# SimingShan/red-diffeq

Hardware: AMD Instinct MI355X
Metric: shot-timesteps/sec (fwd+adj) + per-iter FWI wallclock, OpenFWI 70×70 (higher is better)
Workload: dtype f32; 1 GPU; configs[1]: OpenFWI FlatVel-A 70x70 (310x310 padded), 8 shots/GPU (8 total), nt=1000, fwd+adj gradient + TV + Adam step; global_batch=1, shots_per_gpu=8, shots_total=8, nt=1000, parallelism=shot-parallel x1

## Files before the change

### include/red_diffeq_fwi.h

```cpp
#ifndef RED_DIFFEQ_FWI_H
#define RED_DIFFEQ_FWI_H

#include <stddef.h>
#include <stdint.h>
#include <hip/hip_runtime_api.h>

#ifdef __cplusplus
extern "C" {
#endif

#define RDQ_E_INVALID (-10001)
#define RDQ_E_NOMEM (-10002)
#define RDQ_E_HANDOFF (-10003)

typedef struct rdq_fwi_geom {
    int32_t nz, nx;
    int32_t nbc;
    int32_t nt;
    int32_t ns, ng;
    int32_t sample_temporal;
    float dx, dt;
    int32_t isz, igz;
    const int32_t *isx;
    const int32_t *igx;
    const double *wavelet;
} rdq_fwi_geom;

typedef struct rdq_fwi_plan rdq_fwi_plan;

typedef struct rdq_fwi_sizes_t {
    int32_t Hp, Wp, ld, nrec;
    size_t coeffs;
    size_t vstat;
    size_t seis;
    size_t history;
    size_t ring;
    size_t gA;
    size_t gk_part;
    size_t gbeta;
    size_t colsum;
} rdq_fwi_sizes_t;

int rdq_fwi_plan_create(const rdq_fwi_geom *geom, rdq_fwi_plan **plan);
int rdq_fwi_plan_destroy(rdq_fwi_plan *plan);
int rdq_fwi_sizes(const rdq_fwi_plan *plan, int32_t B, rdq_fwi_sizes_t *out);
int rdq_fwi_set_graphs(rdq_fwi_plan *plan, int32_t enable);
int rdq_fwi_set_tuning(rdq_fwi_plan *plan, int32_t fwd_steps, int32_t adj_steps, int32_t chains);
#define RDQ_VARIANT_FWD_GEN 1
#define RDQ_VARIANT_ADJ_EXACT 2
#define RDQ_VARIANT_NO_XCD_LOCAL 4
#define RDQ_VARIANT_NARROW_CHUNKED 8
#define RDQ_VARIANT_CHUNKED_ADJ_FMA 16
int rdq_fwi_set_variant(rdq_fwi_plan *plan, int32_t flags);
int rdq_fwi_set_wide_adj_steps(rdq_fwi_plan *plan, int32_t steps);
int rdq_fwi_set_wide_adj_shots(rdq_fwi_plan *plan, int32_t shots);
int rdq_fwi_set_wide_fwd_shots(rdq_fwi_plan *plan, int32_t shots);
int rdq_fwi_set_wide_fwd_steps(rdq_fwi_plan *plan, int32_t steps);
int rdq_fwi_set_rows_per_wave(rdq_fwi_plan *plan, int32_t fwd_rows, int32_t adj_rows);
int rdq_fwi_set_sweep_delay(rdq_fwi_plan *plan, int32_t fwd_ticks, int32_t adj_ticks);
int rdq_fwi_set_persistent(rdq_fwi_plan *plan, int32_t mode);
int rdq_fwi_status(rdq_fwi_plan *plan, hipStream_t stream);
int rdq_fwi_debug_words(rdq_fwi_plan *plan, uint32_t out[32]);
int rdq_fwi_set_status_buffer(rdq_fwi_plan *plan, uint32_t *words);
int rdq_fwi_launch_info(rdq_fwi_plan *plan, int32_t B, int32_t out[6]);
int rdq_fwi_wide_info(rdq_fwi_plan *plan, int32_t B, int32_t out[4]);
int rdq_fwi_set_profile(rdq_fwi_plan *plan, int32_t enable);
int rdq_fwi_read_profile(rdq_fwi_plan *plan, uint64_t out[12]);
int rdq_fwi_profile_waves(rdq_fwi_plan *plan, int32_t adj, uint64_t *out, size_t count);

#define RDQ_VEL_NORMALIZED 0
#define RDQ_VEL_PHYSICAL 1

int rdq_fwi_coeffs(const rdq_fwi_plan *plan, int32_t B, const float *v, const int64_t strides[4],
                   int32_t vel_mode, float *coeffs, void *vstat, hipStream_t stream);

int rdq_fwi_forward(const rdq_fwi_plan *plan, int32_t B, const float *coeffs, float *seis,
                    float *history, float *ring, hipStream_t stream);

int rdq_fwi_adjoint(const rdq_fwi_plan *plan, int32_t B, const float *coeffs,
                    const float *history, const float *dseis, float *ring, float *gA,
                    double *gk_part, float *gbeta, hipStream_t stream);

typedef struct rdq_fwi_ckpt_sizes_t {
    int32_t nseg; int32_t seg_levels;
    size_t ckpt;
    size_t seg;
} rdq_fwi_ckpt_sizes_t;
int rdq_fwi_ckpt_sizes(const rdq_fwi_plan *plan, int32_t B, int32_t K, rdq_fwi_ckpt_sizes_t *out);
int rdq_fwi_forward_ckpt(const rdq_fwi_plan *plan, int32_t B, int32_t K, const float *coeffs,
                         float *seis, float *ckpt, float *ring, hipStream_t stream);
int rdq_fwi_adjoint_ckpt(const rdq_fwi_plan *plan, int32_t B, int32_t K, const float *coeffs,
                         const float *ckpt, float *seg, const float *dseis, float *ring,
                         float *gA, double *gk_part, float *gbeta, hipStream_t stream);
int rdq_fwi_ckpt_info(rdq_fwi_plan *plan, int32_t B, int32_t K, int32_t out[4]);

int rdq_fwi_grad_finalize(const rdq_fwi_plan *plan, int32_t B, const float *coeffs,
                          const void *vstat, const float *gA, const double *gk_part,
                          const float *gbeta, int32_t vel_mode, double *colsum, float *g_v,
                          hipStream_t stream);

size_t rdq_l1_partial_bytes(int32_t B, int64_t n);
int rdq_l1_forward(int32_t B, int64_t n, const float *pred, const float *y, const float *mask,
                   float *loss, float *nobs, void *partial, hipStream_t stream);
int rdq_l1_backward(int32_t B, int64_t n, const float *pred, const float *y, const float *mask,
                    const float *nobs, const float *gout, float *dpred, hipStream_t stream);

int rdq_smooth_reg_forward(int32_t kind, int32_t B, int32_t H, int32_t W, const float *mu,
                           float *loss, hipStream_t stream);
int rdq_smooth_reg_backward(int32_t kind, int32_t B, int32_t H, int32_t W, const float *mu,
                            const float *gout, float *grad, hipStream_t stream);

#ifdef __cplusplus
}
#endif
#endif
```

### red-diffeq_amd/csrc/fwi.hip

```cpp
#include <hip/hip_runtime.h>

#include <algorithm>
#include <atomic>
#include <cmath>
#include <cstdint>
#include <cstdlib>
#include <cstring>
#include <new>
#include <vector>
#include <initializer_list>
#include <mutex>
#include <utility>

#include "red_diffeq_fwi.h"

#pragma clang fp contract(off)

namespace {

constexpr float C1X2 = -5.0f;
constexpr float C2 = (float)(4.0 / 3.0);
constexpr float C3 = (float)(-1.0 / 12.0);

#define RDQ_CHECK(x)                                   \
// ... 710 lines not shown
        rofs[r] = wrapn(uz, g.Hp) * g.ld;                                                          \
        const int rr = w * R + r;                                                                  \
        if (rr >= H && rr < RH - H && uz < g.Hp) rin |= 1u << r;                                   \
    }

template <int T, int NW, int R, bool GEN, bool PAIR>
__global__ __launch_bounds__(64 * NW) void k_fwd_tw(FwdTBArgs a)
{
    __shared__ f32x2 xch[2][NW][4][64];
    __shared__ f32x2 As[NW][R][64];
    TW_REGION_INIT()
    const int jg = s - g.s_off, s_first = g.s_off + jg * a.spw, nsh = min(a.spw, a.ns_sh - jg * a.spw);
    (void)bs; (void)so;
    f32x2 C1[R], C2v[R];
    unsigned smask = 0;
    int rrow = -1;
    {
        const float *AL = a.coeffs + (size_t)b * g.slice;
        const __amdgpu_buffer_rsrc_t RA = rsrc_of(AL, sbytes), R1 = rsrc_of(AL + g.cstride, sbytes),
                                     R2 = rsrc_of(AL + 2 * g.cstride, sbytes);
#pragma unroll
        for (int r = 0; r < R; ++r) {
            const int gz = wrapn(uz0 + r, g.Hp);
            if constexpr (GEN) {
                const Coef c0 = gen_coef(a.cg, b, gz, gx0), c1 = gen_coef(a.cg, b, gz, gx1);
                As[w][r][lane] = f32x2{c0.al, c1.al}; C1[r] = f32x2{c0.t1, c1.t1}; C2v[r] = f32x2{c0.t2, c1.t2};
            } else {
                As[w][r][lane] = ld2<PAIR>(RA, v0, v1, rofs[r] * 4);
                C1[r] = ld2<PAIR>(R1, v0, v1, rofs[r] * 4);
                C2v[r] = ld2<PAIR>(R2, v0, v1, rofs[r] * 4);
            }
            if (gz == g.isz) smask |= 1u << r;
            if (gz == g.igz) rrow = r;
        }
    }
    int rs0 = 0, re0 = 0, rs1 = 0, re1 = 0;
    if (rrow >= 0) { rs0 = g.rcv_start[gx0]; re0 = g.rcv_start[gx0 + 1]; rs1 = g.rcv_start[gx1]; re1 = g.rcv_start[gx1 + 1]; }
    const int rc0 = xin0 && rs0 < re0 ? g.rcv_list[rs0] : -1, rc1 = xin1 && rs1 < re1 ? g.rcv_list[rs1] : -1;
    const bool rmulti = __any(re0 - rs0 > 1 || re1 - rs1 > 1);
    const f32x2 kC2 = {C2, C2}, kC3 = {C3, C3};
    auto kargs = [&]() {
        const __attribute__((address_space(4))) FwdTBArgs *k_ =
            (const __attribute__((address_space(4))) FwdTBArgs *)__builtin_amdgcn_kernarg_segment_ptr();
        asm volatile("" : "+s"(k_));
        return k_;
    };
    f32x2 P0[R], P1[R];
    auto load_shot = [&](int ss_) {
        const auto *k_ = kargs();
        const size_t so_ = (size_t)(b * k_->g.ns + ss_) * k_->g.slice;
        const __amdgpu_buffer_rsrc_t RPv = rsrc_of(k_->in_prev + so_, sbytes), RCu = rsrc_of(k_->in_cur + so_, sbytes);
#pragma unroll
        for (int r = 0; r < R; ++r) {
            P0[r] = ld2<PAIR>(RPv, v0, v1, rofs[r] * 4);
            P1[r] = ld2<PAIR>(RCu, v0, v1, rofs[r] * 4);
        }
    };
    load_shot(s_first);
    for (int sh = 0; sh < nsh; ++sh) {
    const auto *ka = kargs();
    const int ss = s_first + sh, bss = b * ka->g.ns + ss;
    const size_t soo = (size_t)bss * ka->g.slice;
    if ((T & 1) && sh) __syncthreads();
    const int isx = ka->g.isx[ss];
    const bool sc0 = gx0 == isx, sc1 = gx1 == isx;
    const float bsrc = smask ? ka->coeffs[4 * ka->g.cstride + (size_t)b * ka->g.slice + (size_t)ka->g.isz * ka->g.ld + isx] : 0.0f;
#pragma unroll
    for (int t = 0; t < T; ++t) {
        f32x2 *cur = (t & 1) ? P0 : P1;
        f32x2 *prv = (t & 1) ? P1 : P0;
        tw_put<NW, R>(xch, t & 1, w, lane, cur);
        __syncthreads();
        const Halo2 h2 = tw_get<NW>(xch, t & 1, w, lane);
#pragma unroll
        for (int r = 0; r < R; ++r) {
            TW_VERT(cur, r, h2, zm2, zm1, zp1, zp2)
            const f32x2 c = cur[r];
            const HTaps x = htaps(c);
            f32x2 s1 = zm1 + zp1; s1 = s1 + x.l1; s1 = s1 + x.r1;
            f32x2 s2 = zm2 + zp2; s2 = s2 + x.l2; s2 = s2 + x.r2;
            f32x2 lap = kC2 * s1; const f32x2 l2 = kC3 * s2; lap = lap + l2;
            f32x2 a1 = C1[r] * c; const f32x2 a2 = C2v[r] * prv[r]; a1 = a1 - a2;
            const f32x2 a3 = As[w][r][lane] * lap;
            prv[r] = a1 + a3;
        }
        if (smask) {
            const float add = bsrc * ka->w[t];
            const f32x2 av = {sc0 ? add : -0.0f, sc1 ? add : -0.0f};
#pragma unroll
            for (int r = 0; r < R; ++r)
                if (smask & (1u << r)) prv[r] = prv[r] + av;
        }
        const int n = ka->n0 + t;
        if (ka->hist) {
            const __amdgpu_buffer_rsrc_t HS = rsrc_of(ka->hist + (size_t)(n + 2 - ka->hbase) * ka->g.level + soo, sbytes);
#pragma unroll
            for (int r = 0; r < R; ++r)
                if (rin & (1u << r)) st2<PAIR, CP_NT>(prv[r], HS, vi0, vi1, rofs[r] * 4);
        }
        if (ka->seis && rrow >= 0 && (rin & (1u << rrow)) && (n % ka->g.st) == 0) {
            f32x2 val = prv[0];
#pragma unroll
            for (int r = 1; r < R; ++r) if (r == rrow) val = prv[r];
            float *SK = ka->seis + ((size_t)bss * ka->g.nrec + n / ka->g.st) * ka->g.ng;
            if (rc0 >= 0) SK[rc0] = val.x;
            if (rc1 >= 0) SK[rc1] = val.y;
            if (rmulti) {
                if (xin0) for (int j = rs0 + 1; j < re0; ++j) SK[ka->g.rcv_list[j]] = val.x;
                if (xin1) for (int j = rs1 + 1; j < re1; ++j) SK[ka->g.rcv_list[j]] = val.y;
            }
        }
    }
    if (ka->out_cur) {
        constexpr bool odd = (T & 1) != 0;
        const __amdgpu_buffer_rsrc_t OC = rsrc_of(ka->out_cur + soo, sbytes), OP = rsrc_of(ka->out_prev + soo, sbytes);
#pragma unroll
        for (int r = 0; r < R; ++r)
            if (rin & (1u << r)) {
                st2<PAIR>(odd ? P0[r] : P1[r], OC, vi0, vi1, rofs[r] * 4);
                st2<PAIR>(odd ? P1[r] : P0[r], OP, vi0, vi1, rofs[r] * 4);
            }
    }
    if (sh + 1 < nsh) load_shot(ss + 1);
    }
}

template <int T, int NW, int R, bool PAIR, bool EXACT>
__global__ __launch_bounds__(64 * NW) void k_adj_tw(AdjTBArgs a)
{
    __shared__ f32x2 xq[2][NW][4][64];
    __shared__ f32x2 xp[2][NW][4][64];
    __shared__ f32x2 As[NW][R][64];
    TW_REGION_INIT()
    const int jg = s - g.s_off, s_first = g.s_off + jg * a.spw, nsh = min(a.spw, a.ns_sh - jg * a.spw);
    (void)bs; (void)so;
    f32x2 KP[R];
    unsigned pmask = 0, smask = 0, rmask = 0;
    const f32x2 kC2 = {C2, C2}, kC3 = {C3, C3}, kC1X2 = {C1X2, C1X2}, k2 = {2.0f, 2.0f}, k1 = {1.0f, 1.0f};
    const bool plane = lane >= H / 2 - 1 && lane < 64 - H / 2 + 1;
    const int pv0 = plane ? v0 : OOB, pv1 = plane ? v1 : OOB;
    {
        int gz[R];
#pragma unroll
        for (int r = 0; r < R; ++r) {
            gz[r] = wrapn(uz0 + r, g.Hp);
            const int rr = w * R + r;
            if (rr >= H - 2 && rr < RH - H + 2) pmask |= 1u << r;
            if (gz[r] == g.isz) smask |= 1u << r;
            if (gz[r] == g.igz) rmask |= 1u << r;
        }
        Coef c0[R], c1[R];
#pragma unroll
        for (int r = 0; r < R; ++r) { c0[r] = gen_coef(a.cg, b, gz[r], gx0); c1[r] = gen_coef(a.cg, b, gz[r], gx1); }
#pragma unroll
        for (int r = 0; r < R; ++r) { As[w][r][lane] = f32x2{c0[r].al, c1[r].al}; KP[r] = f32x2{c0[r].kp, c1[r].kp}; }
    }
    const int rcv0 = rmask ? g.rlane[gx0] : -1, rcv1 = rmask ? g.rlane[gx1] : -1;
    f32x2 L0[R], L1[R], GA[R], Pn[R];
    auto kargs = [&]() {
        const __attribute__((address_space(4))) AdjTBArgs *k_ =
            (const __attribute__((address_space(4))) AdjTBArgs *)__builtin_amdgcn_kernarg_segment_ptr();
        asm volatile("" : "+s"(k_));
        return k_;
    };
    auto load_shot = [&](int ss_) {
        const auto *k_ = kargs();
        const size_t so_ = (size_t)(b * k_->g.ns + ss_) * k_->g.slice;
        const __amdgpu_buffer_rsrc_t RL1 = rsrc_of(k_->in_l1 + so_, sbytes), RL2 = rsrc_of(k_->in_l2 + so_, sbytes);
        const __amdgpu_buffer_rsrc_t RG = rsrc_of(k_->gA + so_, sbytes);
        const __amdgpu_buffer_rsrc_t HR = rsrc_of(k_->hist + (size_t)(k_->k0 - k_->hbase) * k_->g.level + so_, sbytes);
#pragma unroll
        for (int r = 0; r < R; ++r) L1[r] = ld2<PAIR>(RL1, v0, v1, rofs[r] * 4);
#pragma unroll
        for (int r = 0; r < R; ++r) L0[r] = ld2<PAIR>(RL2, v0, v1, rofs[r] * 4);
#pragma unroll
        for (int r = 0; r < R; ++r) Pn[r] = (pmask & (1u << r)) ? ld2<PAIR>(HR, pv0, pv1, rofs[r] * 4) : f32x2{0.0f, 0.0f};
#pragma unroll
        for (int r = 0; r < R; ++r) GA[r] = (rin & (1u << r)) ? ld2<PAIR>(RG, vi0, vi1, rofs[r] * 4) : f32x2{0.0f, 0.0f};
    };
    load_shot(s_first);
    for (int sh = 0; sh < nsh; ++sh) {
    const auto *ka = kargs();
    const int ss = s_first + sh, bss = b * ka->g.ns + ss;
    const size_t soo = (size_t)bss * ka->g.slice;
    const int isx = ka->g.isx[ss];
    const bool sc0 = xin0 && gx0 == isx, sc1 = xin1 && gx1 == isx;
    const __amdgpu_buffer_rsrc_t DSR = rsrc_of(ka->dseis + (size_t)bss * ka->g.nrec * ka->g.dstride);
    const bool gbl = (smask & rin) && (sc0 || sc1);
    float gbacc = gbl ? ka->gbeta[bss] : 0.0f;
    double ksum = 0.0;
#pragma unroll
    for (int t = 0; t < T; ++t) {
        __builtin_amdgcn_sched_barrier(0);
        const int k = ka->k0 - t;
        f32x2 *cur = (t & 1) ? L0 : L1;
        f32x2 *prv = (t & 1) ? L1 : L0;
        f32x2 P[R];
#pragma unroll
        for (int r = 0; r < R; ++r) P[r] = Pn[r];
        if (t + 1 < T) {
            const __amdgpu_buffer_rsrc_t HR = rsrc_of(ka->hist + (size_t)(k - 1 - ka->hbase) * ka->g.level + soo, sbytes);
#pragma unroll
            for (int r = 0; r < R; ++r) if (pmask & (1u << r)) Pn[r] = ld2<PAIR>(HR, pv0, pv1, rofs[r] * 4);
        }
        const int ri = rmask ? rec_index(k - 1, ka->g.st) : -1;
        f32x2 dsv = {-0.0f, -0.0f};
        if (ri >= 0) {
            const int ro = ri * ka->g.dstride;
            const float d0 = bload(DSR, rcv0 >= 0 ? (ro + rcv0) * 4 : OOB, 0);
            const float d1 = bload(DSR, rcv1 >= 0 ? (ro + rcv1) * 4 : OOB, 0);
            dsv = f32x2{rcv0 >= 0 ? d0 : -0.0f, rcv1 >= 0 ? d1 : -0.0f};
        }
        f32x2 q[R];
#pragma unroll
        for (int r = 0; r < R; ++r) q[r] = As[w][r][lane] * cur[r];
        tw_put<NW, R>(xq, t & 1, w, lane, q);
        tw_put<NW, R>(xp, t & 1, w, lane, P);
        __syncthreads();
        const Halo2 hq = tw_get<NW>(xq, t & 1, w, lane);
        const Halo2 hp = tw_get<NW>(xp, t & 1, w, lane);
#pragma unroll
        for (int r = 0; r < R; ++r) {
            TW_VERT(q, r, hq, qm2, qm1, qp1, qp2)
            const HTaps x = htaps(q[r]);
            f32x2 n1 = qm1 + qp1; n1 = n1 + x.l1; n1 = n1 + x.r1;
            f32x2 n2 = qm2 + qp2; n2 = n2 + x.l2; n2 = n2 + x.r2;
            if constexpr (EXACT) {
                f32x2 nb = kC2 * n1; const f32x2 nb2 = kC3 * n2; nb = nb + nb2;
                f32x2 t1 = kC1X2 * As[w][r][lane]; t1 = t1 + k2; t1 = t1 - KP[r];
                const f32x2 t2 = k1 - KP[r];
                f32x2 l = t1 * cur[r]; const f32x2 l2 = t2 * prv[r]; l = l - l2; l = l + nb;
                prv[r] = l;
            } else {
                const f32x2 nb = fma2(kC3, n2, kC2 * n1);
                const f32x2 t1 = fma2(kC1X2, As[w][r][lane], k2) - KP[r], t2 = k1 - KP[r];
                prv[r] = fma2(t1, cur[r], fma2(-t2, prv[r], nb));
            }
        }
        if (ri >= 0) {
#pragma unroll
            for (int r = 0; r < R; ++r)
                if (rmask & (1u << r)) prv[r] = prv[r] + dsv;
        }
#pragma unroll
        for (int r = 0; r < R; ++r) {
            if (!(rin & (1u << r))) continue;
            TW_VERT(P, r, hp, pm2, pm1, pp1, pp2)
            const f32x2 pc = P[r];
            const HTaps x = htaps(pc);
            f32x2 s1 = pm1 + pp1; s1 = s1 + x.l1; s1 = s1 + x.r1;
            f32x2 s2 = pm2 + pp2; s2 = s2 + x.l2; s2 = s2 + x.r2;
            const f32x2 l = prv[r];
            const f32x2 dl = cur[r] - l;
            if constexpr (EXACT) {
                f32x2 lap = kC2 * s1; const f32x2 lq = kC3 * s2; lap = lap + lq;
                f32x2 d = kC1X2 * pc; d = d + lap;
                const f32x2 c = l * d;
                GA[r] = GA[r] + c;
                f32x2 kk = KP[r] * pc; kk = kk * dl;
                ksum += xin0 ? (double)kk.x : 0.0;
                ksum += xin1 ? (double)kk.y : 0.0;
            } else {
                const f32x2 d = fma2(kC1X2, pc, fma2(kC3, s2, kC2 * s1));
                GA[r] = fma2(l, d, GA[r]);
                const f32x2 kk = (KP[r] * pc) * dl;
                ksum += (double)(xin0 ? kk.x : 0.0f);
                ksum += (double)(xin1 ? kk.y : 0.0f);
            }
            if ((smask & (1u << r)) && (sc0 || sc1)) { const float gb = (sc0 ? l.x : l.y) * ka->w[t]; gbacc = gbacc + gb; }
        }
    }
    {
        constexpr bool odd = (T & 1) != 0;
        const __amdgpu_buffer_rsrc_t O1 = rsrc_of(ka->out_l1 + soo, sbytes), O2 = rsrc_of(ka->out_l2 + soo, sbytes);
        const __amdgpu_buffer_rsrc_t RG = rsrc_of(ka->gA + soo, sbytes);
#pragma unroll
        for (int r = 0; r < R; ++r)
            if (rin & (1u << r)) {
                st2<PAIR>(odd ? L0[r] : L1[r], O1, vi0, vi1, rofs[r] * 4);
                st2<PAIR>(odd ? L1[r] : L0[r], O2, vi0, vi1, rofs[r] * 4);
                st2<PAIR>(GA[r], RG, vi0, vi1, rofs[r] * 4);
            }
    }
    if (sh + 1 < nsh) load_shot(ss + 1);
    if (gbl) ka->gbeta[bss] = gbacc;
#pragma unroll
    for (int o = 32; o > 0; o >>= 1) ksum += __shfl_xor(ksum, o, 64);
    double *red = reinterpret_cast<double *>(&xq[0][0][0][0]);
    __syncthreads();
    if (lane == 0) red[w] = ksum;
    __syncthreads();
    if (threadIdx.x == 0) {
        double tot = red[0];
        for (int i = 1; i < NW; ++i) tot += red[i];
        unsafeAtomicAdd(&ka->gk_part[(size_t)bss * ka->nblk + ti.tile], tot);
    }
    }
}
#undef TW_VERT
#undef TW_REGION_INIT

constexpr int CP_SC1 = 16;
constexpr int PT_ADJ_SG = 8;
constexpr size_t PROF_RAW = 8;
constexpr size_t PROF_WAVES = 4096 * 16;
constexpr size_t PROF_WORDS = PROF_RAW + PROF_WAVES * 3;
constexpr unsigned long long PT_TIMEOUT_TICKS = 20000000ull;

typedef unsigned int u32x2 __attribute__((ext_vector_type(2)));
typedef unsigned int u32x4 __attribute__((ext_vector_type(4)));
typedef float f32x2 __attribute__((ext_vector_type(2)));
__device__ __forceinline__ u32x4 gran2(unsigned tag, float v0, float v1)
{
    u32x4 x;
    x.x = __float_as_uint(v0); x.y = tag; x.z = __float_as_uint(v1); x.w = tag;
    return x;
}
__device__ __forceinline__ void gran_put(__amdgpu_buffer_rsrc_t r, int voff, int soff, unsigned tag, float v0, float v1)
{
    __builtin_amdgcn_raw_buffer_store_b128(gran2(tag, v0, v1), r, voff, soff, CP_SC1);
}
__device__ __forceinline__ void gran_put_l2(__amdgpu_buffer_rsrc_t r, int voff, int soff, unsigned tag, float v0, float v1)
{
    __builtin_amdgcn_raw_buffer_store_b128(gran2(tag, v0, v1), r, voff, soff, 0);
}
__device__ __forceinline__ u32x4 gran_get(__amdgpu_buffer_rsrc_t r, int voff, int soff)
{
    return __builtin_amdgcn_raw_buffer_load_b128(r, voff, soff, CP_SC1);
}

__device__ __forceinline__ float wav_s(const float *w, int i)
{
    return ((const __attribute__((address_space(4))) float *)w)[i];
}

__device__ __forceinline__ int wrap_row(int uz, int Hp)
{
    uz = uz < 0 ? uz + Hp : uz;
    return uz >= Hp ? uz - Hp : uz;
}

struct PtTile { int tx, ty, tile, sl; bool valid, local; };
constexpr unsigned long long PT_ARRIVE_TICKS = 10000000ull;

__device__ PtTile pt_assign(const TBGeo &g, unsigned *status, int xcd_mode)
{
    __shared__ int sh[3];
    unsigned *cnt = status + 16;
    if (threadIdx.x == 0) {
        unsigned x = 0;
        if (xcd_mode) {
            asm volatile("s_getreg_b32 %0, hwreg(HW_REG_XCC_ID)" : "=s"(x));
            x &= 7u;
        }
        const unsigned slot = __hip_atomic_fetch_add(cnt + x, 1u, __ATOMIC_RELAXED, __HIP_MEMORY_SCOPE_AGENT);
        unsigned n[8], tot = 0;
        const unsigned long long t0 = __builtin_amdgcn_s_memrealtime();
        bool ok = true;
        for (;;) {
            tot = 0;
            for (int i = 0; i < 8; ++i) {
                n[i] = __hip_atomic_load(cnt + i, __ATOMIC_RELAXED, __HIP_MEMORY_SCOPE_AGENT);
                tot += n[i];
            }
            if (tot >= gridDim.x) break;
            if (__builtin_amdgcn_s_memrealtime() - t0 > PT_ARRIVE_TICKS) { ok = false; break; }
            __builtin_amdgcn_s_sleep(2);
        }
        int sl = -1, tile = 0, local = 0;
        if (ok) {
            const int Tt = g.ntiles, S = g.nsl;
            int placed = 0, take[8];
            for (int i = 0; i < 8; ++i) {
                take[i] = xcd_mode ? min((int)n[i] / Tt, S - placed) : 0;
                placed += take[i];
            }
            int base = 0;
            for (int i = 0; i < (int)x; ++i) base += take[i];
            if ((int)slot < take[x] * Tt) {
                sl = base + (int)slot / Tt; tile = (int)slot % Tt; local = 1;
            } else {
                int r = (int)slot - take[x] * Tt;
                for (int i = 0; i < (int)x; ++i) r += (int)n[i] - take[i] * Tt;
                if (r < (S - placed) * Tt) { sl = placed + r / Tt; tile = r % Tt; }
            }
        } else {
            __hip_atomic_store(status, 2u, __ATOMIC_RELAXED, __HIP_MEMORY_SCOPE_AGENT);
        }
        sh[0] = sl; sh[1] = tile; sh[2] = local;
    }
    __syncthreads();
    PtTile t;
    t.sl = sh[0]; t.tile = sh[1]; t.local = sh[2] != 0;
    t.valid = t.sl >= 0;
    t.ty = t.tile / g.tiles_x;
    t.tx = t.tile - t.ty * g.tiles_x;
    return t;
}

#define PT_REGION_INIT(NW_, RW_)                                                                    \
    PT_REGION_HEAD(NW_, RW_)                                                                        \
    const int bs = __builtin_amdgcn_readfirstlane(g.sl_off + ti.sl);                                \
    const int b = __builtin_amdgcn_readfirstlane(bs / g.ns);                                        \
    const int s = __builtin_amdgcn_readfirstlane(bs - b * g.ns);                                    \
    PT_REGION_GEOM()

#define PT_REGION_HEAD(NW_, RW_)                                                                    \
    constexpr int R = (RW_), RP = (RW_) / 2, RH = (NW_) * (RW_), H = 2 * T, IW = 64 - 2 * H,       \
                  IH = RH - 2 * H;                                                                  \
    const int lane = threadIdx.x & 63;                                                              \
    const int w = __builtin_amdgcn_readfirstlane(threadIdx.x >> 6);                                \
    const PtTile ti = pt_assign(g, a.status, a.xcd_mode);                                           \
    if (!ti.valid) return;                                                                          \
    const bool gl2 = ti.local;

#define PT_REGION_GEOM()                                                                            \
    const int tx = __builtin_amdgcn_readfirstlane(ti.tx), ty = __builtin_amdgcn_readfirstlane(ti.ty); \
    const int tile = __builtin_amdgcn_readfirstlane(ti.tile);                                       \
    const int ux = tx * IW - H + lane;                                                              \
    const int gx = wrapn(ux, g.Wp);                                                                 \
    const bool xin = lane >= H && lane < 64 - H && ux < g.Wp;                                       \
    const int vw = min(IW, g.Wp - tx * IW), vh = min(IH, g.Hp - ty * IH);                           \
    const bool bx = g.tiles_x == 1 || lane - H < H || lane - H >= vw - H;                           \
    const bool cx = lane - H < vw + H;                                                              \
    const int uz0 = ty * IH - H + w * R;                                                            \
    unsigned rin = 0, rby = 0, rcy = 0;                                                             \
    _Pragma("unroll") for (int r = 0; r < R; ++r) {                                                 \
        const int rr = w * R + r, ly = rr - H;                                                      \
        if (rr >= H && rr < RH - H && uz0 + r < g.Hp) rin |= 1u << r;                               \
        if (g.ntiles == g.tiles_x || ly < H || ly >= vh - H) rby |= 1u << r;                        \
        if (ly < vh + H) rcy |= 1u << r;                                                            \
    }                                                                                               \
    const size_t so = (size_t)bs * g.slice;                                                         \
    const int vo16 = gx * 16;                                                                       \
    const bool hx = !xin && cx, xb = xin && bx;                                                     \
                                                        \
    const int vo_hx = hx ? vo16 : OOB, vo_cx = cx ? vo16 : OOB;                                     \
    const int vo_xin = xin ? vo16 : OOB, vo_xb = xb ? vo16 : OOB;                                   \
    const bool keep_in = xin || cx;
#define PT_ROFS(r) (wrap_row(uz0 + (r), g.Hp) * g.ld)

#define PT_SWEEP(GR, TAG, V0, V1, SG)                                                               \
    {                                                                                               \
        unsigned long long t0_ = 0;                                                                 \
        const unsigned long long ts_ = prof ? __builtin_amdgcn_s_memrealtime() : 0;                 \
        if constexpr (PT_PRIO) __builtin_amdgcn_s_setprio(PT_PRIO_WAIT);                            \
        for (unsigned pass_ = 0; live; ++pass_) {                                                   \
             \
            unsigned rin_ = rin, rcy_ = rcy;                                                        \
            LAUNDER(rin_); LAUNDER(rcy_);                                                           \
            bool ok_ = true;                                                                        \
            _Pragma("unroll") for (int g_ = 0; g_ < R; g_ += (SG)) {                                \
                u32x4 x_[(SG)];                                                                     \
                int o_[(SG)];                                                                       \
                constexpr int GN_ = (SG) < R ? (SG) : R;    \
                _Pragma("unroll") for (int i_ = 0; i_ < GN_; ++i_) {                                \
                    const int r = g_ + i_ < R ? g_ + i_ : R - 1;                                    \
                    const bool rowin_ = g_ + i_ < R && ((rin_ >> r) & 1u), rowcy_ = g_ + i_ < R && ((rcy_ >> r) & 1u); \
                    o_[i_] = rowin_ ? vo_hx : (rowcy_ ? vo_cx : OOB);                               \
                    x_[i_] = gran_get(GR, o_[i_], PT_ROFS(r) * 16);                                 \
                }                                                                                   \
                _Pragma("unroll") for (int i_ = 0; i_ < GN_; ++i_) {                                \
                    const int r = g_ + i_ < R ? g_ + i_ : R - 1;                                    \
                    const bool nd_ = o_[i_] != OOB;                                                 \
                    ok_ = ok_ && (!nd_ || (x_[i_].y == (TAG) && x_[i_].w == (TAG)));                \
                    PT_AT(V0, r) = nd_ ? __uint_as_float(x_[i_].x) : PT_AT(V0, r);                  \
                    PT_AT(V1, r) = nd_ ? __uint_as_float(x_[i_].z) : PT_AT(V1, r);                  \
                }                                                                                   \
            }                                                                                       \
            const bool done_ = __all(ok_);                                                          \
            if (prof && pass_ == 0) tfp += __builtin_amdgcn_s_memrealtime() - ts_;                   \
            if (done_) { npass += pass_ + 1; break; }                                               \
            if (pass_ == 0) t0_ = __builtin_amdgcn_s_memrealtime();                                 \
            if ((pass_ & 15) == 15) {                                                               \
                if (__hip_atomic_load(a.status, __ATOMIC_RELAXED, __HIP_MEMORY_SCOPE_AGENT) != 0)   \
                    live = false;                                                                   \
                else if (__builtin_amdgcn_s_memrealtime() - t0_ > PT_TIMEOUT_TICKS) {               \
                    __hip_atomic_store(a.status, 1u, __ATOMIC_RELAXED, __HIP_MEMORY_SCOPE_AGENT);   \
                    if (lane == 0) {                          \
                        a.status[1] = (TAG); a.status[2] = blockIdx.x; a.status[3] = bs;            \
                        a.status[4] = tile; a.status[5] = gl2; a.status[6] = w;                      \
                    }                                                                               \
                    live = false;                                                                   \
                }                                                                                   \
            }                                                                                       \
            __builtin_amdgcn_s_sleep(1);                                                            \
        }                                                                                           \
        if constexpr (PT_PRIO) __builtin_amdgcn_s_setprio(PT_PRIO_SWEPT);                           \
                     \
        unsigned rin_ = rin, rcy_ = rcy;                                                            \
        LAUNDER(rin_); LAUNDER(rcy_);                                                               \
        _Pragma("unroll") for (int r = 0; r < R; ++r) {                                             \
            const bool rowin_ = (rin_ >> r) & 1u, rowcy_ = (rcy_ >> r) & 1u;                        \
            const bool keep_ = rowin_ ? keep_in : (rowcy_ && cx);                                   \
            PT_AT(V0, r) = keep_ ? PT_AT(V0, r) : 0.0f;                                             \
            PT_AT(V1, r) = keep_ ? PT_AT(V1, r) : 0.0f;                                             \
        }                                                                                           \
    }

#define PT_PUBLISH(GR, TAG, V0, V1)                                                                 \
    {                                                                                               \
        unsigned rin_ = rin, rby_ = rby;                                                            \
        LAUNDER(rin_); LAUNDER(rby_);                                                               \
        if (gl2) {                                                                                  \
            _Pragma("unroll") for (int r = 0; r < R; ++r) {                                         \
                if (!((rin_ >> r) & 1u)) continue;                                                  \
                gran_put_l2(GR, ((rby_ >> r) & 1u) ? vo_xin : vo_xb, PT_ROFS(r) * 16, (TAG),        \
                            PT_AT(V0, r), PT_AT(V1, r));                                            \
            }                                                                                       \
        } else {                                                                                    \
            _Pragma("unroll") for (int r = 0; r < R; ++r) {                                         \
                if (!((rin_ >> r) & 1u)) continue;                                                  \
                gran_put(GR, ((rby_ >> r) & 1u) ? vo_xin : vo_xb, PT_ROFS(r) * 16, (TAG),           \
                         PT_AT(V0, r), PT_AT(V1, r));                                               \
            }                                                                                       \
        }                                                                                           \
    }

#define PT_SWEEP_DELAY()                                                                            \
    if (a.sweep_delay > 0) {                                                                        \
        const unsigned long long d0_ = __builtin_amdgcn_s_memrealtime();                            \
        while (__builtin_amdgcn_s_memrealtime() - d0_ < (unsigned long long)a.sweep_delay)          \
            __builtin_amdgcn_s_sleep(1);                                                            \
    }

#define PT_PROF(ACC)                                                                                \
    if (prof) { const unsigned long long now_ = __builtin_amdgcn_s_memrealtime(); ACC += now_ - tm; tm = now_; }

#define LAUNDER(x)                                                                                  \
    do {                                                                                            \
        x = __builtin_amdgcn_readfirstlane(x);    \
        asm volatile("" : "+s"(x));                                                                 \
    } while (0)

struct FwdPtArgs {
    TBGeo g;
    const float *coeffs;
    const float *wav;
    float *hist;
    float *seis;
    unsigned long long *gran;
    unsigned *status;
    unsigned long long *prof;
    int nt;
    int xcd_mode;
    int sweep_delay;
};

#define FWD_HIST(V, N)                                                                              \
    {                                                                                               \
        const int so_ = ((N) - n0) * L4;                                                            \
        _Pragma("unroll") for (int r = 0; r < R; ++r)                                               \
            __builtin_amdgcn_raw_buffer_store_b32(__float_as_uint(PT_AT(V, r)), HFe, hv[r], so_, CP_NT); \
    }
#define FWD_RECORD                                                                                  \
    {                                                                                               \
        int rrw_ = rrow;                                                                            \
        LAUNDER(rrw_);                                                                              \
        if (rrw_ >= 0) {                                                                            \
            _Pragma("unroll") for (int t = 0; t < T; ++t) {                                         \
                const int n = n0 + t;                                                               \
                const int ri_ = n < a.nt ? rec_index(n, g.st) : -1;                                 \
                if (ri_ >= 0) {                                                                     \
                    __builtin_amdgcn_raw_buffer_store_b32(__float_as_uint(rv[t]), SKR, vrec, ri_ * ng4, 0); \
                    unsigned rm_ = rmulti;                                                          \
                    LAUNDER(rm_);                                                                   \
                    if (rm_ && rec) {                          \
                        float *SK = a.seis + ((size_t)bs * g.nrec + ri_) * g.ng;                    \
                        for (int j = rs + 1; j < re; ++j) SK[g.rcv_list[j]] = rv[t];                \
                    }                                                                               \
                }                                                                                   \
            }                                                                                       \
        }                                                                                           \
    }

template <int RP, bool M>
__device__ constexpr int pt_pair(int r) { return M ? (r < RP ? r : 2 * RP - 1 - r) : r % RP; }
template <int RP, bool M>
__device__ constexpr int pt_half(int r) { return M ? (r < RP ? 0 : 1) : r / RP; }
#define PT_AT(V, r) V[pt_pair<RP, PT_MIR>(r)][pt_half<RP, PT_MIR>(r)]
__device__ __forceinline__ f32x2 swp(f32x2 v) { return f32x2{v.y, v.x}; }
#define MIR_VERT(X, i, m1, p1, m2, p2)                                                              \
    const f32x2 m1 = (i) >= 1 ? X[(i) - 1] : E1;                                                    \
    const f32x2 p1 = (i) <= RP - 2 ? X[(i) + 1] : swp(X[RP - 1]);                                   \
    const f32x2 m2 = (i) >= 2 ? X[(i) - 2] : ((i) == 1 ? E1 : E2);                                  \
    const f32x2 p2 = (i) <= RP - 3 ? X[(i) + 2] : ((i) == RP - 2 ? swp(X[RP - 1]) : swp(X[RP - 2]));

#define FWD_PAIRS_NB(CUR, PRV, LO, HI)                                                                        \
    {                                                                                               \
        _Pragma("unroll") for (int i = (LO); i < (HI); ++i) {                                        \
            MIR_VERT(CUR, i, m1, p1, m2, p2)                                                        \
            f32x2 s1 = m1 + p1; s1 = s1 + xl1[i]; s1 = s1 + xr1[i];                                 \
            const f32x2 la = kC2 * s1;                                                              \
            f32x2 s2 = m2 + p2;                               \
            s2.x = s2.x + dpp_shr1(xl1[i].x); s2.y = s2.y + dpp_shr1(xl1[i].y);                     \
            s2.x = s2.x + dpp_shl1(xr1[i].x); s2.y = s2.y + dpp_shl1(xr1[i].y);                     \
            const f32x2 l2 = kC3 * s2; const f32x2 lap = la + l2;                                   \
            const f32x2 a3 = A[i] * lap;                                                            \
            PRV[i] = tt[i] + a3;                                                                    \
        }                                                                                           \
        unsigned sm0_ = (HI) > (LO) ? smask : 0u;                                                  \
        LAUNDER(sm0_);                                    \
        if (sm0_) {                                   \
            float wt_ = wv[t];                                                                      \
            asm volatile("" : "+s"(wt_));                                                           \
            const float add = scol ? bsrc * wt_ : -0.0f;                                            \
            unsigned one_ = s1row;                                                                  \
            LAUNDER(one_);                                                                          \
            if (one_) {                                                                             \
                const f32x2 av = shalf ? f32x2{-0.0f, add} : f32x2{add, -0.0f};                     \
                int sp_ = spair;                                                                    \
                LAUNDER(sp_);                                                                       \
                _Pragma("unroll") for (int i = (LO); i < (HI); ++i)                                  \
                    if (i == sp_) PRV[i] = PRV[i] + av;                                             \
            } else {                                                                                \
                unsigned sm_ = smask;                                                               \
                LAUNDER(sm_);                                                                       \
                _Pragma("unroll") for (int r = 0; r < R; ++r)                                       \
                    if (pt_pair<RP, PT_MIR>(r) >= (LO) && pt_pair<RP, PT_MIR>(r) < (HI) && ((sm_ >> r) & 1u)) \
                        PT_AT(PRV, r) = PT_AT(PRV, r) + add;                                        \
            }                                                                                       \
        }                                                                                           \
    }
#define FWD_STEP_NB(CUR, PRV)                                                                       \
    {                                                                                               \
        u32x2 f_;                                                                                   \
        f32x2 E1, E2;                                                                               \
        xm_load<NW>(xm, n & 1, w, lane, f_, E1, E2);                                                \
        f32x2 xl1[RP], xr1[RP], tt[RP];                                                             \
        _Pragma("unroll") for (int i = 0; i < RP; ++i) {                                             \
            const f32x2 c = CUR[i];                                                                 \
            xl1[i] = f32x2{dpp_shr1(c.x), dpp_shr1(c.y)};                                           \
            xr1[i] = f32x2{dpp_shl1(c.x), dpp_shl1(c.y)};                                           \
            f32x2 a1 = C1[i] * c; const f32x2 a2 = C2v[i] * PRV[i]; a1 = a1 - a2;                   \
            tt[i] = a1;                                                                             \
            asm volatile("" : "+v"(tt[i]));              \
        }                                                                                           \
        xm_wait<NW>(xm, n & 1, w, lane, (unsigned)n + 1u, f_, E1, E2, a.status, live);              \
        FWD_PAIRS_NB(CUR, PRV, 0, 2)                                                                          \
        if (t + 1 < T) xm_put<NW>(xm, (n + 1) & 1, w, lane, (unsigned)n + 2u, PRV[0], PRV[1]);      \
        __builtin_amdgcn_s_setprio(PT_PRIO_BODY);                                                   \
        FWD_PAIRS_NB(CUR, PRV, 2, RP)                                                                         \
        if (a.hist && (t + 1 < T || e + 1 == nep)) FWD_HIST(PRV, n)                                 \
        int rr_ = rrow;                                                                             \
        LAUNDER(rr_);                                                                               \
        if (rr_ >= 0) {                               \
            int rp_ = rpair;                                                                        \
            LAUNDER(rp_);                                                                           \
            f32x2 v_ = PRV[0];                                                                      \
            _Pragma("unroll") for (int i = 1; i < RP; ++i) if (i == rp_) v_ = PRV[i];                \
            rv[t] = rhalf ? v_.y : v_.x;                                                            \
        }                                                                                           \
    }

template <int T, int NW, int RW, bool PROF>
__global__ __launch_bounds__(64 * NW) void k_fwd_pt(FwdPtArgs a)
{
    unsigned long long *const prof = PROF ? a.prof : nullptr;
    constexpr bool PT_MIR = true;
    constexpr bool PT_PRIO = true;
    __shared__ XmBox<NW> xm;
    const TBGeo &g = a.g;
    PT_REGION_INIT(NW, RW)
    const float *AL = a.coeffs + (size_t)b * g.slice;
    f32x2 A[RP], C1[RP], C2v[RP], P0[RP], P1[RP];
    const f32x2 kC2 = {C2, C2}, kC3 = {C3, C3};
    unsigned smask = 0;
    int rrow = -1;
#pragma unroll
    for (int r = 0; r < R; ++r) {
        const int gz = wrap_row(uz0 + r, g.Hp);
        const int o = gz * g.ld + gx;
        PT_AT(A, r) = AL[o]; PT_AT(C1, r) = AL[g.cstride + o]; PT_AT(C2v, r) = AL[2 * g.cstride + o];
        PT_AT(P0, r) = 0.0f; PT_AT(P1, r) = 0.0f;
        if (gz == g.isz) smask |= 1u << r;
        if (gz == g.igz && ((rin >> r) & 1u)) rrow = r;
    }
    smask = __builtin_amdgcn_readfirstlane(smask);
    rrow = __builtin_amdgcn_readfirstlane(rrow);
    const int isx = g.isx[s];
    const bool scol = gx == isx;
    const float bsrc = (smask != 0) ? AL[4 * g.cstride + (size_t)g.isz * g.ld + isx] : 0.0f;

    int rs = 0, re = 0, rcv0 = -1;
    if (rrow >= 0) {
        rs = g.rcv_start[gx]; re = g.rcv_start[gx + 1];
        rcv0 = rs < re ? g.rcv_list[rs] : -1;
    }
    const bool rec = rrow >= 0 && xin && rcv0 >= 0;
    const unsigned rmulti = __any(re - rs > 1);
    const __amdgpu_buffer_rsrc_t SKR = rsrc_of(a.seis + (size_t)bs * g.nrec * g.ng);
    const int vrec = rec ? rcv0 * 4 : OOB, ng4 = g.ng * 4;
    const unsigned s1row = smask != 0 && (smask & (smask - 1u)) == 0;
    const int sr1 = smask ? __builtin_ctz(smask) : 0;
    const int spair = __builtin_amdgcn_readfirstlane(PT_MIR ? (sr1 < RP ? sr1 : R - 1 - sr1) : sr1 % RP);
    const int rpair = __builtin_amdgcn_readfirstlane(rrow < 0 ? 0 : PT_MIR ? (rrow < RP ? rrow : R - 1 - rrow) : rrow % RP);
    const bool shalf = sr1 >= RP, rhalf = rrow >= RP;
    float rv[T];
#pragma unroll
    for (int t = 0; t < T; ++t) rv[t] = 0.0f;
    const size_t L = g.level;
    const int L4 = (int)(L * 4);
    int hv[R];
#pragma unroll
    for (int r = 0; r < R; ++r) hv[r] = (((rin >> r) & 1u) && xin) ? (PT_ROFS(r) + gx) * 4 : OOB;
    const int nep = (a.nt + T - 1) / T;
    bool live = true;
    unsigned long long tsw = 0, tst = 0, tpb = 0, tm = prof ? __builtin_amdgcn_s_memrealtime() : 0;
    unsigned long long tfp = 0, npass = 0;
    float wv[T];
#pragma unroll
    for (int t = 0; t < T; ++t) wv[t] = wav_s(a.wav, min(t, a.nt - 1));
    __builtin_amdgcn_s_waitcnt(0x0F70);
#define FWD_ISSUE _Pragma("unroll") for (int t = 0; t < T; ++t) wv[t] = wav_s(a.wav, min(n0 + T + t, a.nt - 1));
    xm_init<NW>(xm, w, lane);
    __syncthreads();
    xm_put<NW>(xm, 0, w, lane, 1u, f32x2{0.0f, 0.0f}, f32x2{0.0f, 0.0f});
#define FWD_STEP_SEL FWD_STEP_NB
    for (int e = 0; e < nep; ++e) {
        const int n0 = e * T;
        const __amdgpu_buffer_rsrc_t HFe = rsrc_of(a.hist + (size_t)(n0 + 2) * L + so);
        PT_PROF(tsw)
#pragma unroll
        for (int t = 0; t < T; ++t) {
            const int n = n0 + t;
            if (n >= a.nt) break;
            if (t & 1) FWD_STEP_SEL(P0, P1)
            else FWD_STEP_SEL(P1, P0)
        }
        if (T & 1) {
#pragma unroll
            for (int i = 0; i < RP; ++i) { const f32x2 tmp = P0[i]; P0[i] = P1[i]; P1[i] = tmp; }
        }
        PT_PROF(tst)
        if (e + 1 < nep) {
            const unsigned tag = (unsigned)(e + 1);
            const __amdgpu_buffer_rsrc_t GR = rsrc_of(a.gran + (size_t)(2 * ((e + 1) & 1)) * L + 2 * so);
            PT_PUBLISH(GR, tag, P0, P1)
            PT_PROF(tpb)
            FWD_ISSUE
            PT_SWEEP_DELAY()
            PT_SWEEP(GR, tag, P0, P1, R)
            if (a.hist) FWD_HIST(P1, n0 + T - 1)
            xm_put<NW>(xm, (n0 + T) & 1, w, lane, (unsigned)(n0 + T) + 1u, P1[0], P1[1]);
        }
        FWD_RECORD
    }
#undef FWD_STEP_SEL
#undef FWD_ISSUE
    PT_PROF(tsw)
    if (prof && lane == 0) {
        atomicAdd(prof + 0, tsw); atomicAdd(prof + 1, tst); atomicAdd(prof + 2, tpb); atomicAdd(prof + 3, 1ull);
        atomicAdd(prof + 4, tfp); atomicAdd(prof + 5, npass);
        if (blockIdx.x < PROF_WAVES / 16) {
            unsigned long long *raw = prof + PROF_RAW + ((size_t)blockIdx.x * 16 + w) * 3;
            raw[0] = tsw; raw[1] = tst; raw[2] = tpb;
        }
    }
}

#undef FWD_HIST
#undef FWD_RECORD


struct AdjPtArgs {
    TBGeo g;
    const float *coeffs;
    const float *wav;
    const float *hist;
    const float *dseis;
    float *gA;
    double *gk_part;
    float *gbeta;
    unsigned long long *gran;
    unsigned *status;
    unsigned long long *prof;
    int nt, nblk;
    int xcd_mode;
    int sweep_delay;
};

__device__ __forceinline__ float bload_nt(__amdgpu_buffer_rsrc_t r, int voff, int soff)
{
    return __uint_as_float(__builtin_amdgcn_raw_buffer_load_b32(r, voff, soff, CP_NT));
}

#define ADJ_PLOAD(PC, PH, HR, SOFF)                                                                 \
    {                                                                                               \
        const int so_ = (SOFF);                                                                     \
        _Pragma("unroll") for (int i = 0; i < RP; ++i) {                                             \
            PC[i].x = bload_nt(HR, pv[i + 2], so_);                                                 \
            PC[i].y = bload_nt(HR, pv[i + 6], so_);                                                 \
        }                                                                                           \
        PH[0] = bload_nt(HR, pv[0], so_); PH[1] = bload_nt(HR, pv[1], so_);                         \
        PH[2] = bload_nt(HR, pv[10], so_); PH[3] = bload_nt(HR, pv[11], so_);                       \
    }

#define PAIR_VERT(X, i, m1, p1, m2, p2)                                                             \
    const f32x2 m1 = (i) >= 1 ? X[(i) - 1] : eU1;                                                   \
    const f32x2 p1 = (i) <= RP - 2 ? X[(i) + 1] : eD1;                                              \
    const f32x2 m2 = (i) >= 2 ? X[(i) - 2] : ((i) == 1 ? eU1 : eU2);                                \
    const f32x2 p2 = (i) <= RP - 3 ? X[(i) + 2] : ((i) == RP - 2 ? eD1 : eD2);

#define ADJ_GRAD(CU, LN, P, PH, WK)                                                                 \
    if (grad) {                                                                                     \
        const f32x2 eU1 = {PH[1], P[RP - 1].x}, eU2 = {PH[0], P[RP - 2].x};                         \
        const f32x2 eD1 = {P[0].y, PH[2]}, eD2 = {P[1].y, PH[3]};                                   \
        _Pragma("unroll") for (int i = 0; i < RP; ++i) {                                             \
            PAIR_VERT(P, i, m1, p1, m2, p2)                                                         \
            const f32x2 c = P[i];                                                                   \
            const f32x2 xl1 = {dpp_shr1(c.x), dpp_shr1(c.y)}, xr1 = {dpp_shl1(c.x), dpp_shl1(c.y)}; \
            f32x2 s1 = m1 + p1; s1 = s1 + xl1; s1 = s1 + xr1;                                       \
            f32x2 s2 = m2 + p2;                               \
            s2.x = s2.x + dpp_shr1(xl1.x); s2.y = s2.y + dpp_shr1(xl1.y);                           \
            s2.x = s2.x + dpp_shl1(xr1.x); s2.y = s2.y + dpp_shl1(xr1.y);                           \
            const f32x2 l = LN[i];                                                                  \
            f32x2 lap = kC2 * s1; const f32x2 lq = kC3 * s2; lap = lap + lq;                        \
            f32x2 d = kC1X2 * c; d = d + lap;                                                       \
            const f32x2 cc = l * d;                                                                 \
            GA[i] = GA[i] + cc;                                                                     \
            f32x2 kk = KP[i] * c; const f32x2 dl = CU[i] - l; kk = kk * dl;          \
            if (xin) {                                                               \
                if ((rin >> i) & 1u) ksum += (double)kk.x;                                          \
                if ((rin >> (i + RP)) & 1u) ksum += (double)kk.y;                                   \
            }                                                                                       \
        }                                                                                           \
        if (srow >= 0) {                                   \
            int sr_ = srow;                                                                         \
            LAUNDER(sr_);                                                                           \
            float ls_ = 0.0f;                                                                       \
            _Pragma("unroll") for (int r = 0; r < R; ++r) if (r == sr_) ls_ = PT_AT(LN, r);         \
            const float gb = scol ? ls_ * (WK) : -0.0f;                                             \
            gbacc = gbacc + gb;                                                                     \
        }                                                                                           \
    }

#define ADJ_STEP(CUR, PRV, P, PH, PN, PHN)                                                          \
    {                                                                                               \
        if (t + 1 < T) ADJ_PLOAD(PN, PHN, HRe, (T - 2 - t) * L4)                                    \
        const float dcur = dv[t];                                                                   \
        f32x2 q[RP];                                                                                \
        _Pragma("unroll") for (int i = 0; i < RP; ++i) q[i] = A[i] * CUR[i];                         \
        const Halo4 h4 = exchange_nw<NW>(xch, j & 1, w, lane, q[0].x, q[1].x, q[RP - 2].y, q[RP - 1].y); \
        const f32x2 eU1 = {h4.u1, q[RP - 1].x}, eU2 = {h4.u2, q[RP - 2].x};                         \
        const f32x2 eD1 = {q[0].y, h4.d1}, eD2 = {q[1].y, h4.d2};                                   \
        _Pragma("unroll") for (int i = 0; i < RP; ++i) {                                             \
            PAIR_VERT(q, i, m1, p1, m2, p2)                                                         \
            const f32x2 c = q[i];                                                                   \
            const f32x2 xl1 = {dpp_shr1(c.x), dpp_shr1(c.y)}, xr1 = {dpp_shl1(c.x), dpp_shl1(c.y)}; \
            f32x2 n1 = m1 + p1; n1 = n1 + xl1; n1 = n1 + xr1;                                       \
            f32x2 n2 = m2 + p2;                               \
            n2.x = n2.x + dpp_shr1(xl1.x); n2.y = n2.y + dpp_shr1(xl1.y);                           \
            n2.x = n2.x + dpp_shl1(xr1.x); n2.y = n2.y + dpp_shl1(xr1.y);                           \
            f32x2 nb = kC2 * n1; const f32x2 nb2 = kC3 * n2; nb = nb + nb2;                         \
            f32x2 l = T1v[i] * CUR[i]; const f32x2 l2 = T2v[i] * PRV[i]; l = l - l2; l = l + nb;     \
            PRV[i] = l;                                                                             \
        }                                                                                           \
        if (rrow >= 0 && rec_index(k - 1, g.st) >= 0) {       \
            int rr_ = rrow;                                                                         \
            LAUNDER(rr_);                                                                           \
            _Pragma("unroll") for (int r = 0; r < R; ++r)                                           \
                if (r == rr_) PT_AT(PRV, r) = PT_AT(PRV, r) + dcur;        \
        }                                                                                           \
        if (t + 1 < T || last) ADJ_GRAD(CUR, PRV, P, PH, wv[t])                                     \
    }

template <int T, int NW, bool PROF>
__global__ __launch_bounds__(64 * NW) void k_adj_pt(AdjPtArgs a)
{
    unsigned long long *const prof = PROF ? a.prof : nullptr;
    constexpr bool PT_MIR = false;
    constexpr bool PT_PRIO = false;
    __shared__ float xch[2][NW][4][64];
    __shared__ double red[64 * NW];
    const TBGeo &g = a.g;
    PT_REGION_INIT(NW, TB_R)
    const float *AL = a.coeffs + (size_t)b * g.slice;
    f32x2 A[RP], T1v[RP], T2v[RP], KP[RP], L0[RP], L1[RP], GA[RP];
    const f32x2 kC2 = {C2, C2}, kC3 = {C3, C3}, kC1X2 = {C1X2, C1X2};
    int srow = -1, rrow = -1;
#pragma unroll
    for (int r = 0; r < R; ++r) {
        const int gz = wrap_row(uz0 + r, g.Hp);
        const int o = gz * g.ld + gx;
        PT_AT(A, r) = AL[o]; PT_AT(T1v, r) = AL[g.cstride + o]; PT_AT(T2v, r) = AL[2 * g.cstride + o];
        PT_AT(KP, r) = AL[3 * g.cstride + o];
        PT_AT(L0, r) = 0.0f; PT_AT(L1, r) = 0.0f;
        PT_AT(GA, r) = 0.0f;
        if (gz == g.isz && ((rin >> r) & 1u)) srow = r;
        if (gz == g.igz) rrow = r;
    }
    const bool scol = xin && gx == g.isx[s];
    const int rcv0 = rrow >= 0 ? g.rlane[gx] : -1;
    const float *DSb = a.dseis + (size_t)bs * g.nrec * g.dstride;
    const __amdgpu_buffer_rsrc_t DSR = rsrc_of(DSb);
#define DLOAD(KK)                                                                                   \
    ({                                                                                              \
        const int ri_ = (KK) >= 1 ? rec_index((KK) - 1, g.st) : -1;                                 \
        const bool ok_ = rcv0 >= 0 && ri_ >= 0;                                                     \
        const float v_ = bload(DSR, ok_ ? (ri_ * g.dstride + rcv0) * 4 : OOB, 0);                   \
        ok_ ? v_ : -0.0f;                                                                           \
    })
    const bool grad = rin != 0;
    double ksum = 0.0;
    float gbacc = 0.0f;
    const size_t L = g.level;
    const int L4 = (int)(L * 4);
    f32x2 PA[RP], PB[RP];
    float PHA[4], PHB[4];
    int pv[12];
#pragma unroll
    for (int i = 0; i < 12; ++i) pv[i] = grad ? (wrap_row(uz0 + i - 2, g.Hp) * g.ld + gx) * 4 : OOB;
#define HIST_RSRC(KN) rsrc_of(a.hist + (ptrdiff_t)((KN) - (T - 1)) * (ptrdiff_t)L + (ptrdiff_t)so)
    float wv[T], dv[T];
    {
        const __amdgpu_buffer_rsrc_t H0 = HIST_RSRC(a.nt);
        ADJ_PLOAD(PA, PHA, H0, (T - 1) * L4)
    }
#pragma unroll
    for (int t = 0; t < T; ++t) {
        wv[t] = a.wav[max(a.nt - t - 1, 0)];
        dv[t] = DLOAD(a.nt - t);
    }
    __builtin_amdgcn_s_waitcnt(0x0F70);
#define ADJ_ISSUE                                                                                   \
    {                                                                                               \
        const __amdgpu_buffer_rsrc_t HN = HIST_RSRC(kn);                                            \
        ADJ_PLOAD(PA, PHA, HN, (T - 1) * L4)                                                        \
        _Pragma("unroll") for (int t = 0; t < T; ++t) {                                             \
            wv[t] = a.wav[max(kn - t - 1, 0)];                                                      \
            dv[t] = DLOAD(kn - t);                                                                  \
        }                                                                                           \
    }
    const int nep = (a.nt + T - 1) / T;
    bool live = true;
    unsigned long long tsw = 0, tst = 0, tpb = 0, tm = prof ? __builtin_amdgcn_s_memrealtime() : 0;
    unsigned long long tfp = 0, npass = 0;
    for (int e = 0; e < nep; ++e) {
        const int ke = a.nt - e * T;
        const bool last = e + 1 == nep;
        const __amdgpu_buffer_rsrc_t HRe = HIST_RSRC(ke);
#pragma unroll
        for (int t = 0; t < T; ++t) {
            const int j = e * T + t;
            if (j >= a.nt) break;
            const int k = ke - t;
            if (t & 1) ADJ_STEP(L0, L1, PB, PHB, PA, PHA)
            else ADJ_STEP(L1, L0, PA, PHA, PB, PHB)
        }
        if (T & 1) {
#pragma unroll
            for (int i = 0; i < RP; ++i) {
                const f32x2 tl = L0[i]; L0[i] = L1[i]; L1[i] = tl;
                const f32x2 tp = PA[i]; PA[i] = PB[i]; PB[i] = tp;
                const float th = PHA[i]; PHA[i] = PHB[i]; PHB[i] = th;
            }
        }
        PT_PROF(tst)
        if (!last) {
            const unsigned tag = (unsigned)(e + 1);
            const __amdgpu_buffer_rsrc_t GR = rsrc_of(a.gran + (size_t)(2 * ((e + 1) & 1)) * L + 2 * so);
            PT_PUBLISH(GR, tag, L0, L1)
            ADJ_GRAD(L0, L1, PB, PHB, wv[T - 1])
            const int kn = ke - T;
            PT_PROF(tpb)
            PT_SWEEP_DELAY()
            PT_SWEEP(GR, tag, L0, L1, PT_ADJ_SG)
            ADJ_ISSUE
            PT_PROF(tsw)
        }
    }
#undef DLOAD
#undef ADJ_ISSUE
#undef HIST_RSRC
    if (prof && lane == 0) {
        atomicAdd(prof + 0, tsw); atomicAdd(prof + 1, tst); atomicAdd(prof + 2, tpb); atomicAdd(prof + 3, 1ull);
        atomicAdd(prof + 4, tfp); atomicAdd(prof + 5, npass);
        if (blockIdx.x < PROF_WAVES / 16) {
            unsigned long long *raw = prof + PROF_RAW + ((size_t)blockIdx.x * 16 + w) * 3;
            raw[0] = tsw; raw[1] = tst; raw[2] = tpb;
        }
    }
    if (xin) {
#pragma unroll
        for (int r = 0; r < R; ++r)
            if ((rin >> r) & 1u) a.gA[so + (size_t)PT_ROFS(r) + gx] = PT_AT(GA, r);
    }
    if (srow >= 0 && scol) a.gbeta[bs] = gbacc;
    const int tid = threadIdx.x;
    red[tid] = ksum;
    __syncthreads();
    for (int w2 = 512; w2 > 0; w2 >>= 1) {
        if (tid < w2 && tid + w2 < 64 * NW) red[tid] += red[tid + w2];
        __syncthreads();
    }
    if (tid == 0) a.gk_part[(size_t)bs * a.nblk + tile] = red[0];
}

#define ADJR_LOAD(PD, HR, SOFF)                                                                     \
    {                                                                                               \
        const int so_ = (SOFF);                                                                     \
        _Pragma("unroll") for (int i = 0; i < RP; ++i) {                                             \
            PD[i].x = bload_nt(HR, pr[i], so_);                                                     \
            PD[i].y = bload_nt(HR, pr[R - 1 - i], so_);             \
        }                                                                                           \
    }

#define ADJR_GRAD(CU, LN, WK, P0, P1, P2)                                                           \
    if (grad) {                                                                                     \
        f32x2 u[RP];                                                                                \
        _Pragma("unroll") for (int i = 0; i < RP; ++i) {                                             \
            u[i] = fma2(-T1v[i], P1[i], P0[i]);                                                     \
            u[i] = fma2(T2v[i], P2[i], u[i]);                                                       \
        }                                                                                           \
        int sg_ = srow;                                \
        LAUNDER(sg_);                                                                               \
        if (sg_ >= 0) {                                                                             \
            int sp_ = spair;                                                                        \
            LAUNDER(sp_);                                                                           \
            const float sa_ = scol ? bsrc * (WK) : 0.0f;      \
            const f32x2 sv_ = shalf ? f32x2{0.0f, sa_} : f32x2{sa_, 0.0f};                          \
            f32x2 lp_ = LN[0];                                                                      \
            _Pragma("unroll") for (int i = 0; i < RP; ++i) {                                         \
                if (i == sp_) u[i] = u[i] - sv_;                                                    \
                if (i > 0 && i == sp_) lp_ = LN[i];                                                 \
            }                                                                                       \
            const float ls_ = shalf ? lp_.y : lp_.x;                                                \
            const float gb = scol ? ls_ * (WK) : -0.0f;     \
            gbacc = gbacc + gb;                                                                     \
        }                                                                                           \
             \
        _Pragma("unroll") for (int i = 0; i < RP; ++i) {                                             \
            const f32x2 dd = fma2(A[i], kC1X2 * P1[i], u[i]);                                       \
            GA[i] = fma2(LN[i], dd, GA[i]);                                                         \
            GK[i] = fma2(P1[i], CU[i] - LN[i], GK[i]);                                              \
        }                                                                                           \
    }

#define ADJR_PAIRS_NB(CUR, PRV, LO, HI)                                                             \
    {                                                                                               \
        _Pragma("unroll") for (int i = (LO); i < (HI); ++i) {                                        \
            MIR_VERT(q, i, m1, p1, m2, p2)                                                          \
            const f32x2 c = q[i];                                                                   \
            const f32x2 xl1 = {dpp_shr1(c.x), dpp_shr1(c.y)}, xr1 = {dpp_shl1(c.x), dpp_shl1(c.y)}; \
            f32x2 n1 = m1 + p1; n1 = n1 + xl1; n1 = n1 + xr1;                                       \
            f32x2 n2 = m2 + p2;                               \
            n2.x = n2.x + dpp_shr1(xl1.x); n2.y = n2.y + dpp_shr1(xl1.y);                           \
            n2.x = n2.x + dpp_shl1(xr1.x); n2.y = n2.y + dpp_shl1(xr1.y);                           \
            const f32x2 nb = fma2(kC3, n2, kC2 * n1);                                               \
            PRV[i] = fma2(T1v[i], CUR[i], fma2(-T2v[i], PRV[i], nb));                               \
        }                                                                                           \
        int rr_ = (LO) == 0 ? rlo : rhi;                   \
        LAUNDER(rr_);                                                                               \
        if ((HI) > (LO) && rr_ && rec_index(k - 1, g.st) >= 0) {                                    \
            int rp_ = rpair;                                                                        \
            LAUNDER(rp_);                                                                           \
            const f32x2 dv_ = rhalf ? f32x2{-0.0f, dcur} : f32x2{dcur, -0.0f};        \
            _Pragma("unroll") for (int i = (LO); i < (HI); ++i) if (i == rp_) PRV[i] = PRV[i] + dv_; \
        }                                                                                           \
    }
#define ADJR_STEP_NB(CUR, PRV, P0, P1, P2, PN)                                                      \
    {                                                                                               \
        if (ldall || (grad && k >= 2)) ADJR_LOAD(PN, HRe, (T - 1 - t) * L4)                         \
        const float dcur = dv[t];                                                                   \
        u32x2 f_;                                                                                   \
        f32x2 E1, E2;                                                                               \
        xm_load<NW>(xm, j & 1, w, lane, f_, E1, E2);                                                \
        f32x2 q[RP];                                                                                \
        _Pragma("unroll") for (int i = 0; i < RP; ++i) q[i] = A[i] * CUR[i];                         \
        xm_wait<NW>(xm, j & 1, w, lane, (unsigned)j + 1u, f_, E1, E2, a.status, live);              \
        ADJR_PAIRS_NB(CUR, PRV, 0, 2)                                                               \
        if (t + 1 < T) xm_put<NW>(xm, (j + 1) & 1, w, lane, (unsigned)j + 2u, A[0] * PRV[0], A[1] * PRV[1]); \
        __builtin_amdgcn_s_setprio(PT_PRIO_BODY);                                                   \
        ADJR_PAIRS_NB(CUR, PRV, 2, RP)                                                              \
        if (t + 1 < T || last) ADJR_GRAD(CUR, PRV, wv[t], P0, P1, P2)                               \
    }

template <int T, int NW, int RW, bool PROF>
__global__ __launch_bounds__(64 * NW) void k_adj_pr(AdjPtArgs a)
{
    unsigned long long *const prof = PROF ? a.prof : nullptr;
    constexpr bool PT_PRIO = true;
    constexpr bool PT_MIR = true;
    __shared__ XmBox<NW> xm;
    __shared__ double red[64 * NW];
    static_assert(sizeof(XmBox<NW>) + sizeof(double) * 64 * NW == (size_t)NW * 4608 && NW <= 16,
                  "k_adj_pr: 4 KB of mailboxes + 512 B of reduction per wave (72 KB at 16 waves)");
    const TBGeo &g = a.g;
    PT_REGION_INIT(NW, RW)
    const float *AL = a.coeffs + (size_t)b * g.slice;
    f32x2 A[RP], T1v[RP], T2v[RP], L0[RP], L1[RP], GA[RP], GK[RP];
    const f32x2 kC2 = {C2, C2}, kC3 = {C3, C3}, kC1X2 = {C1X2, C1X2};
    int srow = -1, rrow = -1;
#pragma unroll
    for (int r = 0; r < R; ++r) {
        const int gz = wrap_row(uz0 + r, g.Hp);
        const int o = gz * g.ld + gx;
        PT_AT(A, r) = AL[o]; PT_AT(T1v, r) = AL[g.cstride + o]; PT_AT(T2v, r) = AL[2 * g.cstride + o];
        PT_AT(L0, r) = 0.0f; PT_AT(L1, r) = 0.0f;
        PT_AT(GA, r) = 0.0f; PT_AT(GK, r) = 0.0f;
        if (gz == g.isz && ((rin >> r) & 1u)) srow = r;
        if (gz == g.igz) rrow = r;
    }
    const int isx = g.isx[s];
    const bool scol = xin && gx == isx;
    const float bsrc = srow >= 0 ? AL[4 * g.cstride + (size_t)g.isz * g.ld + isx] : 0.0f;
    const int rcv0 = rrow >= 0 ? g.rlane[gx] : -1;
    const float *DSb = a.dseis + (size_t)bs * g.nrec * g.dstride;
    const __amdgpu_buffer_rsrc_t DSR = rsrc_of(DSb);
    const int spair = __builtin_amdgcn_readfirstlane(srow < 0 ? 0 : srow < RP ? srow : R - 1 - srow);
    const int rpair = __builtin_amdgcn_readfirstlane(rrow < 0 ? 0 : rrow < RP ? rrow : R - 1 - rrow);
    const bool shalf = srow >= RP, rhalf = rrow >= RP;
    const int rlo = __builtin_amdgcn_readfirstlane(rrow >= 0 && rpair < 2 ? 1 : 0);
    const int rhi = __builtin_amdgcn_readfirstlane(rrow >= 0 && rpair >= 2 ? 1 : 0);
#define DLOAD(KK)                                                                                   \
    ({                                                                                              \
        const int ri_ = (KK) >= 1 ? rec_index((KK) - 1, g.st) : -1;                                 \
        const bool ok_ = rcv0 >= 0 && ri_ >= 0;                                                     \
        const float v_ = bload(DSR, ok_ ? (ri_ * g.dstride + rcv0) * 4 : OOB, 0);                   \
        ok_ ? v_ : -0.0f;                                                                           \
    })
    const bool grad = rin != 0;
    float gbacc = 0.0f;
    const size_t L = g.level;
    const int L4 = (int)(L * 4);
    f32x2 Q0[RP], Q1[RP], Q2[RP], Q3[RP];
    int pr[R];
#pragma unroll
    for (int r = 0; r < R; ++r)
        pr[r] = grad ? (PT_ROFS(r) + gx) * 4 : OOB;
#pragma unroll
    for (int i = 0; i < RP; ++i) { Q0[i] = 0.0f; Q1[i] = 0.0f; Q2[i] = 0.0f; Q3[i] = 0.0f; }
#define HIST_RSRC(KN) rsrc_of(a.hist + (ptrdiff_t)((KN) - T - 1) * (ptrdiff_t)L + (ptrdiff_t)so)
    float wv[T], dv[T];
    if (grad) {
        const __amdgpu_buffer_rsrc_t H0 = rsrc_of(a.hist + (ptrdiff_t)(a.nt - 1) * (ptrdiff_t)L + (ptrdiff_t)so);
        ADJR_LOAD(Q0, H0, 2 * L4)
        ADJR_LOAD(Q1, H0, L4)
        ADJR_LOAD(Q2, H0, 0)
    }
#pragma unroll
    for (int t = 0; t < T; ++t) {
        wv[t] = a.wav[max(a.nt - t - 1, 0)];
        dv[t] = DLOAD(a.nt - t);
    }
    __builtin_amdgcn_s_waitcnt(0x0F70);
#define ADJ_ISSUE                                                                                   \
    _Pragma("unroll") for (int t = 0; t < T; ++t) {                                                 \
        wv[t] = a.wav[max(kn - t - 1, 0)];                                                          \
        dv[t] = DLOAD(kn - t);                                                                      \
    }
    const int nep = (a.nt + T - 1) / T;
    bool live = true;
    unsigned long long tsw = 0, tst = 0, tpb = 0, tm = prof ? __builtin_amdgcn_s_memrealtime() : 0;
    unsigned long long tfp = 0, npass = 0;
    xm_init<NW>(xm, w, lane);
    __syncthreads();
    xm_put<NW>(xm, 0, w, lane, 1u, f32x2{0.0f, 0.0f}, f32x2{0.0f, 0.0f});
    for (int e = 0; e < nep; ++e) {
        const int ke = a.nt - e * T;
        const bool last = e + 1 == nep;
        const __amdgpu_buffer_rsrc_t HRe = HIST_RSRC(ke);
        int ldall = grad && ke >= T + 1;
        LAUNDER(ldall);
#pragma unroll
        for (int t = 0; t < T; ++t) {
            const int j = e * T + t;
            if (j >= a.nt) break;
            const int k = ke - t;
            if ((t & 3) == 0) ADJR_STEP_NB(L1, L0, Q0, Q1, Q2, Q3)
            else if ((t & 3) == 1) ADJR_STEP_NB(L0, L1, Q1, Q2, Q3, Q0)
            else if ((t & 3) == 2) ADJR_STEP_NB(L1, L0, Q2, Q3, Q0, Q1)
            else ADJR_STEP_NB(L0, L1, Q3, Q0, Q1, Q2)
        }
        if (T & 1) {
#pragma unroll
            for (int i = 0; i < RP; ++i) { const f32x2 tl = L0[i]; L0[i] = L1[i]; L1[i] = tl; }
        }
#define QW(o) (((T - 1 + (o)) & 3) == 0 ? Q0 : ((T - 1 + (o)) & 3) == 1 ? Q1 : ((T - 1 + (o)) & 3) == 2 ? Q2 : Q3)
        PT_PROF(tst)
        if (!last) {
            const unsigned tag = (unsigned)(e + 1);
            const __amdgpu_buffer_rsrc_t GR = rsrc_of(a.gran + (size_t)(2 * ((e + 1) & 1)) * L + 2 * so);
            PT_PUBLISH(GR, tag, L0, L1)
            ADJR_GRAD(L0, L1, wv[T - 1], QW(0), QW(1), QW(2))
            const int kn = ke - T;
            PT_PROF(tpb)
            PT_SWEEP_DELAY()
            PT_SWEEP(GR, tag, L0, L1, PT_ADJ_SG)
            xm_put<NW>(xm, (e + 1) * T & 1, w, lane, (unsigned)((e + 1) * T) + 1u, A[0] * L1[0], A[1] * L1[1]);
            ADJ_ISSUE
            PT_PROF(tsw)
        }
        if constexpr ((T & 3) != 0) {
#pragma unroll
            for (int i = 0; i < RP; ++i) {
                const f32x2 a0 = QW(1)[i], a1 = QW(2)[i], a2 = QW(3)[i], a3 = QW(4)[i];
                Q0[i] = a0; Q1[i] = a1; Q2[i] = a2; Q3[i] = a3;
            }
        }
    }
#undef QW
#undef DLOAD
#undef ADJ_ISSUE
#undef HIST_RSRC
    if (prof && lane == 0) {
        atomicAdd(prof + 0, tsw); atomicAdd(prof + 1, tst); atomicAdd(prof + 2, tpb); atomicAdd(prof + 3, 1ull);
        atomicAdd(prof + 4, tfp); atomicAdd(prof + 5, npass);
        if (blockIdx.x < PROF_WAVES / 16) {
            unsigned long long *raw = prof + PROF_RAW + ((size_t)blockIdx.x * 16 + w) * 3;
            raw[0] = tsw; raw[1] = tst; raw[2] = tpb;
        }
    }
    double ksum = 0.0;
    if (xin) {
#pragma unroll
        for (int r = 0; r < R; ++r)
            if ((rin >> r) & 1u) {
                a.gA[so + (size_t)PT_ROFS(r) + gx] = PT_AT(GA, r) / PT_AT(A, r);
                const float kp = AL[3 * g.cstride + PT_ROFS(r) + gx];
                ksum += (double)kp * (double)PT_AT(GK, r);
            }
    }
    if (srow >= 0 && scol) a.gbeta[bs] = gbacc;
    const int tid = threadIdx.x;
    red[tid] = ksum;
    __syncthreads();
    for (int w2 = 512; w2 > 0; w2 >>= 1) {
        if (tid < w2 && tid + w2 < 64 * NW) red[tid] += red[tid + w2];
        __syncthreads();
    }
    if (tid == 0) a.gk_part[(size_t)bs * a.nblk + tile] = red[0];
}
#undef ADJR_STEP_NB
#undef ADJR_PAIRS_NB
#undef FWD_STEP_NB
#undef FWD_PAIRS_NB
#undef MIR_VERT
#undef ADJR_GRAD
#undef ADJR_LOAD
#undef ADJ_STEP
#undef ADJ_GRAD
#undef ADJ_PLOAD
#undef PAIR_VERT
#undef PT_AT
#undef PT_SWEEP
#undef PT_PUBLISH
#undef PT_PROF
#undef PT_SWEEP_DELAY
#undef PT_ROFS
#undef PT_REGION_INIT
#undef PT_REGION_HEAD
#undef PT_REGION_GEOM
#undef LAUNDER
#undef TB_VERT

__global__ __launch_bounds__(256) void k_rcv_fold(const float *__restrict__ ds, float *__restrict__ out,
                                                  const int *__restrict__ colx, const int *__restrict__ rcv_start,
                                                  const int *__restrict__ rcv_list, int ng, int ncolr, size_t rows)
{
    const size_t n = rows * (size_t)ncolr;
    for (size_t i = (size_t)blockIdx.x * blockDim.x + threadIdx.x; i < n; i += (size_t)gridDim.x * blockDim.x) {
        const size_t row = i / ncolr;
        const int c = (int)(i - row * ncolr), x = colx[c];
        const float *d = ds + row * ng;
        const int r0 = rcv_start[x], r1 = rcv_start[x + 1];
        float v = d[rcv_list[r0]];
        for (int j = r0 + 1; j < r1; ++j) v = v + d[rcv_list[j]];
        out[i] = v;
    }
}

struct FinArgs {
    int B, ns, nz, nx, nbc, Hp, Wp, ld, isz, nblk;
    float dt, dx;
    double scale;
    size_t cstride, slice;
    const float *coeffs, *gA, *gbeta, *vmin;
    const int64_t *amin;
    const double *gk_part;
    const int *isx;
    double *colsum;
    float *out;
};

constexpr int FIN_MAXW = 4096;
__global__ __launch_bounds__(256) void k_fin_rows(FinArgs p)
{
    __shared__ double gv_s[FIN_MAXW];
    const int z = blockIdx.x, b = blockIdx.y;
    const size_t ro = (size_t)b * p.slice + (size_t)z * p.ld;
    const float *GA = p.gA + (size_t)b * p.ns * p.slice + (size_t)z * p.ld;
    const float *V = p.coeffs + 5 * p.cstride + ro;
    const int amz = (int)(p.amin[b] / p.nx), amx = (int)(p.amin[b] - (int64_t)amz * p.nx);
    const int apz = amz == 0 ? 0 : amz + p.nbc, apx = amx == 0 ? 0 : amx + p.nbc;
    __shared__ double gk_s[256];
    if (z == apz) {
        const int cnt = p.ns * p.nblk, per = (cnt + 255) / 256;
        const double *GK = p.gk_part + (size_t)b * cnt;
        double acc = 0.0;
        const int j0 = threadIdx.x * per, j1 = min(cnt, j0 + per);
        for (int j = j0; j < j1; j += 4) {
            double v[4];
#pragma unroll
            for (int u = 0; u < 4; ++u) v[u] = GK[min(j + u, cnt - 1)];
#pragma unroll
            for (int u = 0; u < 4; ++u) if (j + u < j1) acc += v[u];
        }
        gk_s[threadIdx.x] = acc;
    }
    __syncthreads();
    for (int x = threadIdx.x; x < p.Wp; x += blockDim.x) {
        float a1 = V[x] * p.dt; a1 = a1 / p.dx;
        float ga = 0.0f;
        {
            int s = 0;
            for (; s + 4 <= p.ns; s += 4) {
                float v[4];
#pragma unroll
                for (int u = 0; u < 4; ++u) v[u] = GA[(size_t)(s + u) * p.slice + x];
#pragma unroll
                for (int u = 0; u < 4; ++u) ga = ga + v[u];
            }
            for (; s < p.ns; ++s) ga = ga + GA[(size_t)s * p.slice + x];
        }
        float t = ga * (2.0f * a1); t = t / p.dx; t = t * p.dt;
        double gv = (double)t;
        if (z == p.isz) {
            for (int s = 0; s < p.ns; ++s)
                if (p.isx[s] == x) {
                    const float b1 = V[x] * p.dt;
                    float u = p.gbeta[b * p.ns + s] * (2.0f * b1); u = u * p.dt;
                    gv += (double)u;
                }
        }
        if (z == apz && x == apx) {
            double gk = 0.0;
            for (int j = 0; j < 256; ++j) gk += gk_s[j];
            gv += gk / (double)p.vmin[b];
        }
        gv_s[x] = gv;
    }
    __syncthreads();
    double *CS = p.colsum + ((size_t)b * p.Hp + z) * p.nx;
    for (int ix = 1 + threadIdx.x; ix < p.nx - 1; ix += blockDim.x) CS[ix] = gv_s[ix + p.nbc];
    const int w = threadIdx.x >> 6, lane = threadIdx.x & 63;
    if (w < 2) {
        const int x0 = w == 0 ? 0 : p.nbc + p.nx - 1, x1 = w == 0 ? p.nbc + 1 : p.Wp;
        double acc = 0.0;
        for (int x = x0 + lane; x < x1; x += 64) acc += gv_s[x];
        for (int o = 32; o > 0; o >>= 1) acc += __shfl_down(acc, o, 64);
        if (lane == 0) {
            if (p.nx == 1) { if (w == 0) { double t2 = acc; for (int x = p.nbc + 1; x < p.Wp; ++x) t2 += gv_s[x]; CS[0] = t2; } }
            else CS[w == 0 ? 0 : p.nx - 1] = acc;
        }
    }
}
__global__ __launch_bounds__(256) void k_fin_cols(FinArgs p)
{
    const int i = blockIdx.x * blockDim.x + threadIdx.x;
    const int b = blockIdx.y;
    if (i >= p.nz * p.nx) return;
    const int iz = i / p.nx, ix = i - iz * p.nx;
    const int z0 = iz == 0 ? 0 : iz + p.nbc;
    const int z1 = iz == p.nz - 1 ? p.Hp : iz + p.nbc + 1;
    const double *cs = p.colsum + (size_t)b * p.Hp * p.nx + ix;
    double acc = 0.0;
    int z = z0;
    for (; z + 16 <= z1; z += 16) {
        double v[16];
#pragma unroll
        for (int u = 0; u < 16; ++u) v[u] = cs[(size_t)(z + u) * p.nx];
#pragma unroll
        for (int u = 0; u < 16; ++u) acc += v[u];
    }
    for (; z < z1; ++z) acc += cs[(size_t)z * p.nx];
    p.out[(size_t)b * p.nz * p.nx + i] = (float)(acc * p.scale);
}

constexpr int L1_BLOCK = 256;
constexpr int L1_ITEMS = 16;

__device__ __forceinline__ double block_sum(double v, double *sh)
{
    const int t = threadIdx.x;
    sh[t] = v;
    __syncthreads();
    for (int w = blockDim.x / 2; w > 0; w >>= 1) {
        if (t < w) sh[t] += sh[t + w];
        __syncthreads();
    }
    const double r = sh[0];
    __syncthreads();
    return r;
}

__global__ __launch_bounds__(L1_BLOCK) void k_l1_partial(int64_t n, const float *__restrict__ pred,
                                                         const float *__restrict__ y,
                                                         const float *__restrict__ mask,
                                                         double *__restrict__ part, int nchunk)
{
    __shared__ double sh[L1_BLOCK];
    const int b = blockIdx.y, c = blockIdx.x;
    const int64_t base = (int64_t)b * n;
    const int64_t c0 = (int64_t)c * L1_BLOCK * L1_ITEMS;
    double se = 0.0, sm = 0.0;
    float dv[L1_ITEMS], mv[L1_ITEMS];
#pragma unroll
    for (int k = 0; k < L1_ITEMS; ++k) {
        const int64_t j = min(c0 + (int64_t)k * L1_BLOCK + threadIdx.x, n - 1);
        mv[k] = mask ? mask[base + j] : 1.0f;
        dv[k] = fabsf(y[base + j] - pred[base + j]);
    }
#pragma unroll
    for (int k = 0; k < L1_ITEMS; ++k) {
        const int64_t j = c0 + (int64_t)k * L1_BLOCK + threadIdx.x;
        if (j < n) {
            se += (double)(dv[k] * mv[k]);
            sm += (double)mv[k];
        }
    }
    se = block_sum(se, sh);
    sm = block_sum(sm, sh);
    if (threadIdx.x == 0) {
        part[((size_t)b * nchunk + c) * 2] = se;
        part[((size_t)b * nchunk + c) * 2 + 1] = sm;
    }
}

__global__ __launch_bounds__(L1_BLOCK) void k_l1_final(int B, int nchunk, const double *__restrict__ part,
                                                       float *loss, float *nobs)
{
    __shared__ double sh[L1_BLOCK];
    const int b = blockIdx.x;
    const double *pb = part + (size_t)b * nchunk * 2;
    double se = 0.0, sm = 0.0;
    int c = threadIdx.x;
    for (; c + 7 * L1_BLOCK < nchunk; c += 8 * L1_BLOCK) {
        double e[8], m[8];
#pragma unroll
        for (int u = 0; u < 8; ++u) { e[u] = pb[(c + u * L1_BLOCK) * 2]; m[u] = pb[(c + u * L1_BLOCK) * 2 + 1]; }
#pragma unroll
        for (int u = 0; u < 8; ++u) { se += e[u]; sm += m[u]; }
    }
    for (; c < nchunk; c += L1_BLOCK) { se += pb[c * 2]; sm += pb[c * 2 + 1]; }
    se = block_sum(se, sh);
    sm = block_sum(sm, sh);
    if (threadIdx.x == 0) {
        const float no = fmaxf((float)sm, 1.0f);
        nobs[b] = no;
        loss[b] = (float)(se / (double)no);
    }
}

__global__ __launch_bounds__(256) void k_l1_backward(int B, int64_t n, const float *__restrict__ pred,
                                                     const float *__restrict__ y,
                                                     const float *__restrict__ mask,
                                                     const float *__restrict__ nobs,
                                                     const float *__restrict__ gout,
                                                     float *__restrict__ dpred)
{
    const int64_t j = (int64_t)blockIdx.x * blockDim.x + threadIdx.x;
    const int b = blockIdx.y;
    if (j >= n) return;
    const int64_t i = (int64_t)b * n + j;
    const float g = gout[b] / nobs[b];
    const float m = mask ? mask[i] : 1.0f;
    const float d = pred[i] - y[i];
    const float sg = d > 0.0f ? 1.0f : (d < 0.0f ? -1.0f : 0.0f);
    dpred[i] = sg * (m * g);
}

__global__ __launch_bounds__(256) void k_smooth_fwd(int kind, int H, int W, const float *__restrict__ mu,
                                                    float *loss)
{
    __shared__ double sh[256];
    const int b = blockIdx.x;
    const float *m = mu + (size_t)b * H * W;
    double sx = 0.0, sy = 0.0;
    const int n = H * W;
    constexpr int CH = 8;
    for (int base = threadIdx.x; base < n; base += CH * blockDim.x) {
        float c[CH], r[CH], d[CH];
#pragma unroll
        for (int u = 0; u < CH; ++u) {
            const int i = base + u * blockDim.x;
            const int z = i / W, x = i - z * W;
            c[u] = i < n ? m[i] : 0.0f;
            r[u] = (i < n && x + 1 < W) ? m[i + 1] : 0.0f;
            d[u] = (i < n && z + 1 < H) ? m[i + W] : 0.0f;
        }
#pragma unroll
        for (int u = 0; u < CH; ++u) {
            const int i = base + u * blockDim.x;
            if (i >= n) break;
            const int z = i / W, x = i - z * W;
            if (x + 1 < W) { const float e = r[u] - c[u]; sx += kind == 0 ? (double)fabsf(e) : (double)(e * e); }
            if (z + 1 < H) { const float e = d[u] - c[u]; sy += kind == 0 ? (double)fabsf(e) : (double)(e * e); }
        }
    }
    sx = block_sum(sx, sh);
    sy = block_sum(sy, sh);
    if (threadIdx.x == 0) {
        const float tx = (float)(sx / (double)((size_t)H * (W - 1)));
        const float ty = (float)(sy / (double)((size_t)(H - 1) * W));
        loss[b] = tx + ty;
    }
}

__global__ __launch_bounds__(256) void k_smooth_bwd(int kind, int H, int W, const float *__restrict__ mu,
                                                    const float *__restrict__ gout, float *__restrict__ grad)
{
    const int i = blockIdx.x * blockDim.x + threadIdx.x;
    const int b = blockIdx.y;
    if (i >= H * W) return;
    const float *m = mu + (size_t)b * H * W;
    const int z = i / W, x = i - z * W;
    const float gx = gout[b] / (float)((size_t)H * (W - 1));
    const float gy = gout[b] / (float)((size_t)(H - 1) * W);
    auto dterm = [&](float d, float g) {
        if (kind == 0) return d > 0.0f ? g : (d < 0.0f ? -g : 0.0f);
        return 2.0f * d * g;
    };
    float acc = 0.0f;
    if (x + 1 < W) acc -= dterm(m[i + 1] - m[i], gx);
    if (x > 0) acc += dterm(m[i] - m[i - 1], gx);
    if (z + 1 < H) acc -= dterm(m[i + W] - m[i], gy);
    if (z > 0) acc += dterm(m[i] - m[i - W], gy);
    grad[(size_t)b * H * W + i] = acc;
}

}

struct GraphEntry {
    int kind;
    int B;
    int K;
    const void *ptrs[8];
    hipGraphExec_t exec;
    uint64_t last_use;
};

constexpr int RDQ_SWEEP_DELAY_FWD = 15, RDQ_SWEEP_DELAY_ADJ = 0;

struct rdq_fwi_plan {
    rdq_fwi_geom g;
    std::vector<int32_t> isx, igx;
    std::vector<double> wav;
    std::vector<float> wavf;
    int Hp, Wp, ld, nrec;
    int *d_isx = nullptr, *d_rcv_start = nullptr, *d_rcv_list = nullptr;
    int *d_rlane = nullptr;
    int *d_colx = nullptr;
    int ncolr = 0;
    bool rmulti = false;
    float *d_wav = nullptr;
    unsigned *d_status = nullptr;
    unsigned *d_status_own = nullptr;
    unsigned long long *d_prof = nullptr;
    std::vector<unsigned long long> prof_host;
    bool graphs = true;
    int persist = 1;
    int xcd_mode = 1;
    std::vector<std::pair<const void *, int>> resident;
    int fwd_rw = 6, adj_rw = 6;
    int fwd_T = 4, adj_T = 4;
    int fwd_delay = RDQ_SWEEP_DELAY_FWD, adj_delay = RDQ_SWEEP_DELAY_ADJ;
    int adj_Tw = 0;
    int fwd_Tw = 0;
    int adj_spw = 0;
    int fwd_spw = 0;
    int chains = 0;
    bool fwd_gen = true;
    bool adj_fma = true;
    bool adj_tw_fma = false;
    bool wide = true;
    hipStream_t cap = nullptr;
    std::vector<hipStream_t> aux;
    std::vector<hipEvent_t> evs;
    std::vector<GraphEntry> cache;
    uint64_t tick = 0;
    std::mutex mu;
    hipStream_t last = nullptr;
    bool have_last = false;
    hipEvent_t handover = nullptr;
};

namespace {

int tiles_x(int Wp, int T) { return (Wp + (64 - 4 * T) - 1) / (64 - 4 * T); }
int tiles_y(int Hp, int T) { return (Hp + (TB_RH - 4 * T) - 1) / (TB_RH - 4 * T); }


TBGeo tb_geo(const rdq_fwi_plan *p, int B)
{
    TBGeo g;
    g.B = B; g.ns = p->g.ns; g.Hp = p->Hp; g.Wp = p->Wp; g.ld = p->ld;
    g.isz = p->g.isz; g.igz = p->g.igz; g.ng = p->g.ng; g.nrec = p->nrec; g.st = p->g.sample_temporal;
    g.slice = (size_t)p->Hp * p->ld;
    g.cstride = (size_t)B * g.slice;
    g.level = (size_t)B * g.ns * g.slice;
    g.isx = p->d_isx; g.rcv_start = p->d_rcv_start; g.rcv_list = p->d_rcv_list;
    g.rlane = p->d_rlane; g.dstride = p->rmulti ? p->ncolr : p->g.ng;
    g.s_off = 0; g.ns_grp = p->g.ns;
    g.sl_off = 0; g.nsl = B * p->g.ns;
    return g;
}

int chain_count(const rdq_fwi_plan *p)
{
    const int c = p->chains > 0 ? p->chains : (p->wide ? 2 : 1);
    return std::max(1, std::min(c, p->g.ns));
}

constexpr int TW_ADJ_DEFAULT = 5;
int wide_adj_depth(const rdq_fwi_plan *p) { return p->adj_Tw > 0 ? p->adj_Tw : TW_ADJ_DEFAULT; }
int wide_fwd_depth(const rdq_fwi_plan *p) { return p->fwd_Tw > 0 ? p->fwd_Tw : p->fwd_T; }

int device_cus()
{
    constexpr int MAXDEV = 64;
    static std::atomic<int> cache[MAXDEV];
    int dev = 0, n = 0;
    if (hipGetDevice(&dev) != hipSuccess) return 256;
    if (dev >= 0 && dev < MAXDEV && (n = cache[dev].load(std::memory_order_relaxed)) > 0) return n;
    if (hipDeviceGetAttribute(&n, hipDeviceAttributeMultiprocessorCount, dev) != hipSuccess || n < 1) n = 256;
    if (dev >= 0 && dev < MAXDEV) cache[dev].store(n, std::memory_order_relaxed);
    return n;
}

int wide_spw(int setting, int regions, int ns, bool adj, int chains)
{
    if (setting > 0) return std::max(1, std::min(setting, ns));
    const int cus = std::max(1, device_cus() / std::max(1, chains));
    const double kappa = adj ? 0.25 : 0.6;
    int pick = 1;
    double best = 1e300;
    for (const int c : {16, 8, 4, 2, 1}) {
        const int spw = std::min(c, ns), groups = (ns + spw - 1) / spw;
        const long long wgs = (long long)regions * groups, rounds = (wgs + cus - 1) / cus;
        const double cost = (double)rounds * (spw + kappa);
        if (cost < best - 1e-9) { best = cost; pick = spw; }
    }
    return pick;
}

int plan_enter(rdq_fwi_plan *p, hipStream_t st)
{
    if (p->have_last && p->last != st) {
        hipStreamCaptureStatus cs = hipStreamCaptureStatusNone, cl = hipStreamCaptureStatusNone;
        RDQ_CHECK(hipStreamIsCapturing(st, &cs));
        RDQ_CHECK(hipStreamIsCapturing(p->last, &cl));
        if (cs == hipStreamCaptureStatusNone && cl == hipStreamCaptureStatusNone) {
            if (!p->handover) RDQ_CHECK(hipEventCreateWithFlags(&p->handover, hipEventDisableTiming));
            RDQ_CHECK(hipEventRecord(p->handover, p->last));
            RDQ_CHECK(hipStreamWaitEvent(st, p->handover, 0));
        }
    }
    p->last = st;
    p->have_last = true;
    return 0;
}

struct GkWriters {
    std::vector<int> chain;
    std::vector<unsigned> stamp;
    unsigned launch = 0;
    int nblk;
    GkWriters(size_t slices, int nblk_) : chain(slices * nblk_, -1), stamp(slices * nblk_, 0u), nblk(nblk_) {}
    bool add(int c, unsigned grid, int tiles_x, int ntiles, int B, int ns, int ns_grp, int s_off, int spw, int ns_sh)
    {
        ++launch;
        const int nsg = B * ns_grp;
        for (unsigned L = 0; L < grid; ++L) {
            const TileId ti = decode_tile((int)L, tiles_x, ntiles, nsg);
            if (!ti.valid) continue;
            if (ti.tile >= nblk) return false;
            const int b = ti.sl / ns_grp, jg = ti.sl - b * ns_grp;
            const int s_first = s_off + jg * spw, nsh = std::min(spw, ns_sh - jg * spw);
            for (int sh = 0; sh < nsh; ++sh) {
                const size_t slot = (size_t)(b * ns + s_first + sh) * nblk + ti.tile;
                if (s_first + sh >= ns || slot >= chain.size()) return false;
                if (stamp[slot] == launch || (chain[slot] >= 0 && chain[slot] != c)) return false;
                stamp[slot] = launch;
                chain[slot] = c;
            }
        }
        return true;
    }
};

int ensure_aux(rdq_fwi_plan *p, int S)
{
    while ((int)p->aux.size() < S - 1) {
        hipStream_t s;
        RDQ_CHECK(hipStreamCreateWithFlags(&s, hipStreamNonBlocking));
        p->aux.push_back(s);
    }
    while ((int)p->evs.size() < S) {
        hipEvent_t e;
        RDQ_CHECK(hipEventCreateWithFlags(&e, hipEventDisableTiming));
        p->evs.push_back(e);
    }
    return 0;
}

int fork_chains(rdq_fwi_plan *p, hipStream_t st, int S)
{
    if (S == 1) return 0;
    RDQ_TRY(ensure_aux(p, S));
    RDQ_CHECK(hipEventRecord(p->evs[0], st));
    for (int c = 1; c < S; ++c) RDQ_CHECK(hipStreamWaitEvent(p->aux[c - 1], p->evs[0], 0));
    return 0;
}

int join_chains(rdq_fwi_plan *p, hipStream_t st, int S)
{
    for (int c = 1; c < S; ++c) {
        RDQ_CHECK(hipEventRecord(p->evs[c], p->aux[c - 1]));
        RDQ_CHECK(hipStreamWaitEvent(st, p->evs[c], 0));
    }
    return 0;
}

CoefGen coef_gen(const rdq_fwi_plan *p, int B, const float *coeffs)
{
    CoefGen c;
    const size_t cstride = (size_t)B * p->Hp * p->ld;
    c.vmod = coeffs + 6 * cstride;
    c.ks = c.vmod + (size_t)B * p->g.nz * p->g.nx;
    c.nz = p->g.nz; c.nx = p->g.nx; c.nbc = p->g.nbc; c.Hp = p->Hp; c.Wp = p->Wp;
    c.dt = p->g.dt; c.dx = p->g.dx;
    c.a = (float)((double)(p->g.nbc - 1) * (double)p->g.dx);
    return c;
}

template <class Args>
struct KernelRef {
    void (*fn)(Args);
    int threads;
};

template <class Args>
void launch_kernel(KernelRef<Args> k, unsigned grid, hipStream_t st, const Args &a)
{
    void *argv[] = {const_cast<Args *>(&a)};
    (void)hipLaunchKernel(reinterpret_cast<const void *>(k.fn), dim3(grid), dim3(k.threads), argv, 0, st);
}

template <int N, class F>
auto with_depth(int T, F &&f)
{
    if constexpr (N == 1) return f(std::integral_constant<int, 1>{});
    else return T >= N ? f(std::integral_constant<int, N>{}) : with_depth<N - 1>(T, f);
}

KernelRef<FwdTBArgs> fwd_tb_kernel(int T, bool gen)
{
    return with_depth<TB_MAXT>(T, [&](auto t) -> KernelRef<FwdTBArgs> {
        return {gen ? k_fwd_tb<t(), true> : k_fwd_tb<t(), false>, 64 * TB_NW};
    });
}
KernelRef<AdjTBArgs> adj_tb_kernel(int T)
{
    return with_depth<TB_MAXT>(T, [](auto t) -> KernelRef<AdjTBArgs> { return {k_adj_tb<t()>, 64 * TB_NW}; });
}

constexpr int TW_FWD_NW = 16, TW_FWD_R = 8, TW_ADJ_NW = 16, TW_ADJ_R = 4;
static_assert(ADJ_W_MAX >= TW_ADJ_MAXT && ADJ_W_MAX >= TB_MAXT, "AdjTBArgs::w holds one sample per step of a launch");
int tw_tiles_x(int Wp, int T) { return (Wp + (TW_W - 4 * T) - 1) / (TW_W - 4 * T); }
int tw_tiles_y(int Hp, int T, bool adj)
{
    const int ih = (adj ? TW_ADJ_NW * TW_ADJ_R : TW_FWD_NW * TW_FWD_R) - 4 * T;
    return (Hp + ih - 1) / ih;
}

static_assert(FWD_W_MAX >= TW_FWD_MAXT && FWD_W_MAX >= TB_MAXT, "FwdTBArgs::w holds one sample per step of a launch");

KernelRef<FwdTBArgs> fwd_tw_kernel(int T, bool gen, bool pair)
{
    constexpr int N = TW_FWD_NW, R = TW_FWD_R;
    return with_depth<TW_FWD_MAXT>(T, [&](auto t) -> KernelRef<FwdTBArgs> {
        if (gen) return {pair ? k_fwd_tw<t(), N, R, true, true> : k_fwd_tw<t(), N, R, true, false>, 64 * N};
        return {pair ? k_fwd_tw<t(), N, R, false, true> : k_fwd_tw<t(), N, R, false, false>, 64 * N};
    });
}
KernelRef<AdjTBArgs> adj_tw_kernel(int T, bool pair, bool exact)
{
    constexpr int N = TW_ADJ_NW, R = TW_ADJ_R;
    return with_depth<TW_ADJ_MAXT>(T, [&](auto t) -> KernelRef<AdjTBArgs> {
        if (exact) return {pair ? k_adj_tw<t(), N, R, true, true> : k_adj_tw<t(), N, R, false, true>, 64 * N};
        return {pair ? k_adj_tw<t(), N, R, true, false> : k_adj_tw<t(), N, R, false, false>, 64 * N};
    });
}

int chunk_depth(const rdq_fwi_plan *p, bool adj)
{
    if (p->wide) return adj ? wide_adj_depth(p) : wide_fwd_depth(p);
    return adj ? p->adj_T : p->fwd_T;
}
KernelRef<FwdTBArgs> chunk_fwd_kernel(const rdq_fwi_plan *p, int nsteps)
{
    return p->wide ? fwd_tw_kernel(nsteps, p->fwd_gen, (p->Wp & 1) == 0) : fwd_tb_kernel(p->fwd_T, p->fwd_gen);
}
KernelRef<AdjTBArgs> chunk_adj_kernel(const rdq_fwi_plan *p, int nsteps)
{
    return p->wide ? adj_tw_kernel(nsteps, (p->Wp & 1) == 0, !p->adj_tw_fma) : adj_tb_kernel(p->adj_T);
}

template <int T, bool PROF>
KernelRef<FwdPtArgs> fwd_pt_T(int NW, int rw)
{
    if (NW == 16) return {k_fwd_pt<T, 16, 4, PROF>, 64 * 16};
    if (NW != 12) return {k_fwd_pt<T, 8, 8, PROF>, 64 * 8};
    switch (rw) {
    case 24: return {k_fwd_pt<T, 4, 24, PROF>, 64 * 4};
    case 12: return {k_fwd_pt<T, 8, 12, PROF>, 64 * 8};
    case 6: return {k_fwd_pt<T, 16, 6, PROF>, 64 * 16};
    default: return {k_fwd_pt<T, 12, 8, PROF>, 64 * 12};
    }
}
KernelRef<FwdPtArgs> fwd_pt_kernel(const rdq_fwi_plan *p, int NW, int T, bool prof)
{
    if (prof && T == 4) return fwd_pt_T<4, true>(NW, p->fwd_rw);
    return with_depth<TB_MAXT>(T, [&](auto t) { return fwd_pt_T<t(), false>(NW, p->fwd_rw); });
}
template <int T, bool PROF>
KernelRef<AdjPtArgs> adj_pt_T(int NW, int rw, bool fma)
{
    if (!fma) {
        if (NW != 12) return {k_adj_pt<T, 8, PROF>, 64 * 8};
        return {k_adj_pt<T, 12, PROF>, 64 * 12};
    }
    if (NW == 16) return {k_adj_pr<T, 16, 4, PROF>, 64 * 16};
    if (NW != 12) return {k_adj_pr<T, 8, 8, PROF>, 64 * 8};
    switch (rw) {
    case 12: return {k_adj_pr<T, 8, 12, PROF>, 64 * 8};
    case 6: return {k_adj_pr<T, 16, 6, PROF>, 64 * 16};
    default: return {k_adj_pr<T, 12, 8, PROF>, 64 * 12};
    }
}
KernelRef<AdjPtArgs> adj_pt_kernel(const rdq_fwi_plan *p, int NW, int T, bool fma, bool prof)
{
    if (prof && T == 4) return adj_pt_T<4, true>(NW, p->adj_rw, fma);
    return with_depth<TB_MAXT>(T, [&](auto t) { return adj_pt_T<t(), false>(NW, p->adj_rw, fma); });
}

template <class Args>
int resident_capacity(rdq_fwi_plan *p, KernelRef<Args> k)
{
    const void *fn = reinterpret_cast<const void *>(k.fn);
    for (const auto &e : p->resident)
        if (e.first == fn) return e.second;
    int dev = 0, cus = 0, nb = 0;
    if (hipGetDevice(&dev) != hipSuccess) return -1;
    if (hipDeviceGetAttribute(&cus, hipDeviceAttributeMultiprocessorCount, dev) != hipSuccess) return -1;
    if (hipOccupancyMaxActiveBlocksPerMultiprocessor(&nb, fn, k.threads, 0) != hipSuccess) return -1;
    if (cus * nb) p->resident.emplace_back(fn, cus * nb);
    return cus * nb;
}

int capacity_nw(rdq_fwi_plan *p, int NW, bool adj, int T)
{
    if (!adj) return resident_capacity(p, fwd_pt_kernel(p, NW, T, false));
    return std::min(resident_capacity(p, adj_pt_kernel(p, NW, T, false, false)),
                    resident_capacity(p, adj_pt_kernel(p, NW, T, true, false)));
}

static int region_rows(int NW) { return NW == 12 ? 96 : 64; }

unsigned pt_tiles_padded(const rdq_fwi_plan *p, int T, int NW)
{
    const int ih = region_rows(NW) - 4 * T;
    const int nt_ = tiles_x(p->Wp, T) * ((p->Hp + ih - 1) / ih);
    return (unsigned)((nt_ + 7) / 8 * 8);
}

int gk_blocks(const rdq_fwi_plan *p)
{
    int n = 0;
    for (int T = 1; T <= TW_ADJ_MAXT; ++T)
        n = std::max(n, tw_tiles_x(p->Wp, T) * tw_tiles_y(p->Hp, T, true));
    for (int T = 1; T <= TB_MAXT; ++T) {
        n = std::max(n, tiles_x(p->Wp, T) * tiles_y(p->Hp, T));
        n = std::max(n, tw_tiles_x(p->Wp, T) * tw_tiles_y(p->Hp, T, true));
        for (int NW : {8, 12, 16}) {
            const int ih = region_rows(NW) - 4 * T;
            n = std::max(n, tiles_x(p->Wp, T) * ((p->Hp + ih - 1) / ih));
        }
    }
    return n;
}

int pt_slices_per_launch(const rdq_fwi_plan *p, int B, int T, int NW, int cap)
{
    if (cap <= 0) return 0;
    const unsigned per = (unsigned)cap / pt_tiles_padded(p, T, NW);
    if (per < 1) return 0;
    const int total = B * p->g.ns, groups = (total + (int)per - 1) / (int)per;
    return (total + groups - 1) / groups;
}

unsigned pt_grid(const rdq_fwi_plan *p, int T, int NW, int nsl, bool adj)
{
    const unsigned S = (unsigned)nsl;
    unsigned grid = pt_tiles_padded(p, T, NW) * S;
    if (p->xcd_mode) {
        const int ih = region_rows(NW) - 4 * T;
        const unsigned Tt = (unsigned)(tiles_x(p->Wp, T) * ((p->Hp + ih - 1) / ih));
        const unsigned want = 8u * Tt * ((S + 7u) / 8u);
        const int cap = capacity_nw(const_cast<rdq_fwi_plan *>(p), NW, adj, T);
        if (want > grid && (int)want <= cap) grid = want;
    }
    if (p->persist == -1) {
        const int cap = capacity_nw(const_cast<rdq_fwi_plan *>(p), NW, adj, T);
        grid = std::max(grid, 2u * (unsigned)std::max(cap, 1));
    }
    return grid;
}

constexpr unsigned PT_SMALL_WG = 200;
int persistent_nw(rdq_fwi_plan *p, int B, bool adj, int *per = nullptr)
{
    if (!p->persist) return 0;
    const int T = adj ? p->adj_T : p->fwd_T;
    const int want = p->persist == -1 ? 1 : p->persist;
    if (want == 1 || want == 16) {
        const int k = pt_slices_per_launch(p, B, T, 16, capacity_nw(p, 16, adj, T));
        const bool small = k >= B * p->g.ns && pt_tiles_padded(p, T, 16) * (unsigned)(B * p->g.ns) <= PT_SMALL_WG;
        if (k > 0 && (want == 16 || small)) { if (per) *per = k; return 16; }
    }
    if (want == 1 || want == 12) {
        const int k = pt_slices_per_launch(p, B, T, 12, capacity_nw(p, 12, adj, T));
        if (k > 0) { if (per) *per = k; return 12; }
    }
    if (want == 1 || want == 8) {
        const int k = pt_slices_per_launch(p, B, T, 8, capacity_nw(p, 8, adj, T));
        if (k > 0) { if (per) *per = k; return 8; }
    }
    return 0;
}

constexpr int ZERO_MAXR = 6;
struct ZeroArgs {
    void *p[ZERO_MAXR];
    size_t n[ZERO_MAXR];
    int nr;
};
__global__ __launch_bounds__(256) void k_zero_regions(ZeroArgs z)
{
    const size_t stride = (size_t)gridDim.x * blockDim.x, t = (size_t)blockIdx.x * blockDim.x + threadIdx.x;
    for (int r = 0; r < z.nr; ++r) {
        if ((reinterpret_cast<uintptr_t>(z.p[r]) & 15) == 0) {
            uint4 *q = static_cast<uint4 *>(z.p[r]);
            const size_t n4 = z.n[r] / 16;
            for (size_t i = t; i < n4; i += stride) q[i] = make_uint4(0u, 0u, 0u, 0u);
            const size_t tail = (z.n[r] - n4 * 16) / 4;
            if (t < tail) reinterpret_cast<unsigned *>(q + n4)[t] = 0u;
        } else {
            unsigned *q = static_cast<unsigned *>(z.p[r]);
            for (size_t i = t; i < z.n[r] / 4; i += stride) q[i] = 0u;
        }
    }
}
static int zero_regions(std::initializer_list<std::pair<void *, size_t>> regs, hipStream_t st)
{
    ZeroArgs z{};
    size_t tot = 0;
    auto flush = [&]() -> int {
        if (!z.nr) return 0;
        const size_t blocks = std::min<size_t>(2048, std::max<size_t>(1, (tot / 16 + 255) / 256));
        hipLaunchKernelGGL(k_zero_regions, dim3((unsigned)blocks), dim3(256), 0, st, z);
        RDQ_CHECK(hipGetLastError());
        z = ZeroArgs{};
        tot = 0;
        return 0;
    };
    for (const auto &r : regs)
        if (r.first && (r.second & 3)) return RDQ_E_INVALID;
    for (const auto &r : regs) {
        if (!r.first || !r.second) continue;
        if (z.nr == ZERO_MAXR) RDQ_TRY(flush());
        z.p[z.nr] = r.first;
        z.n[z.nr++] = r.second;
        tot += r.second;
    }
    return flush();
}

int launch_forward_pt(rdq_fwi_plan *p, int B, int NW, int per, const float *coeffs, float *seis, float *hist, float *ring,
                      hipStream_t st)
{
    FwdPtArgs a{};
    a.g = tb_geo(p, B);
    const int T = p->fwd_T;
    const size_t L = a.g.level;
    if (int e = zero_regions({{hist, hist ? 2 * L * sizeof(float) : 0}, {ring, 4 * L * sizeof(unsigned long long)},
                              {p->d_status + 16, 8 * sizeof(unsigned)}}, st))
        return e;
    const int ih = region_rows(NW) - 4 * T;
    a.g.tiles_x = tiles_x(p->Wp, T);
    a.g.ntiles = a.g.tiles_x * ((p->Hp + ih - 1) / ih);
    a.coeffs = coeffs; a.wav = p->d_wav; a.hist = hist; a.seis = seis;
    a.gran = reinterpret_cast<unsigned long long *>(ring);
    a.status = p->d_status; a.nt = p->g.nt; a.prof = p->d_prof; a.xcd_mode = p->xcd_mode;
    a.sweep_delay = p->fwd_delay;
    for (int s0 = 0; s0 < B * p->g.ns; s0 += per) {
        a.g.sl_off = s0;
        a.g.nsl = std::min(per, B * p->g.ns - s0);
        const unsigned grid = pt_grid(p, T, NW, a.g.nsl, false);
        if (s0 > 0) RDQ_TRY(zero_regions({{p->d_status + 16, 8 * sizeof(unsigned)}}, st));
        launch_kernel(fwd_pt_kernel(p, NW, T, a.prof != nullptr), grid, st, a);
        RDQ_CHECK(hipGetLastError());
    }
    return 0;
}

int launch_adjoint_pt(rdq_fwi_plan *p, int B, int NW, int per, const float *coeffs, const float *hist, const float *dseis,
                      float *ring, float *gA, double *gk, float *gbeta, hipStream_t st)
{
    AdjPtArgs a{};
    a.g = tb_geo(p, B);
    const int T = p->adj_T;
    const size_t L = a.g.level;
    const int nblk_alloc = gk_blocks(p);
    if (int e = zero_regions({{ring, 4 * L * sizeof(unsigned long long)}, {gA, L * sizeof(float)},
                              {gk, (size_t)B * p->g.ns * nblk_alloc * sizeof(double)},
                              {gbeta, (size_t)B * p->g.ns * sizeof(float)}, {p->d_status + 16, 8 * sizeof(unsigned)}},
                             st))
        return e;
    const int ih = region_rows(NW) - 4 * T;
    a.g.tiles_x = tiles_x(p->Wp, T);
    a.g.ntiles = a.g.tiles_x * ((p->Hp + ih - 1) / ih);
    a.coeffs = coeffs; a.wav = p->d_wav; a.hist = hist; a.dseis = dseis;
    a.gA = gA; a.gk_part = gk; a.gbeta = gbeta;
    a.gran = reinterpret_cast<unsigned long long *>(ring);
    a.status = p->d_status; a.nt = p->g.nt; a.nblk = nblk_alloc; a.prof = p->d_prof ? p->d_prof + PROF_WORDS : nullptr;
    a.xcd_mode = p->xcd_mode;
    a.sweep_delay = p->adj_delay;
    for (int s0 = 0; s0 < B * p->g.ns; s0 += per) {
        a.g.sl_off = s0;
        a.g.nsl = std::min(per, B * p->g.ns - s0);
        const unsigned grid = pt_grid(p, T, NW, a.g.nsl, true);
        if (s0 > 0) RDQ_TRY(zero_regions({{p->d_status + 16, 8 * sizeof(unsigned)}}, st));
        launch_kernel(adj_pt_kernel(p, NW, T, p->adj_fma, a.prof != nullptr), grid, st, a);
        RDQ_CHECK(hipGetLastError());
    }
    return 0;
}

struct CkptPlan {
    int K, nseg;
    int lo(int c) const { return hi(c + 1); }
    int hi(int c) const { return (int)std::max<long long>(nt - (long long)c * K, 0); }
    int nt;
};
CkptPlan ckpt_plan(const rdq_fwi_plan *p, int K)
{
    CkptPlan c;
    c.nt = p->g.nt;
    c.K = std::min(K, c.nt);
    c.nseg = (c.nt + c.K - 1) / c.K;
    return c;
}

__global__ __launch_bounds__(256) void k_ckpt_levels(const float *src, float *dst, size_t level, size_t model,
                                                     size_t off, size_t run, int B)
{
    const int lvl = blockIdx.y / B, b = blockIdx.y - lvl * B;
    const size_t base = (size_t)lvl * level + (size_t)b * model + off;
    const size_t stride = (size_t)gridDim.x * blockDim.x;
    for (size_t i = (size_t)blockIdx.x * blockDim.x + threadIdx.x; i < run; i += stride)
        dst[base + i] = src ? src[base + i] : 0.0f;
}

enum class Pass { fwd_ring, fwd_hist, adj_hist, adj_ckpt };
enum class Store { none, ring, ckpt, hist };
struct LevelPair {
    Store store;
    int slot;
};
struct Launch {
    enum Kind { levels, fwd, adj } kind;
    int chain, s_off, ns_sh;
    int first, nsteps;
    int seg, hbase;
    int tiles_x, ntiles, spw, ns_grp;
    unsigned grid;
    LevelPair in, out;
};

std::vector<Launch> chunked_schedule(const rdq_fwi_plan *p, int B, Pass pass, const CkptPlan &cp)
{
    const int Tf = chunk_depth(p, false), Ta = chunk_depth(p, true), S = chain_count(p), ns = p->g.ns;
    std::vector<Launch> sched;
    auto add = [&](Launch::Kind kind, int c, int sg, int first, int nsteps, LevelPair in, LevelPair out) {
        Launch l{};
        l.kind = kind; l.chain = c; l.seg = sg; l.first = first; l.nsteps = nsteps; l.in = in; l.out = out;
        l.hbase = pass == Pass::fwd_ring ? 0 : cp.lo(sg);
        l.s_off = c * ns / S;
        l.ns_sh = (c + 1) * ns / S - l.s_off;
        if (kind != Launch::levels) {
            const bool adj = kind == Launch::adj;
            const int Tl = p->wide ? nsteps : (adj ? Ta : Tf);
            l.tiles_x = p->wide ? tw_tiles_x(p->Wp, Tl) : tiles_x(p->Wp, Tl);
            l.ntiles = l.tiles_x * (p->wide ? tw_tiles_y(p->Hp, Tl, adj) : tiles_y(p->Hp, Tl));
            l.spw = p->wide ? wide_spw(adj ? p->adj_spw : p->fwd_spw, B * l.ntiles, l.ns_sh, adj, S) : 1;
            l.ns_grp = (l.ns_sh + l.spw - 1) / l.spw;
            l.grid = (unsigned)((l.ntiles + 7) / 8 * 8 * B * l.ns_grp);
        }
        sched.push_back(l);
    };
    for (int c = 0; c < S; ++c) {
        int i = 0;
        if (pass == Pass::fwd_ring) {
            for (int sg = cp.nseg - 1; sg >= 0; --sg) {
                const int lo = cp.lo(sg), hi = cp.hi(sg);
                for (int n0 = lo; n0 < hi; n0 += Tf, ++i) {
                    const int n = std::min(Tf, hi - n0), pin = i & 1, pout = pin ^ 1;
                    add(Launch::fwd, c, sg, n0, n,
                        n0 == lo && lo > 0 ? LevelPair{Store::ckpt, 2 * sg} : LevelPair{Store::ring, 2 * pin},
                        n0 + n == hi && hi < cp.nt ? LevelPair{Store::ckpt, 2 * (sg - 1)} : LevelPair{Store::ring, 2 * pout});
                }
            }
            continue;
        }
        for (int sg = 0; sg < cp.nseg; ++sg) {
            const int lo = cp.lo(sg), hi = cp.hi(sg);
            if (pass == Pass::adj_ckpt)
                add(Launch::levels, c, sg, lo, 0, lo > 0 ? LevelPair{Store::ckpt, 2 * sg} : LevelPair{Store::none, 0},
                    LevelPair{Store::hist, 0});
            if (pass != Pass::adj_hist)
                for (int n0 = lo; n0 < hi; n0 += Tf)
                    add(Launch::fwd, c, sg, n0, std::min(Tf, hi - n0), LevelPair{Store::hist, n0 - lo},
                        LevelPair{Store::none, 0});
            if (pass != Pass::fwd_hist)
                for (int k0 = hi; k0 > lo; k0 -= Ta, ++i) {
                    const int pin = i & 1, pout = pin ^ 1;
                    add(Launch::adj, c, sg, k0, std::min(Ta, k0 - lo), LevelPair{Store::ring, 2 * pin},
                        LevelPair{Store::ring, 2 * pout});
                }
        }
    }
    return sched;
}

// ... 15 lines not shown

int enqueue_chunked(rdq_fwi_plan *p, int B, Pass pass, int K, const ChunkBufs &b, hipStream_t st)
{
    const std::vector<Launch> sched = chunked_schedule(p, B, pass, ckpt_plan(p, K));
    FwdTBArgs f{};
    AdjTBArgs a{};
    f.g = a.g = tb_geo(p, B);
    const size_t L = a.g.level, slice = a.g.slice;
    const int S = chain_count(p), ns = p->g.ns, nblk_alloc = gk_blocks(p);
    const bool adjoint = pass == Pass::adj_hist || pass == Pass::adj_ckpt;
    if (adjoint) {
        GkWriters writers((size_t)B * ns, nblk_alloc);
        for (const Launch &l : sched)
            if (l.kind == Launch::adj &&
                !writers.add(l.chain, l.grid, l.tiles_x, l.ntiles, B, ns, l.ns_grp, l.s_off, l.spw, l.ns_sh))
                return RDQ_E_INVALID;
    }
    if (adjoint)
        RDQ_TRY(zero_regions({{b.ring, 4 * L * sizeof(float)}, {b.gA, L * sizeof(float)},
                              {b.gk, (size_t)B * ns * nblk_alloc * sizeof(double)},
                              {b.gbeta, (size_t)B * ns * sizeof(float)}}, st));
    else if (pass == Pass::fwd_hist) RDQ_TRY(zero_regions({{b.hist, 2 * L * sizeof(float)}}, st));
    else RDQ_TRY(zero_regions({{b.ring, 4 * L * sizeof(float)}}, st));
    f.coeffs = a.coeffs = b.coeffs;
    f.cg = a.cg = coef_gen(p, B, b.coeffs);
    f.seis = b.seis; f.hist = b.hist;
    a.hist = b.hist; a.dseis = b.dseis; a.gA = b.gA; a.gk_part = b.gk; a.gbeta = b.gbeta;
    a.nblk = nblk_alloc;
    auto level = [&](LevelPair lp, int j) -> float * {
        float *base = lp.store == Store::ring ? b.ring : lp.store == Store::ckpt ? b.ckpt
                      : lp.store == Store::hist ? b.hist : nullptr;
        return base ? base + (size_t)(lp.slot + j) * L : nullptr;
    };
    RDQ_TRY(fork_chains(p, st, S));
    for (const Launch &l : sched) {
        const hipStream_t cs = l.chain == 0 ? st : p->aux[l.chain - 1];
        if (l.kind == Launch::levels) {
            const size_t run = (size_t)l.ns_sh * slice;
            const unsigned gx = (unsigned)std::min<size_t>((run + 255) / 256, 1024);
            hipLaunchKernelGGL(k_ckpt_levels, dim3(gx, 2 * B), dim3(256), 0, cs, level(l.in, 0), level(l.out, 0), L,
                               (size_t)ns * slice, (size_t)l.s_off * slice, run, B);
        } else if (l.kind == Launch::fwd) {
            f.g.s_off = l.s_off; f.g.ns_grp = l.ns_grp; f.g.tiles_x = l.tiles_x; f.g.ntiles = l.ntiles;
            f.ns_sh = l.ns_sh; f.spw = l.spw;
            f.n0 = l.first; f.nsteps = l.nsteps; f.hbase = l.hbase;
            for (int t = 0; t < FWD_W_MAX; ++t) f.w[t] = t < l.nsteps ? p->wavf[l.first + t] : 0.0f;
            f.in_prev = level(l.in, 0); f.in_cur = level(l.in, 1);
            f.out_prev = level(l.out, 0); f.out_cur = level(l.out, 1);
            launch_kernel(chunk_fwd_kernel(p, l.nsteps), l.grid, cs, f);
        } else {
            a.g.s_off = l.s_off; a.g.ns_grp = l.ns_grp; a.g.tiles_x = l.tiles_x; a.g.ntiles = l.ntiles;
            a.ns_sh = l.ns_sh; a.spw = l.spw;
            a.k0 = l.first; a.nsteps = l.nsteps; a.hbase = l.hbase;
            for (int t = 0; t < ADJ_W_MAX; ++t) a.w[t] = t < l.nsteps ? p->wavf[l.first - 1 - t] : 0.0f;
            a.in_l1 = level(l.in, 0); a.in_l2 = level(l.in, 1);
            a.out_l1 = level(l.out, 0); a.out_l2 = level(l.out, 1);
            launch_kernel(chunk_adj_kernel(p, l.nsteps), l.grid, cs, a);
        }
    }
    RDQ_CHECK(hipGetLastError());
    return join_chains(p, st, S);
}

void drop_graphs(rdq_fwi_plan *p)
{
    if (p->cache.empty()) return;
    (void)hipDeviceSynchronize();
    for (auto &e : p->cache) (void)hipGraphExecDestroy(e.exec);
    p->cache.clear();
}

template <class T>
void set_knob(rdq_fwi_plan *p, T &knob, T value)
{
    if (knob != value) drop_graphs(p);
    knob = value;
}

int fold_residuals(const rdq_fwi_plan *p, int B, const float *&dseis, float *ring, hipStream_t st)
{
    if (!p->rmulti) return 0;
    float *fold = ring + 8 * (size_t)B * p->g.ns * p->Hp * p->ld;
    const size_t rows = (size_t)B * p->g.ns * p->nrec, n = rows * p->ncolr;
    hipLaunchKernelGGL(k_rcv_fold, dim3((unsigned)std::min<size_t>((n + 255) / 256, 4096)), dim3(256), 0, st,
                       dseis, fold, p->d_colx, p->d_rcv_start, p->d_rcv_list, p->g.ng, p->ncolr, rows);
    RDQ_CHECK(hipGetLastError());
    dseis = fold;
    return 0;
}

template <class F>
int run_cached(rdq_fwi_plan *p, int kind, int B, std::initializer_list<const void *> key, hipStream_t st, F &&launch,
               int K = 0)
{
    if (!p->graphs) return launch(st);
    const void *k[8] = {nullptr};
    int n = 0;
    for (const void *v : key) k[n++] = v;
    for (auto &e : p->cache)
        if (e.kind == kind && e.B == B && e.K == K && std::equal(k, k + 8, e.ptrs)) {
            e.last_use = ++p->tick;
            RDQ_CHECK(hipGraphLaunch(e.exec, st));
            return 0;
        }
    if (!p->cap) RDQ_CHECK(hipStreamCreateWithFlags(&p->cap, hipStreamNonBlocking));
    hipGraph_t graph = nullptr;
    RDQ_CHECK(hipStreamBeginCapture(p->cap, hipStreamCaptureModeThreadLocal));
    const int rc = launch(p->cap);
    const hipError_t ee = hipStreamEndCapture(p->cap, &graph);
    if (rc) { if (graph) (void)hipGraphDestroy(graph); return rc; }
    RDQ_CHECK(ee);
    GraphEntry e{};
    e.kind = kind; e.B = B; e.K = K;
    std::copy(k, k + 8, e.ptrs);
    const hipError_t ie = hipGraphInstantiate(&e.exec, graph, nullptr, nullptr, 0);
    (void)hipGraphDestroy(graph);
    RDQ_CHECK(ie);
    e.last_use = ++p->tick;
    if (p->cache.size() >= 16) {
        auto old = std::min_element(p->cache.begin(), p->cache.end(),
                                    [](const GraphEntry &a, const GraphEntry &b) { return a.last_use < b.last_use; });
        RDQ_CHECK(hipStreamSynchronize(st));
        (void)hipGraphExecDestroy(old->exec);
        p->cache.erase(old);
    }
    p->cache.push_back(e);
    RDQ_CHECK(hipGraphLaunch(e.exec, st));
    return 0;
}

}

extern "C" {

constexpr int RDQ_RECURRENCE_MIN_NBC = 20;
static bool recurrence_ok(const rdq_fwi_plan *p) { return p->g.nbc >= RDQ_RECURRENCE_MIN_NBC; }

int rdq_fwi_plan_create(const rdq_fwi_geom *geom, rdq_fwi_plan **out)
{
    if (!geom || !out || geom->nz < 1 || geom->nx < 1 || geom->nbc < 0 || geom->nt < 1 || geom->ns < 1 ||
        geom->ng < 1 || geom->sample_temporal < 1 || !geom->isx || !geom->igx || !geom->wavelet)
        return RDQ_E_INVALID;
    rdq_fwi_plan *p = new (std::nothrow) rdq_fwi_plan();
    if (!p) return RDQ_E_NOMEM;
    p->g = *geom;
    p->Hp = geom->nz + 2 * geom->nbc;
    p->Wp = geom->nx + 2 * geom->nbc;
    p->ld = (p->Wp + 63) / 64 * 64;
    p->nrec = (geom->nt + geom->sample_temporal - 1) / geom->sample_temporal;
    p->isx.assign(geom->isx, geom->isx + geom->ns);
    p->igx.assign(geom->igx, geom->igx + geom->ng);
    p->wav.assign(geom->wavelet, geom->wavelet + geom->nt);
    p->wavf.resize(geom->nt);
    for (int i = 0; i < geom->nt; ++i) p->wavf[i] = (float)p->wav[i];
    for (int v : p->isx) if (v < 0 || v >= p->Wp) { delete p; return RDQ_E_INVALID; }
    for (int v : p->igx) if (v < 0 || v >= p->Wp) { delete p; return RDQ_E_INVALID; }
    if (geom->isz < 0 || geom->isz >= p->Hp || geom->igz < 0 || geom->igz >= p->Hp) { delete p; return RDQ_E_INVALID; }
    if (p->Wp > FIN_MAXW) { delete p; return RDQ_E_INVALID; }
    p->g.isx = p->isx.data();
    p->g.igx = p->igx.data();
    p->g.wavelet = p->wav.data();
    std::vector<int> order(geom->ng), start(p->Wp + 1, 0);
    for (int r = 0; r < geom->ng; ++r) order[r] = r;
    std::stable_sort(order.begin(), order.end(), [&](int a, int b) { return p->igx[a] < p->igx[b]; });
    for (int r = 0; r < geom->ng; ++r) start[p->igx[r] + 1]++;
    for (int x = 0; x < p->Wp; ++x) start[x + 1] += start[x];
    std::vector<int> rlane(p->Wp, -1), colx;
    for (int x = 0; x < p->Wp; ++x) {
        if (start[x + 1] - start[x] > 1) p->rmulti = true;
        if (start[x + 1] > start[x]) colx.push_back(x);
    }
    p->ncolr = (int)colx.size();
    for (int c = 0; c < p->ncolr; ++c) rlane[colx[c]] = p->rmulti ? c : order[start[colx[c]]];
    hipError_t e = hipMalloc(&p->d_isx, sizeof(int) * geom->ns);
    if (e == hipSuccess) e = hipMalloc(&p->d_rcv_start, sizeof(int) * (p->Wp + 1));
    if (e == hipSuccess) e = hipMalloc(&p->d_rcv_list, sizeof(int) * geom->ng);
    if (e == hipSuccess) e = hipMemcpy(p->d_isx, p->isx.data(), sizeof(int) * geom->ns, hipMemcpyHostToDevice);
    if (e == hipSuccess) e = hipMemcpy(p->d_rcv_start, start.data(), sizeof(int) * (p->Wp + 1), hipMemcpyHostToDevice);
    if (e == hipSuccess) e = hipMemcpy(p->d_rcv_list, order.data(), sizeof(int) * geom->ng, hipMemcpyHostToDevice);
    if (e == hipSuccess) e = hipMalloc(&p->d_rlane, sizeof(int) * p->Wp);
    if (e == hipSuccess) e = hipMemcpy(p->d_rlane, rlane.data(), sizeof(int) * p->Wp, hipMemcpyHostToDevice);
    if (e == hipSuccess) e = hipMalloc(&p->d_colx, sizeof(int) * std::max(p->ncolr, 1));
    if (e == hipSuccess && p->ncolr)
        e = hipMemcpy(p->d_colx, colx.data(), sizeof(int) * p->ncolr, hipMemcpyHostToDevice);
    if (e == hipSuccess) e = hipMalloc(&p->d_wav, sizeof(float) * geom->nt);
    if (e == hipSuccess) e = hipMemcpy(p->d_wav, p->wavf.data(), sizeof(float) * geom->nt, hipMemcpyHostToDevice);
    if (e == hipSuccess) e = hipMalloc(&p->d_status_own, 256);
    if (e == hipSuccess) e = hipMemset(p->d_status_own, 0, 256);
    p->d_status = p->d_status_own;
    p->adj_fma = recurrence_ok(p);
    if (e != hipSuccess) { rdq_fwi_plan_destroy(p); return -(int)e; }
    *out = p;
    return 0;
}

int rdq_fwi_plan_destroy(rdq_fwi_plan *p)
{
    if (!p) return 0;
    drop_graphs(p);
    if (p->cap) (void)hipStreamDestroy(p->cap);
    for (auto st : p->aux) (void)hipStreamDestroy(st);
    for (auto e : p->evs) (void)hipEventDestroy(e);
    if (p->handover) (void)hipEventDestroy(p->handover);
    if (p->d_isx) (void)hipFree(p->d_isx);
    if (p->d_rcv_start) (void)hipFree(p->d_rcv_start);
    if (p->d_rcv_list) (void)hipFree(p->d_rcv_list);
    if (p->d_rlane) (void)hipFree(p->d_rlane);
    if (p->d_colx) (void)hipFree(p->d_colx);
    if (p->d_wav) (void)hipFree(p->d_wav);
    if (p->d_status_own) (void)hipFree(p->d_status_own);
    if (p->d_prof) (void)hipFree(p->d_prof);
    delete p;
    return 0;
}

int rdq_fwi_set_graphs(rdq_fwi_plan *p, int32_t enable)
{
    if (!p) return RDQ_E_INVALID;
    std::lock_guard<std::mutex> lk(p->mu);
    p->graphs = enable != 0;
    return 0;
}

int rdq_fwi_set_tuning(rdq_fwi_plan *p, int32_t fwd_steps, int32_t adj_steps, int32_t chains)
{
    if (!p || fwd_steps < 1 || fwd_steps > TB_MAXT || adj_steps < 1 || adj_steps > TB_MAXT || chains < 0 ||
        chains > 16)
        return RDQ_E_INVALID;
    std::lock_guard<std::mutex> lk(p->mu);
    set_knob(p, p->fwd_T, fwd_steps);
    set_knob(p, p->adj_T, adj_steps);
    set_knob(p, p->chains, chains);
    return 0;
}

int rdq_fwi_set_wide_fwd_steps(rdq_fwi_plan *p, int32_t steps)
{
    if (!p || steps < 0 || steps > TW_FWD_MAXT) return RDQ_E_INVALID;
    std::lock_guard<std::mutex> lk(p->mu);
    set_knob(p, p->fwd_Tw, steps);
    return 0;
}

int rdq_fwi_set_wide_fwd_shots(rdq_fwi_plan *p, int32_t shots)
{
    if (!p || shots < 0 || shots > 64) return RDQ_E_INVALID;
    std::lock_guard<std::mutex> lk(p->mu);
    set_knob(p, p->fwd_spw, shots);
    return 0;
}

int rdq_fwi_set_wide_adj_shots(rdq_fwi_plan *p, int32_t shots)
{
    if (!p || shots < 0 || shots > 64) return RDQ_E_INVALID;
    std::lock_guard<std::mutex> lk(p->mu);
    set_knob(p, p->adj_spw, shots);
    return 0;
}

int rdq_fwi_set_wide_adj_steps(rdq_fwi_plan *p, int32_t steps)
{
    if (!p || steps < 0 || steps > TW_ADJ_MAXT) return RDQ_E_INVALID;
    std::lock_guard<std::mutex> lk(p->mu);
    set_knob(p, p->adj_Tw, steps);
    return 0;
}

int rdq_fwi_set_variant(rdq_fwi_plan *p, int32_t flags)
{
    if (!p || (flags & ~31)) return RDQ_E_INVALID;
    std::lock_guard<std::mutex> lk(p->mu);
    const bool gen = (flags & RDQ_VARIANT_FWD_GEN) != 0;
    const bool fma = (flags & RDQ_VARIANT_ADJ_EXACT) == 0 && recurrence_ok(p);
    const bool twfma = (flags & RDQ_VARIANT_CHUNKED_ADJ_FMA) != 0 && (flags & RDQ_VARIANT_ADJ_EXACT) == 0 &&
                       recurrence_ok(p);
    const int xcd = (flags & RDQ_VARIANT_NO_XCD_LOCAL) ? 0 : 1;
    const bool wide = (flags & RDQ_VARIANT_NARROW_CHUNKED) == 0;
    set_knob(p, p->fwd_gen, gen);
    set_knob(p, p->adj_fma, fma);
    set_knob(p, p->adj_tw_fma, twfma);
    set_knob(p, p->xcd_mode, xcd);
    set_knob(p, p->wide, wide);
    return 0;
}

int rdq_fwi_set_rows_per_wave(rdq_fwi_plan *p, int32_t fwd_rows, int32_t adj_rows)
{
    if (!p || (fwd_rows != 6 && fwd_rows != 8 && fwd_rows != 12 && fwd_rows != 24) ||
        (adj_rows != 6 && adj_rows != 8 && adj_rows != 12))
        return RDQ_E_INVALID;
    std::lock_guard<std::mutex> lk(p->mu);
    set_knob(p, p->fwd_rw, fwd_rows);
    set_knob(p, p->adj_rw, adj_rows);
    return 0;
}
int rdq_fwi_set_persistent(rdq_fwi_plan *p, int32_t mode)
{
    if (!p || (mode != 0 && mode != 1 && mode != 8 && mode != 12 && mode != 16 && mode != -1)) return RDQ_E_INVALID;
    std::lock_guard<std::mutex> lk(p->mu);
    set_knob(p, p->persist, mode);
    return 0;
}

int rdq_fwi_launch_info(rdq_fwi_plan *p, int32_t B, int32_t out[6])
{
    if (!p || !out || B < 1) return RDQ_E_INVALID;
    std::lock_guard<std::mutex> lk(p->mu);
    int perf = 0, pera = 0;
    out[0] = persistent_nw(p, B, false, &perf);
    out[1] = persistent_nw(p, B, true, &pera);
    out[2] = out[0] ? p->fwd_T : chunk_depth(p, false);
    out[3] = out[1] ? p->adj_T : chunk_depth(p, true);
    const int ns = B * p->g.ns;
    const CkptPlan all = ckpt_plan(p, p->g.nt);
    out[4] = out[0] ? (ns + perf - 1) / perf : count_launches(chunked_schedule(p, B, Pass::fwd_ring, all), Launch::fwd);
    out[5] = out[1] ? (ns + pera - 1) / pera : count_launches(chunked_schedule(p, B, Pass::adj_hist, all), Launch::adj);
    return 0;
}

int rdq_fwi_set_sweep_delay(rdq_fwi_plan *p, int32_t fwd_ticks, int32_t adj_ticks)
{
    if (!p || fwd_ticks < 0 || fwd_ticks > 100000 || adj_ticks < 0 || adj_ticks > 100000) return RDQ_E_INVALID;
    std::lock_guard<std::mutex> lk(p->mu);
    p->fwd_delay = fwd_ticks;
    p->adj_delay = adj_ticks;
    return 0;
}

int rdq_fwi_wide_info(rdq_fwi_plan *p, int32_t B, int32_t out[4])
{
    if (!p || !out || B < 1) return RDQ_E_INVALID;
    std::lock_guard<std::mutex> lk(p->mu);
    const CkptPlan all = ckpt_plan(p, p->g.nt);
    const Launch f = chunked_schedule(p, B, Pass::fwd_ring, all).front();
    const Launch a = chunked_schedule(p, B, Pass::adj_hist, all).front();
    out[0] = chain_count(p);
    out[1] = f.spw;
    out[2] = a.spw;
    out[3] = f.ns_sh;
    return 0;
}

int rdq_fwi_set_profile(rdq_fwi_plan *p, int32_t enable)
{
    if (!p) return RDQ_E_INVALID;
    std::lock_guard<std::mutex> lk(p->mu);
    drop_graphs(p);
    if (enable && !p->d_prof) {
        RDQ_CHECK(hipMalloc(&p->d_prof, 2 * PROF_WORDS * sizeof(unsigned long long)));
        RDQ_CHECK(hipMemset(p->d_prof, 0, 2 * PROF_WORDS * sizeof(unsigned long long)));
    } else if (!enable && p->d_prof) {
        RDQ_CHECK(hipFree(p->d_prof));
        p->d_prof = nullptr;
    }
    return 0;
}

int rdq_fwi_read_profile(rdq_fwi_plan *p, uint64_t out[12])
{
    if (!p || !out) return RDQ_E_INVALID;
    std::lock_guard<std::mutex> lk(p->mu);
    if (!p->d_prof) { for (int i = 0; i < 8; ++i) out[i] = 0; return 0; }
    RDQ_CHECK(hipDeviceSynchronize());
    p->prof_host.resize(2 * PROF_WORDS);
    RDQ_CHECK(hipMemcpy(p->prof_host.data(), p->d_prof, 2 * PROF_WORDS * sizeof(unsigned long long),
                        hipMemcpyDeviceToHost));
    RDQ_CHECK(hipMemset(p->d_prof, 0, 2 * PROF_WORDS * sizeof(unsigned long long)));
    for (int i = 0; i < 6; ++i) { out[i] = p->prof_host[i]; out[6 + i] = p->prof_host[PROF_WORDS + i]; }
    return 0;
}

int rdq_fwi_profile_waves(rdq_fwi_plan *p, int32_t adj, uint64_t *out, size_t count)
{
    if (!p || !out || (adj != 0 && adj != 1)) return RDQ_E_INVALID;
    std::lock_guard<std::mutex> lk(p->mu);
    const size_t n = std::min(count, PROF_WAVES * 3);
    for (size_t i = 0; i < n; ++i)
        out[i] = p->prof_host.empty() ? 0 : p->prof_host[(adj ? PROF_WORDS : 0) + PROF_RAW + i];
    return 0;
}

int rdq_fwi_status(rdq_fwi_plan *p, hipStream_t st)
{
    if (!p) return RDQ_E_INVALID;
    std::lock_guard<std::mutex> lk(p->mu);
    unsigned v = 0;
    RDQ_CHECK(hipMemcpyAsync(&v, p->d_status, sizeof(v), hipMemcpyDeviceToHost, st));
    RDQ_CHECK(hipStreamSynchronize(st));
    if (v) {
        RDQ_CHECK(hipMemsetAsync(p->d_status, 0, sizeof(v), st));
        RDQ_CHECK(hipStreamSynchronize(st));
        return RDQ_E_HANDOFF;
    }
    return 0;
}

int rdq_fwi_set_status_buffer(rdq_fwi_plan *p, uint32_t *words)
{
    if (!p) return RDQ_E_INVALID;
    std::lock_guard<std::mutex> lk(p->mu);
    set_knob(p, p->d_status, words ? words : p->d_status_own);
    return 0;
}

int rdq_fwi_debug_words(rdq_fwi_plan *p, uint32_t out[32])
{
    if (!p || !out) return RDQ_E_INVALID;
    std::lock_guard<std::mutex> lk(p->mu);
    RDQ_CHECK(hipDeviceSynchronize());
    RDQ_CHECK(hipMemcpy(out, p->d_status, 32 * sizeof(uint32_t), hipMemcpyDeviceToHost));
    return 0;
}

int rdq_fwi_sizes(const rdq_fwi_plan *p, int32_t B, rdq_fwi_sizes_t *o)
{
    if (!p || !o || B < 1) return RDQ_E_INVALID;
    const size_t slice = (size_t)p->Hp * p->ld, ns = p->g.ns;
    o->Hp = p->Hp; o->Wp = p->Wp; o->ld = p->ld; o->nrec = p->nrec;
    o->coeffs = (6 * (size_t)B * slice + (size_t)B * p->g.nz * p->g.nx + B + 4) * sizeof(float);
    o->vstat = (size_t)B * (sizeof(float) + sizeof(int64_t)) + 16;
    o->seis = (size_t)B * ns * p->nrec * p->g.ng * sizeof(float);
    o->history = (size_t)(p->g.nt + 2) * B * ns * slice * sizeof(float);
    o->ring = 4 * (size_t)B * ns * slice * sizeof(unsigned long long);
    if (p->rmulti) o->ring += (size_t)B * ns * p->nrec * p->ncolr * sizeof(float);
    o->gA = (size_t)B * ns * slice * sizeof(float);
    o->gk_part = (size_t)B * ns * gk_blocks(p) * sizeof(double);
    o->gbeta = (size_t)B * ns * sizeof(float);
    o->colsum = (size_t)B * p->Hp * p->g.nx * sizeof(double);
    return 0;
}

static void vstat_ptrs(const void *vstat, int B, float **vmin, int64_t **amin)
{
    char *base = (char *)vstat;
    *vmin = (float *)base;
    *amin = (int64_t *)(base + (((size_t)B * sizeof(float) + 15) / 16) * 16);
}

int rdq_fwi_coeffs(const rdq_fwi_plan *p, int32_t B, const float *vn, const int64_t strides[4],
                   int32_t vel_mode, float *coeffs, void *vstat, hipStream_t st)
{
    if (!p || !vn || !strides || !coeffs || !vstat || B < 1 || (vel_mode != 0 && vel_mode != 1))
        return RDQ_E_INVALID;
    float *vmin; int64_t *amin;
    vstat_ptrs(vstat, B, &vmin, &amin);
    CoefArgs a;
    a.cg = coef_gen(p, B, coeffs);
    const double ad = (double)(p->g.nbc - 1) * (double)p->g.dx;
    {
        const int n = p->g.nz * p->g.nx, parts = std::max(1, std::min(256, (n + 8191) / 8192));
        const int chunk = (n + parts - 1) / parts;
        float *pv = coeffs + 5 * (size_t)B * p->Hp * p->ld;
        int64_t *pi = reinterpret_cast<int64_t *>(pv + (((size_t)B * parts + 3) / 4) * 4);
        hipLaunchKernelGGL(k_vstat_part, dim3(B, parts), dim3(256), 0, st, vn, strides[0], strides[2], strides[3],
                           p->g.nz, p->g.nx, vel_mode, chunk, pv, pi);
        hipLaunchKernelGGL(k_vstat_final, dim3(B), dim3(256), 0, st, pv, pi, parts, (float)std::log(10000000.0),
                           (float)(2.0 * ad), vmin, amin, const_cast<float *>(a.cg.ks));
    }
    a.vn = vn; a.s0 = strides[0]; a.s2 = strides[2]; a.s3 = strides[3];
    a.vel_mode = vel_mode; a.ld = p->ld;
    a.vmod_out = const_cast<float *>(a.cg.vmod);
    a.coeffs = coeffs;
    a.cstride = (size_t)B * p->Hp * p->ld;
    hipLaunchKernelGGL(k_coeffs, dim3((p->ld + 255) / 256, p->Hp, B), dim3(256), 0, st, a);
    hipLaunchKernelGGL(k_coeff_fields, dim3((p->ld + 255) / 256, p->Hp, B), dim3(256), 0, st, a);
    RDQ_CHECK(hipGetLastError());
    return 0;
}

int rdq_fwi_forward(const rdq_fwi_plan *pc, int32_t B, const float *coeffs, float *seis, float *hist,
                    float *ring, hipStream_t st)
{
    rdq_fwi_plan *p = const_cast<rdq_fwi_plan *>(pc);
    if (!p || !coeffs || !seis || (!hist && !ring) || B < 1) return RDQ_E_INVALID;
    std::lock_guard<std::mutex> lk(p->mu);
    RDQ_TRY(plan_enter(p, st));
    int per = 0;
    if (const int nw = persistent_nw(p, B, false, &per)) {
        if (!ring) return RDQ_E_INVALID;
        return launch_forward_pt(p, B, nw, per, coeffs, seis, hist, ring, st);
    }
    ChunkBufs b{};
    b.coeffs = coeffs; b.seis = seis; b.hist = hist; b.ring = ring;
    return run_cached(p, hist ? 0 : 1, B, {coeffs, seis, hist, ring}, st, [&](hipStream_t s) {
        return enqueue_chunked(p, B, hist ? Pass::fwd_hist : Pass::fwd_ring, p->g.nt, b, s);
    });
}

int rdq_fwi_adjoint(const rdq_fwi_plan *pc, int32_t B, const float *coeffs, const float *hist,
                    const float *dseis, float *ring, float *gA, double *gk, float *gbeta, hipStream_t st)
{
    rdq_fwi_plan *p = const_cast<rdq_fwi_plan *>(pc);
    if (!p || !coeffs || !hist || !dseis || !ring || !gA || !gk || !gbeta || B < 1) return RDQ_E_INVALID;
    std::lock_guard<std::mutex> lk(p->mu);
    RDQ_TRY(plan_enter(p, st));
    RDQ_TRY(fold_residuals(p, B, dseis, ring, st));
    int per = 0;
    if (const int nw = persistent_nw(p, B, true, &per))
        return launch_adjoint_pt(p, B, nw, per, coeffs, hist, dseis, ring, gA, gk, gbeta, st);
    ChunkBufs b{};
    b.coeffs = coeffs; b.hist = const_cast<float *>(hist); b.ring = ring; b.dseis = dseis;
    b.gA = gA; b.gk = gk; b.gbeta = gbeta;
    return run_cached(p, 2, B, {coeffs, hist, dseis, ring, gA, gk, gbeta}, st,
                      [&](hipStream_t s) { return enqueue_chunked(p, B, Pass::adj_hist, p->g.nt, b, s); });
}

int rdq_fwi_ckpt_sizes(const rdq_fwi_plan *p, int32_t B, int32_t K, rdq_fwi_ckpt_sizes_t *o)
{
    if (!p || !o || B < 1 || K < 1) return RDQ_E_INVALID;
    const CkptPlan cp = ckpt_plan(p, K);
    const size_t level = (size_t)B * p->g.ns * p->Hp * p->ld * sizeof(float);
    o->nseg = cp.nseg;
    o->seg_levels = cp.K + 2;
    o->ckpt = 2 * (size_t)(cp.nseg - 1) * level;
    o->seg = (size_t)(cp.K + 2) * level;
    return 0;
}

int rdq_fwi_ckpt_info(rdq_fwi_plan *p, int32_t B, int32_t K, int32_t out[4])
{
    if (!p || !out || B < 1 || K < 1) return RDQ_E_INVALID;
    std::lock_guard<std::mutex> lk(p->mu);
    const CkptPlan cp = ckpt_plan(p, K);
    const std::vector<Launch> bwd = chunked_schedule(p, B, Pass::adj_ckpt, cp);
    out[0] = 0;
    out[1] = cp.nseg;
    out[2] = count_launches(chunked_schedule(p, B, Pass::fwd_ring, cp), Launch::fwd);
    out[3] = count_launches(bwd, Launch::fwd) + count_launches(bwd, Launch::adj);
    return 0;
}

int rdq_fwi_forward_ckpt(const rdq_fwi_plan *pc, int32_t B, int32_t K, const float *coeffs, float *seis,
                         float *ckpt, float *ring, hipStream_t st)
{
    rdq_fwi_plan *p = const_cast<rdq_fwi_plan *>(pc);
    if (!p || !coeffs || !seis || !ring || B < 1 || K < 1) return RDQ_E_INVALID;
    if (!ckpt && ckpt_plan(p, K).nseg > 1) return RDQ_E_INVALID;
    std::lock_guard<std::mutex> lk(p->mu);
    RDQ_TRY(plan_enter(p, st));
    ChunkBufs b{};
    b.coeffs = coeffs; b.seis = seis; b.ckpt = ckpt; b.ring = ring;
    return run_cached(p, 3, B, {coeffs, seis, ckpt, ring}, st,
                      [&](hipStream_t s) { return enqueue_chunked(p, B, Pass::fwd_ring, K, b, s); }, ckpt_plan(p, K).K);
}

int rdq_fwi_adjoint_ckpt(const rdq_fwi_plan *pc, int32_t B, int32_t K, const float *coeffs, const float *ckpt,
                         float *seg, const float *dseis, float *ring, float *gA, double *gk, float *gbeta,
                         hipStream_t st)
{
    rdq_fwi_plan *p = const_cast<rdq_fwi_plan *>(pc);
    if (!p || !coeffs || !seg || !dseis || !ring || !gA || !gk || !gbeta || B < 1 || K < 1) return RDQ_E_INVALID;
    if (!ckpt && ckpt_plan(p, K).nseg > 1) return RDQ_E_INVALID;
    std::lock_guard<std::mutex> lk(p->mu);
    RDQ_TRY(plan_enter(p, st));
    RDQ_TRY(fold_residuals(p, B, dseis, ring, st));
    ChunkBufs b{};
    b.coeffs = coeffs; b.hist = seg; b.ckpt = const_cast<float *>(ckpt); b.ring = ring; b.dseis = dseis;
    b.gA = gA; b.gk = gk; b.gbeta = gbeta;
    return run_cached(p, 4, B, {coeffs, ckpt, seg, dseis, ring, gA, gk, gbeta}, st,
                      [&](hipStream_t s) { return enqueue_chunked(p, B, Pass::adj_ckpt, K, b, s); }, ckpt_plan(p, K).K);
}

int rdq_fwi_grad_finalize(const rdq_fwi_plan *p, int32_t B, const float *coeffs, const void *vstat,
                          const float *gA, const double *gk, const float *gbeta, int32_t vel_mode,
                          double *colsum, float *out, hipStream_t st)
{
    if (!p || !coeffs || !vstat || !gA || !gk || !gbeta || !colsum || !out || B < 1 ||
        (vel_mode != 0 && vel_mode != 1))
        return RDQ_E_INVALID;
    float *vmin; int64_t *amin;
    vstat_ptrs(vstat, B, &vmin, &amin);
    FinArgs a;
    a.B = B; a.ns = p->g.ns; a.nz = p->g.nz; a.nx = p->g.nx; a.nbc = p->g.nbc; a.Hp = p->Hp; a.Wp = p->Wp;
    a.ld = p->ld; a.isz = p->g.isz; a.nblk = gk_blocks(p); a.dt = p->g.dt; a.dx = p->g.dx;
    a.scale = vel_mode == 0 ? 1500.0 : 1.0;
    a.slice = (size_t)p->Hp * p->ld; a.cstride = (size_t)B * a.slice;
    a.coeffs = coeffs; a.gA = gA; a.gbeta = gbeta; a.vmin = vmin; a.amin = amin; a.gk_part = gk;
    a.isx = p->d_isx; a.colsum = colsum; a.out = out;
    if (p->Wp > FIN_MAXW) return RDQ_E_INVALID;
    hipLaunchKernelGGL(k_fin_rows, dim3(p->Hp, B), dim3(256), 0, st, a);
    hipLaunchKernelGGL(k_fin_cols, dim3((p->g.nz * p->g.nx + 255) / 256, B), dim3(256), 0, st, a);
    RDQ_CHECK(hipGetLastError());
    return 0;
}

size_t rdq_l1_partial_bytes(int32_t B, int64_t n)
{
    const int64_t nchunk = (n + L1_BLOCK * L1_ITEMS - 1) / (L1_BLOCK * L1_ITEMS);
    return (size_t)B * nchunk * 2 * sizeof(double);
}

int rdq_l1_forward(int32_t B, int64_t n, const float *pred, const float *y, const float *mask, float *loss,
                   float *nobs, void *partial, hipStream_t st)
{
    if (B < 1 || n < 1 || !pred || !y || !loss || !nobs || !partial) return RDQ_E_INVALID;
    const int nchunk = (int)((n + L1_BLOCK * L1_ITEMS - 1) / (L1_BLOCK * L1_ITEMS));
    hipLaunchKernelGGL(k_l1_partial, dim3(nchunk, B), dim3(L1_BLOCK), 0, st, n, pred, y, mask, (double *)partial, nchunk);
    hipLaunchKernelGGL(k_l1_final, dim3(B), dim3(L1_BLOCK), 0, st, B, nchunk, (const double *)partial, loss, nobs);
    RDQ_CHECK(hipGetLastError());
    return 0;
}

int rdq_l1_backward(int32_t B, int64_t n, const float *pred, const float *y, const float *mask,
                    const float *nobs, const float *gout, float *dpred, hipStream_t st)
{
    if (B < 1 || n < 1 || !pred || !y || !nobs || !gout || !dpred) return RDQ_E_INVALID;
    hipLaunchKernelGGL(k_l1_backward, dim3((unsigned)((n + 255) / 256), B), dim3(256), 0, st, B, n, pred, y, mask,
                       nobs, gout, dpred);
    RDQ_CHECK(hipGetLastError());
    return 0;
}

int rdq_smooth_reg_forward(int32_t kind, int32_t B, int32_t H, int32_t W, const float *mu, float *loss,
                           hipStream_t st)
{
    if ((kind != 0 && kind != 1) || B < 1 || H < 2 || W < 2 || !mu || !loss) return RDQ_E_INVALID;
    hipLaunchKernelGGL(k_smooth_fwd, dim3(B), dim3(256), 0, st, kind, H, W, mu, loss);
    RDQ_CHECK(hipGetLastError());
    return 0;
}

int rdq_smooth_reg_backward(int32_t kind, int32_t B, int32_t H, int32_t W, const float *mu,
                            const float *gout, float *grad, hipStream_t st)
{
    if ((kind != 0 && kind != 1) || B < 1 || H < 2 || W < 2 || !mu || !gout || !grad) return RDQ_E_INVALID;
    hipLaunchKernelGGL(k_smooth_bwd, dim3((H * W + 255) / 256, B), dim3(256), 0, st, kind, H, W, mu, gout, grad);
    RDQ_CHECK(hipGetLastError());
    return 0;
}

}
```

### red-diffeq_amd/red_diffeq/_hip.py

```python
import ctypes
import os

import torch

_PKG = os.path.dirname(os.path.abspath(__file__))
LIB_PATH = os.environ.get("RDQ_HIP_LIB") or os.path.join(os.path.dirname(_PKG), "lib", "libred_diffeq_hip.so")

c_int32, c_int64, c_float, c_double, c_size_t, c_void_p = (
    ctypes.c_int32, ctypes.c_int64, ctypes.c_float, ctypes.c_double, ctypes.c_size_t, ctypes.c_void_p)


class FwiGeom(ctypes.Structure):
    _fields_ = [("nz", c_int32), ("nx", c_int32), ("nbc", c_int32), ("nt", c_int32),
                ("ns", c_int32), ("ng", c_int32), ("sample_temporal", c_int32),
                ("dx", c_float), ("dt", c_float), ("isz", c_int32), ("igz", c_int32),
                ("isx", ctypes.POINTER(c_int32)), ("igx", ctypes.POINTER(c_int32)),
                ("wavelet", ctypes.POINTER(c_double))]


class FwiSizes(ctypes.Structure):
    _fields_ = [("Hp", c_int32), ("Wp", c_int32), ("ld", c_int32), ("nrec", c_int32),
                ("coeffs", c_size_t), ("vstat", c_size_t), ("seis", c_size_t), ("history", c_size_t),
                ("ring", c_size_t), ("gA", c_size_t), ("gk_part", c_size_t), ("gbeta", c_size_t),
                ("colsum", c_size_t)]


class FwiCkptSizes(ctypes.Structure):
    _fields_ = [("nseg", c_int32), ("seg_levels", c_int32), ("ckpt", c_size_t), ("seg", c_size_t)]


class ConvDesc(ctypes.Structure):
    _fields_ = [(n, c_int32) for n in ("B", "cin1", "cin2", "H", "W", "cout", "kh", "kw", "pad", "in_mode")]


SIGNATURES = {
    "rdq_fwi_plan_create": (c_int32, [ctypes.POINTER(FwiGeom), ctypes.POINTER(c_void_p)]),
    "rdq_fwi_plan_destroy": (c_int32, [c_void_p]),
    "rdq_fwi_sizes": (c_int32, [c_void_p, c_int32, ctypes.POINTER(FwiSizes)]),
    "rdq_fwi_set_graphs": (c_int32, [c_void_p, c_int32]),
    "rdq_fwi_set_tuning": (c_int32, [c_void_p, c_int32, c_int32, c_int32]),
    "rdq_fwi_set_variant": (c_int32, [c_void_p, c_int32]),
    "rdq_fwi_set_wide_adj_steps": (c_int32, [c_void_p, c_int32]),
    "rdq_fwi_set_wide_adj_shots": (c_int32, [c_void_p, c_int32]),
    "rdq_fwi_set_wide_fwd_shots": (c_int32, [c_void_p, c_int32]),
    "rdq_fwi_set_wide_fwd_steps": (c_int32, [c_void_p, c_int32]),
    "rdq_fwi_set_persistent": (c_int32, [c_void_p, c_int32]),
    "rdq_fwi_set_rows_per_wave": (c_int32, [c_void_p, c_int32, c_int32]),
    "rdq_fwi_status": (c_int32, [c_void_p, c_void_p]),
    "rdq_fwi_debug_words": (c_int32, [c_void_p, ctypes.POINTER(ctypes.c_uint32)]),
    "rdq_fwi_set_status_buffer": (c_int32, [c_void_p, c_void_p]),
    "rdq_fwi_set_profile": (c_int32, [c_void_p, c_int32]),
    "rdq_fwi_profile_waves": (c_int32, [c_void_p, c_int32, ctypes.POINTER(ctypes.c_uint64), c_size_t]),
    "rdq_fwi_launch_info": (c_int32, [c_void_p, c_int32, ctypes.POINTER(c_int32)]),
    "rdq_fwi_wide_info": (c_int32, [c_void_p, c_int32, ctypes.POINTER(c_int32)]),
    "rdq_fwi_set_sweep_delay": (c_int32, [c_void_p, c_int32, c_int32]),
    "rdq_fwi_read_profile": (c_int32, [c_void_p, ctypes.POINTER(ctypes.c_uint64)]),
    "rdq_fwi_coeffs": (c_int32, [c_void_p, c_int32, c_void_p, ctypes.POINTER(c_int64), c_int32,
                                 c_void_p, c_void_p, c_void_p]),
    "rdq_fwi_forward": (c_int32, [c_void_p, c_int32, c_void_p, c_void_p, c_void_p, c_void_p, c_void_p]),
    "rdq_fwi_adjoint": (c_int32, [c_void_p, c_int32, c_void_p, c_void_p, c_void_p, c_void_p, c_void_p,
                                  c_void_p, c_void_p, c_void_p]),
    "rdq_fwi_ckpt_sizes": (c_int32, [c_void_p, c_int32, c_int32, ctypes.POINTER(FwiCkptSizes)]),
    "rdq_fwi_forward_ckpt": (c_int32, [c_void_p, c_int32, c_int32, c_void_p, c_void_p, c_void_p, c_void_p, c_void_p]),
    "rdq_fwi_adjoint_ckpt": (c_int32, [c_void_p, c_int32, c_int32, c_void_p, c_void_p, c_void_p, c_void_p, c_void_p,
                                       c_void_p, c_void_p, c_void_p, c_void_p]),
    "rdq_fwi_ckpt_info": (c_int32, [c_void_p, c_int32, c_int32, ctypes.POINTER(c_int32)]),
    "rdq_fwi_grad_finalize": (c_int32, [c_void_p, c_int32, c_void_p, c_void_p, c_void_p, c_void_p,
                                        c_void_p, c_int32, c_void_p, c_void_p, c_void_p]),
    "rdq_l1_partial_bytes": (c_size_t, [c_int32, c_int64]),
    "rdq_l1_forward": (c_int32, [c_int32, c_int64, c_void_p, c_void_p, c_void_p, c_void_p, c_void_p,
                                 c_void_p, c_void_p]),
    "rdq_l1_backward": (c_int32, [c_int32, c_int64, c_void_p, c_void_p, c_void_p, c_void_p, c_void_p,
                                  c_void_p, c_void_p]),
    "rdq_smooth_reg_forward": (c_int32, [c_int32, c_int32, c_int32, c_int32, c_void_p, c_void_p, c_void_p]),
    "rdq_smooth_reg_backward": (c_int32, [c_int32, c_int32, c_int32, c_int32, c_void_p, c_void_p,
                                          c_void_p, c_void_p]),
    "rdq_conv2d_ws_bytes": (c_size_t, [ctypes.POINTER(ConvDesc)]),
    "rdq_conv2d_tickets": (c_size_t, [ctypes.POINTER(ConvDesc)]),
    "rdq_conv2d": (c_int32, [ctypes.POINTER(ConvDesc), c_void_p, c_void_p, c_void_p, c_void_p, c_void_p, c_void_p,
                             c_void_p, c_size_t, c_void_p, c_void_p]),
    "rdq_conv2d_rms": (c_int32, [ctypes.POINTER(ConvDesc), c_void_p, c_void_p, c_void_p, c_void_p, c_void_p, c_void_p,
                                 c_void_p, c_size_t, c_void_p, c_void_p]),
    "rdq_conv2d_gn_ws_bytes": (c_size_t, [ctypes.POINTER(ConvDesc), c_int32]),
    "rdq_conv2d_gn_sc_ws_bytes": (c_size_t, [ctypes.POINTER(ConvDesc), c_int32, c_int32]),
    "rdq_conv2d_gn_sc_tickets": (c_size_t, [ctypes.POINTER(ConvDesc), c_int32]),
    "rdq_conv2d_gn_silu_sc": (c_int32, [ctypes.POINTER(ConvDesc), c_void_p, c_void_p, c_void_p, c_void_p, c_int32,
                                        c_float, c_void_p, c_void_p, c_void_p, c_void_p, c_int32, c_void_p, c_void_p,
                                        c_void_p, c_void_p, c_size_t, c_void_p, c_void_p]),
    "rdq_conv2d_gn_silu": (c_int32, [ctypes.POINTER(ConvDesc), c_void_p, c_void_p, c_void_p, c_void_p, c_int32,
                                     c_float, c_void_p, c_void_p, c_void_p, c_void_p, c_void_p, c_void_p, c_size_t,
                                     c_void_p, c_void_p]),
    "rdq_conv2d_gn_silu_lsm": (c_int32, [ctypes.POINTER(ConvDesc), c_void_p, c_void_p, c_void_p, c_void_p, c_int32,
                                         c_float, c_void_p, c_void_p, c_void_p, c_void_p, c_void_p, c_size_t,
                                         c_void_p, c_int32, c_void_p, c_int32, c_void_p, c_void_p, c_void_p, c_void_p,
                                         c_int32, c_void_p]),
    "rdq_conv2d_gn_silu_out": (c_int32, [ctypes.POINTER(ConvDesc), c_void_p, c_void_p, c_void_p, c_void_p, c_int32,
                                         c_float, c_void_p, c_void_p, c_void_p, c_void_p, c_int32, c_void_p, c_void_p,
                                         c_void_p, c_void_p, c_size_t, c_void_p, c_void_p]),
    "rdq_unet_head": (c_int32, [ctypes.POINTER(ConvDesc), c_void_p, c_void_p, c_void_p, c_void_p, c_int32, c_float,
                                c_void_p, c_void_p, c_void_p, c_int32, c_void_p, c_void_p, c_int32, c_void_p, c_void_p]),
    "rdq_conv2d_bf16_wpack_bytes": (c_size_t, [ctypes.POINTER(ConvDesc)]),
    "rdq_conv2d_stem": (c_int32, [ctypes.POINTER(ConvDesc), c_void_p, c_void_p, c_void_p, c_void_p, c_void_p]),
    "rdq_conv2d_bf16_pack": (c_int32, [ctypes.POINTER(ConvDesc), c_void_p, c_void_p, c_void_p]),
    "rdq_conv2d_bf16_ws_bytes": (c_size_t, [ctypes.POINTER(ConvDesc)]),
    "rdq_unet_set_option": (c_int32, [c_int32, c_int32]),
    "rdq_unet_options_generation": (c_int32, []),
    "rdq_conv2d_bf16": (c_int32, [ctypes.POINTER(ConvDesc), c_void_p, c_void_p, c_void_p, c_void_p, c_void_p,
                                  c_void_p, c_void_p, c_size_t, c_void_p]),
    "rdq_conv2d_bf16_gn_ws_bytes": (c_size_t, [ctypes.POINTER(ConvDesc), c_int32]),
    "rdq_conv2d_bf16_gn_silu": (c_int32, [ctypes.POINTER(ConvDesc), c_void_p, c_void_p, c_void_p, c_void_p, c_int32,
                                          c_float, c_void_p, c_void_p, c_void_p, c_void_p, c_void_p, c_void_p,
                                          c_size_t, c_void_p]),
    "rdq_conv2d_bf16_gn_silu8": (c_int32, [ctypes.POINTER(ConvDesc), c_void_p, c_void_p, c_void_p, c_void_p, c_int32,
                                           c_float, c_void_p, c_void_p, c_void_p, c_void_p, c_void_p, c_size_t,
                                           c_void_p]),
    "rdq_conv2d_bf16_gn_silu_x8": (c_int32, [ctypes.POINTER(ConvDesc), c_void_p, c_void_p, c_void_p, c_int32, c_float,
                                             c_void_p, c_void_p, c_void_p, c_void_p, c_void_p, c_void_p, c_size_t,
                                             c_void_p]),
    "rdq_conv2d_bf16_gn_silu_out": (c_int32, [ctypes.POINTER(ConvDesc), c_void_p, c_void_p, c_void_p, c_void_p,
                                              c_int32, c_float, c_void_p, c_void_p, c_void_p, c_void_p, c_int32,
                                              c_void_p, c_void_p, c_void_p, c_void_p, c_size_t, c_void_p]),
    "rdq_group_norm_ws_bytes": (c_size_t, [c_int32, c_int32, c_int32, c_int32]),
    "rdq_group_norm_silu": (c_int32, [c_int32, c_int32, c_int32, c_int32, c_float, c_void_p, c_void_p, c_void_p,
                                      c_void_p, c_void_p, c_void_p, c_void_p]),
    "rdq_rmsnorm": (c_int32, [c_int32, c_int32, c_int32, c_void_p, c_void_p, c_void_p, c_void_p, c_void_p]),
    "rdq_linear": (c_int32, [c_int32, c_int32, c_int32, c_void_p, c_void_p, c_void_p, c_int32, c_int32, c_void_p,
                             c_void_p]),
    "rdq_time_mlp": (c_int32, [c_int32, c_int32, c_float, c_void_p, c_void_p, c_void_p, c_int32, c_void_p, c_void_p,
                               c_int32, c_void_p, c_void_p]),
    "rdq_linear_silu_multi": (c_int32, [c_int32, c_int32, c_void_p, c_int32, c_void_p, c_void_p, c_void_p, c_void_p,
                                        c_void_p]),
    "rdq_sinusoidal_emb": (c_int32, [c_int32, c_int32, c_float, c_void_p, c_void_p, c_void_p]),
    "rdq_linear_attention_ws_bytes": (c_size_t, [c_int32, c_int32, c_int32, c_int32, c_int32]),
    "rdq_linear_attention": (c_int32, [c_int32, c_int32, c_int32, c_int32, c_int32, c_float, c_void_p, c_void_p,
                                       c_void_p, c_void_p, c_void_p]),
    "rdq_linear_attention_block": (c_int32, [c_int32, c_int32, c_int32, c_int32, c_int32, c_float, c_void_p,
                                             c_void_p, c_int32, c_void_p, c_void_p, c_void_p, c_void_p, c_void_p,
                                             c_void_p, c_void_p]),
    "rdq_linear_attention_bf16_ws_bytes": (c_size_t, [c_int32, c_int32, c_int32]),
    "rdq_linear_attention_f32_ws_bytes": (c_size_t, [c_int32, c_int32, c_int32]),
    "rdq_linear_attention_f32": (c_int32, [c_int32, c_int32, c_int32, c_int32, c_float, c_void_p, c_void_p, c_void_p,
                                           c_void_p, c_void_p, c_void_p, c_void_p, c_void_p, c_void_p, c_size_t,
                                           c_void_p]),
    "rdq_linear_attention_bf16": (c_int32, [c_int32, c_int32, c_int32, c_int32, c_float, c_void_p, c_void_p, c_void_p,
                                            c_void_p, c_void_p, c_void_p, c_void_p, c_void_p, c_void_p, c_size_t,
                                            c_void_p]),
    "rdq_full_attention": (c_int32, [c_int32, c_int32, c_int32, c_int32, c_int32, c_void_p, c_void_p, c_void_p,
                                     c_void_p]),
    "rdq_red_q_sample": (c_int32, [c_int32, c_int64, c_void_p, c_void_p, c_void_p, c_void_p, c_void_p, c_void_p,
                                   c_void_p]),
    "rdq_red_q_sample_t": (c_int32, [c_int32, c_int64, c_void_p, c_void_p, c_void_p, c_void_p, c_void_p, c_void_p,
                                     c_void_p, c_void_p]),
    "rdq_red_epilogue": (c_int32, [c_int32, c_int64, c_void_p, c_void_p, c_void_p, c_void_p, c_void_p, c_void_p,
                                   c_void_p, c_void_p]),
    "rdq_adam_step": (c_int32, [c_int64, c_void_p, c_void_p, c_void_p, c_void_p, c_float, c_float, c_float, c_float,
                                c_float, c_int32, c_float, c_float, c_void_p, c_void_p]),
    "rdq_metrics_ws_bytes": (c_size_t, [c_int32, c_int32, c_int32]),
    "rdq_metrics": (c_int32, [c_int32, c_int32, c_int32, c_void_p, ctypes.POINTER(c_int64), c_void_p, c_void_p, c_void_p,
                              c_void_p]),
}


_lib = None


def load_library():
    global _lib
    if _lib is None:
        if not os.path.exists(LIB_PATH):
            raise RuntimeError(
                f"red-diffeq_amd HIP library not built: {LIB_PATH} is missing "
                "(run `make -C red-diffeq_amd` or __graft_entry__.build()).")
        lib = ctypes.CDLL(LIB_PATH)
        for name, (res, args) in SIGNATURES.items():
            fn = getattr(lib, name)
            fn.restype, fn.argtypes = res, args
        _lib = lib
    return _lib


def lib():
    return load_library()


def check(rc, what):
    if rc != 0:
        raise RuntimeError(f"{what} failed with code {rc}")


def require_device(*tensors):
    for t in tensors:
        if t is not None and not t.is_cuda:
            raise RuntimeError("red-diffeq_amd kernels run on the MI355X only (got a CPU tensor); "
                               "there is deliberately no CPU fallback")


def stream_of(t):
    return c_void_p(torch.cuda.current_stream(t.device).cuda_stream)


def ptr(t):
    return c_void_p(t.data_ptr()) if t is not None else c_void_p(0)
```

### red-diffeq_amd/red_diffeq/solvers/pde.py

```python
import ctypes
import os

import numpy as np
import torch
import torch.nn as nn
import torch.nn.functional as F

from .. import _hip
from .. import ops as _ops
from ..utils.data_trans import v_denormalize


def ricker(f, dt, nt):
    nw = 2.2 / f / dt
    nw = 2 * np.floor(nw / 2) + 1
    nc = np.floor(nw / 2)
    k = np.arange(nw)
    alpha = (nc - k) * f * dt * np.pi
    beta = alpha ** 2
    w0 = (1 - beta * 2) * np.exp(-beta)
    w = np.zeros(nt)
    w[:len(w0)] = w0
    return w


def adj_sr(sx, sz, gx, gz, dx, nbc):
    isx = np.around(sx / dx) + nbc
    isz = np.around(sz / dx) + nbc
    igx = np.around(gx / dx) + nbc
    igz = np.around(gz / dx) + nbc
    return isx.astype("int"), int(isz), igx.astype("int"), int(igz)


class FwiPlan:

    def __init__(self, nz, nx, ctx, sample_temporal, isx, isz, igx, igz, wavelet, device):
        self.lib = _hip.lib()
        self.device = device
        self._isx = np.ascontiguousarray(isx, np.int32)
        self._igx = np.ascontiguousarray(igx, np.int32)
        self._wav = np.ascontiguousarray(wavelet, np.float64)
        g = _hip.FwiGeom(nz=nz, nx=nx, nbc=int(ctx["nbc"]), nt=int(ctx["nt"]), ns=len(self._isx),
                         ng=len(self._igx), sample_temporal=int(sample_temporal),
                         dx=float(ctx["dx"]), dt=float(ctx["dt"]), isz=int(isz), igz=int(igz),
                         isx=self._isx.ctypes.data_as(ctypes.POINTER(ctypes.c_int32)),
                         igx=self._igx.ctypes.data_as(ctypes.POINTER(ctypes.c_int32)),
                         wavelet=self._wav.ctypes.data_as(ctypes.POINTER(ctypes.c_double)))
        self.ns, self.ng, self.nt, self.nz, self.nx = len(self._isx), len(self._igx), int(ctx["nt"]), nz, nx
        h = ctypes.c_void_p()
        with torch.cuda.device(device):
            _hip.check(self.lib.rdq_fwi_plan_create(ctypes.byref(g), ctypes.byref(h)), "rdq_fwi_plan_create")
        self.handle = h
        self._sizes = {}
        self.persist_mode = 1
        self._saved_mode = None
        self.status_t = torch.zeros(64, dtype=torch.int32, device=device)
        _hip.check(self.lib.rdq_fwi_set_status_buffer(self.handle, _hip.ptr(self.status_t)),
                   "rdq_fwi_set_status_buffer")
        self.op_id = _ops.register_plan(self)

    def sizes(self, B):
        if B not in self._sizes:
            s = _hip.FwiSizes()
            _hip.check(self.lib.rdq_fwi_sizes(self.handle, B, ctypes.byref(s)), "rdq_fwi_sizes")
            self._sizes[B] = s
        return self._sizes[B]

    def set_graphs(self, enable):
        _hip.check(self.lib.rdq_fwi_set_graphs(self.handle, int(bool(enable))), "rdq_fwi_set_graphs")

    def set_variant(self, fwd_gen_coeffs=True, adj_exact=False, xcd_local=True, wide_chunked=True,
                    chunked_adj_fma=False):
        flags = ((1 if fwd_gen_coeffs else 0) | (2 if adj_exact else 0) | (0 if xcd_local else 4)
                 | (0 if wide_chunked else 8) | (16 if chunked_adj_fma else 0))
        _hip.check(self.lib.rdq_fwi_set_variant(self.handle, flags), "rdq_fwi_set_variant")

    def set_wide_adj_steps(self, steps):
        _hip.check(self.lib.rdq_fwi_set_wide_adj_steps(self.handle, int(steps)), "rdq_fwi_set_wide_adj_steps")

    def set_wide_adj_shots(self, shots):
        _hip.check(self.lib.rdq_fwi_set_wide_adj_shots(self.handle, int(shots)), "rdq_fwi_set_wide_adj_shots")

    def set_wide_fwd_steps(self, steps):
        _hip.check(self.lib.rdq_fwi_set_wide_fwd_steps(self.handle, int(steps)), "rdq_fwi_set_wide_fwd_steps")

    def set_wide_fwd_shots(self, shots):
        _hip.check(self.lib.rdq_fwi_set_wide_fwd_shots(self.handle, int(shots)), "rdq_fwi_set_wide_fwd_shots")

    def set_rows_per_wave(self, fwd_rows, adj_rows):
        _hip.check(self.lib.rdq_fwi_set_rows_per_wave(self.handle, int(fwd_rows), int(adj_rows)),
                   "rdq_fwi_set_rows_per_wave")

    def set_persistent(self, enable):
        mode = int(enable) if not isinstance(enable, bool) else int(enable)
        self._set_mode(mode)
        if self._saved_mode is not None:
            self._saved_mode = mode

    def _set_mode(self, mode):
        _hip.check(self.lib.rdq_fwi_set_persistent(self.handle, mode), "rdq_fwi_set_persistent")
        self.persist_mode = mode

    def status(self, stream=None):
        if stream is None:
            stream = torch.cuda.current_stream(self.device).cuda_stream
        _hip.check(self.lib.rdq_fwi_status(self.handle, ctypes.c_void_p(stream)), "rdq_fwi_status")

    def debug_words(self):
        out = (ctypes.c_uint32 * 32)()
        _hip.check(self.lib.rdq_fwi_debug_words(self.handle, out), "rdq_fwi_debug_words")
        return int(out[0]), [int(v) for v in out[1:7]], [int(v) for v in out[16:24]]

    def launch_info(self, B):
        out = (ctypes.c_int32 * 6)()
        _hip.check(self.lib.rdq_fwi_launch_info(self.handle, int(B), out), "rdq_fwi_launch_info")
        return {"fwd_persistent": bool(out[0]), "adj_persistent": bool(out[1]),
                "fwd_class": int(out[0]), "adj_class": int(out[1]), "fwd_T": int(out[2]),
                "adj_T": int(out[3]), "fwd_launches": int(out[4]), "adj_launches": int(out[5])}

    def set_sweep_delay(self, fwd_ticks, adj_ticks):
        _hip.check(self.lib.rdq_fwi_set_sweep_delay(self.handle, int(fwd_ticks), int(adj_ticks)),
                   "rdq_fwi_set_sweep_delay")

    def wide_info(self, B):
        out = (ctypes.c_int32 * 4)()
        _hip.check(self.lib.rdq_fwi_wide_info(self.handle, int(B), out), "rdq_fwi_wide_info")
        return {"chains": int(out[0]), "fwd_spw": int(out[1]), "adj_spw": int(out[2]), "chain0_shots": int(out[3])}

    def set_profile(self, enable):
        _hip.check(self.lib.rdq_fwi_set_profile(self.handle, int(bool(enable))), "rdq_fwi_set_profile")

    def read_profile(self):
        out = (ctypes.c_uint64 * 12)()
        _hip.check(self.lib.rdq_fwi_read_profile(self.handle, out), "rdq_fwi_read_profile")
        res = {}
        for name, o in (("fwd", 0), ("adj", 6)):
            n = max(int(out[o + 3]), 1)
            res[name] = {"wait_us": out[o] / n / 100.0, "steps_us": out[o + 1] / n / 100.0,
                         "publish_us": out[o + 2] / n / 100.0, "waves": int(out[o + 3]),
                         "first_pass_us": out[o + 4] / n / 100.0, "passes": out[o + 5] / n}
        return res

    def profile_waves(self, adj):
        n = 4096 * 16 * 3
        out = (ctypes.c_uint64 * n)()
        _hip.check(self.lib.rdq_fwi_profile_waves(self.handle, int(bool(adj)), out, n), "rdq_fwi_profile_waves")
        return np.frombuffer(out, dtype=np.uint64).reshape(-1, 3).astype(np.float64) / 100.0

    def set_tuning(self, fwd_steps, adj_steps, chains=0):
        _hip.check(self.lib.rdq_fwi_set_tuning(self.handle, int(fwd_steps), int(adj_steps), int(chains)),
                   "rdq_fwi_set_tuning")

    def __del__(self):
        try:
            _ops.unregister_plan(getattr(self, "op_id", -1))
        except Exception:
            pass
        h = getattr(self, "handle", None)
        if h is not None and h.value:
            try:
                self.lib.rdq_fwi_plan_destroy(h)
            except Exception:
                pass
            self.handle = None

    def coeffs(self, v, vel_mode):
        return torch.ops.red_diffeq.fwi_coeffs(v, self.op_id, vel_mode)

    def forward(self, coeffs, B, keep_history):
        seis, hist = torch.ops.red_diffeq.fwi_forward(coeffs, self.op_id, B, bool(keep_history))
        return seis, (hist if keep_history else None)

    def adjoint(self, coeffs, hist, dseis, B):
        return torch.ops.red_diffeq.fwi_adjoint(coeffs, hist, dseis, self.op_id, B)

    def finalize(self, coeffs, vstat, gA, gk, gb, B, vel_mode):
        return torch.ops.red_diffeq.fwi_grad_finalize(coeffs, vstat, gA, gk, gb, self.op_id, B, vel_mode)

    def ckpt_sizes(self, B, K):
        key = ("ckpt", int(B), int(K))
        if key not in self._sizes:
            s = _hip.FwiCkptSizes()
            _hip.check(self.lib.rdq_fwi_ckpt_sizes(self.handle, int(B), int(K), ctypes.byref(s)), "rdq_fwi_ckpt_sizes")
            self._sizes[key] = s
        return self._sizes[key]

    def ckpt_info(self, B, K):
        out = (ctypes.c_int32 * 4)()
        _hip.check(self.lib.rdq_fwi_ckpt_info(self.handle, int(B), int(K), out), "rdq_fwi_ckpt_info")
        return {"fwd_class": int(out[0]), "nseg": int(out[1]), "fwd_launches": int(out[2]),
                "bwd_launches": int(out[3])}

    def forward_ckpt(self, coeffs, B, K):
        return torch.ops.red_diffeq.fwi_forward_ckpt(coeffs, self.op_id, int(B), int(K))

    def adjoint_ckpt(self, coeffs, ckpt, dseis, B, K):
        seg = torch.empty(int(self.ckpt_sizes(B, K).seg) // 4, dtype=torch.float32, device=coeffs.device)
        return torch.ops.red_diffeq.fwi_adjoint_ckpt(coeffs, ckpt, seg, dseis, self.op_id, int(B), int(K))


def checkpoint_levels(nt, K):
    K = min(int(K), int(nt))
    nseg = -(-int(nt) // K)
    return 2 * (nseg - 1) + K + 2


def choose_checkpoint(nt, level_bytes, budget_bytes):
    nt, level_bytes = int(nt), int(level_bytes)
    if nt < 1 or level_bytes < 1:
        raise ValueError("choose_checkpoint: nt and level_bytes must be positive")
    if (nt + 2) * level_bytes <= budget_bytes:
        return None
    for K in range(nt, 0, -1):
        if checkpoint_levels(nt, K) * level_bytes <= budget_bytes:
            return K
    need = min(checkpoint_levels(nt, K) for K in range(1, nt + 1)) * level_bytes
    raise ValueError(f"history budget of {int(budget_bytes)} bytes is too small: the smallest checkpointed "
                     f"history needs {need} bytes (store-all: {(nt + 2) * level_bytes})")


class FWIForward(nn.Module):

    def __init__(self, ctx, device, sample_temporal=1, sample_spatial=1.0, normalize=True,
                 v_denorm_func=None, s_norm_func=None, shots=None, checkpoint=None, history_budget_gb=None):
        super().__init__()
        self.device = device
        self.normalize = normalize
        if normalize:
            self.v_denorm_func = v_denorm_func
            self.s_norm_func = s_norm_func
        self.sample_temporal = sample_temporal
        if "sx" not in ctx.keys():
            ctx["sx"] = np.linspace(0, ctx["n_grid"] - 1, num=ctx["ns"]) * ctx["dx"]
        else:
            ctx["sx"] = np.array(ctx["sx"]) * ctx["dx"]
        if "gx" not in ctx.keys():
            ctx["gx"] = np.linspace(0, ctx["n_grid"] - 1, num=int(sample_spatial * ctx["ng"])) * ctx["dx"]
        else:
            ctx["gx"] = np.array(ctx["gx"]) * ctx["dx"]
        self.ctx = ctx
        self.checkpoint = checkpoint if checkpoint is not None else ctx.get("checkpoint")
        self.history_budget_gb = history_budget_gb if history_budget_gb is not None else ctx.get("history_budget_gb")
        if isinstance(self.checkpoint, str):
            if self.checkpoint != "auto":
                raise ValueError(f"checkpoint must be None, an int >= 1 or 'auto', got {self.checkpoint!r}")
            if self.history_budget_gb is None:
                raise ValueError("checkpoint='auto' needs history_budget_gb")
        elif self.checkpoint is not None:
            self.checkpoint = int(self.checkpoint)
            if self.checkpoint < 1:
                raise ValueError(f"checkpoint must be >= 1, got {self.checkpoint}")
        self.shots = (0, len(ctx["sx"])) if shots is None else (int(shots[0]), int(shots[1]))
        self.shots_explicit = shots is not None
        self._plans = {}
        self._last = None
        self._fallen_back = False

    def ricker(self, f, dt, nt):
        return ricker(f, dt, nt)

    def adj_sr(self, sx, sz, gx, gz, dx, nbc):
        return adj_sr(sx, sz, gx, gz, dx, nbc)

    def get_Abc(self, vp, nbc, dx):
        dimrange = 1.0 * torch.unsqueeze(torch.arange(nbc, device=vp.device), dim=-1)
        velmin, _ = torch.min(vp.view(vp.shape[0], -1), dim=-1)
        a = (nbc - 1) * dx
        kappa = (3.0 * velmin * np.log(10000000.0) / (2.0 * a)).unsqueeze(0).expand(nbc, -1)
        prof = (kappa * (dimrange * dx / a) ** 2).permute(1, 0).unsqueeze(1)
        damp = torch.zeros_like(vp)
        H, W = vp.shape[-2:]
        damp[:, :, :nbc, :] = torch.flip(prof, dims=[-1]).unsqueeze(-1).expand(-1, -1, -1, W)
        damp[:, :, H - nbc:, :] = prof.unsqueeze(-1).expand(-1, -1, -1, W)
        damp[:, :, :, :nbc] = torch.flip(prof, dims=[-1]).unsqueeze(-2).expand(-1, -1, H, -1)
        damp[:, :, :, W - nbc:] = prof.unsqueeze(-2).expand(-1, -1, H, -1)
        return damp

    def _plan(self, nz, nx, device):
        key = (nz, nx, device.index)
        if key not in self._plans:
            c = self.ctx
            isx, isz, igx, igz = adj_sr(np.asarray(c["sx"]), c["sz"], np.asarray(c["gx"]), c["gz"],
                                        c["dx"], c["nbc"])
            isx = isx[self.shots[0]:self.shots[1]]
            if len(isx) == 0:
                raise ValueError("empty shot range")
            self._plans[key] = FwiPlan(nz, nx, c, self.sample_temporal, isx, isz, igx, igz,
                                       ricker(c["f"], c["dt"], c["nt"]), device)
            if os.environ.get("RDQ_NO_XCD_LOCAL"):
                self._plans[key].set_variant(xcd_local=False)
            if os.environ.get("RDQ_NO_GRAPHS"):
                self._plans[key].set_graphs(False)
            if os.environ.get("RDQ_ROWS_PER_WAVE"):
                self._plans[key].set_rows_per_wave(*[int(x) for x in os.environ["RDQ_ROWS_PER_WAVE"].split(",")])
            if self._fallen_back:
                plan = self._plans[key]
                plan._saved_mode = plan.persist_mode
                plan._set_mode(0)
        return self._plans[key]

    def _fused_denorm(self):
        return self.normalize and self.v_denorm_func is v_denormalize

    def forward(self, v):
        _hip.require_device(v)
        if v.dim() != 4 or v.shape[1] != 1:
            raise ValueError(f"expected v of shape (B,1,H,W), got {tuple(v.shape)}")
        if v.dtype != torch.float32:
            v = v.float()
        if self._fused_denorm():
            vel_mode = 0
        else:
            if self.normalize:
                v = self.v_denorm_func(v)
            vel_mode = 1
        plan = self._plan(v.shape[2], v.shape[3], v.device)
        self._last = plan
        keep = bool(v.requires_grad and torch.is_grad_enabled())
        K = self.checkpoint_interval(plan, v.shape[0]) if keep else None
        if K is not None:
            s = torch.ops.red_diffeq.fwi_ckpt(v, plan.op_id, vel_mode, K)[0]
        else:
            s = torch.ops.red_diffeq.fwi(v, plan.op_id, vel_mode, keep)[0]
        return self.s_norm_func(s) if self.normalize else s

    def checkpoint_interval(self, plan, B):
        if isinstance(self.checkpoint, int):
            return self.checkpoint
        if self.history_budget_gb is None:
            return None
        sz = plan.sizes(B)
        return choose_checkpoint(plan.nt, sz.history // (plan.nt + 2), int(float(self.history_budget_gb) * 2 ** 30))

    def check(self):
        for plan in self._plans.values():
            plan.status()

    def status_word(self):
        return None if self._last is None else self._last.status_t[:1]

    def fallback_to_chunked(self):
        self._fallen_back = True
        for plan in self._plans.values():
            if plan._saved_mode is None:
                plan._saved_mode = plan.persist_mode
            plan._set_mode(0)
            plan.status_t.zero_()

    def restore_persistent(self):
        self._fallen_back = False
        for plan in self._plans.values():
            mode = plan._saved_mode
            if mode is None:
                continue
            plan._saved_mode = None
            plan._set_mode(1 if mode == -1 else mode)

    def coefficients(self, v):
        _hip.require_device(v)
        plan = self._plan(v.shape[2], v.shape[3], v.device)
        v = v.float()
        if self.normalize and not self._fused_denorm():
            v = self.v_denorm_func(v)
        coeffs, vstat = plan.coeffs(v, 0 if self._fused_denorm() else 1)
        sz = plan.sizes(v.shape[0])
        f = coeffs[:6 * v.shape[0] * sz.Hp * sz.ld].view(6, v.shape[0], sz.Hp, sz.ld)[..., :sz.Wp]
        return dict(zip(("alpha", "temp1", "temp2", "kappa", "beta", "v"), f.unbind(0)))
```

Before: 3.124 million shot-timesteps/s.

## Overlap adjoint halo handoff loads with zeroing in persistent adjoint kernel

Adds a shadow sweep mode for the persistent adjoint kernel. It issues the halo-row loads for the neighbour handoff early, zeroes the stale rows while those loads are in flight, then merges them and falls back to the polling loop only if the first pass sees stale tags. This aims to hide the load latency of the inter-wave handoff wait behind other work. It is on by default for the FMA adjoint at depth 4, and it adds finer profiling counters and a control API. The early loads can read data that is not yet published, which costs an extra pass when that happens.

Result: faster. 3.166 million shot-timesteps/s (median of 6 runs) (+1.3%).

```diff
diff --git a/include/red_diffeq_fwi.h b/include/red_diffeq_fwi.h
--- a/include/red_diffeq_fwi.h
+++ b/include/red_diffeq_fwi.h
@@ -58,15 +58,18 @@
 int rdq_fwi_set_wide_fwd_steps(rdq_fwi_plan *plan, int32_t steps);
 int rdq_fwi_set_rows_per_wave(rdq_fwi_plan *plan, int32_t fwd_rows, int32_t adj_rows);
 int rdq_fwi_set_sweep_delay(rdq_fwi_plan *plan, int32_t fwd_ticks, int32_t adj_ticks);
+int rdq_fwi_set_handoff_overlap(rdq_fwi_plan *plan, int32_t fwd_mode, int32_t adj_mode);
 int rdq_fwi_set_persistent(rdq_fwi_plan *plan, int32_t mode);
 int rdq_fwi_status(rdq_fwi_plan *plan, hipStream_t stream);
 int rdq_fwi_debug_words(rdq_fwi_plan *plan, uint32_t out[32]);
 int rdq_fwi_set_status_buffer(rdq_fwi_plan *plan, uint32_t *words);
-int rdq_fwi_launch_info(rdq_fwi_plan *plan, int32_t B, int32_t out[6]);
+int rdq_fwi_launch_info(rdq_fwi_plan *plan, int32_t B, int32_t out[8]);
 int rdq_fwi_wide_info(rdq_fwi_plan *plan, int32_t B, int32_t out[4]);
 int rdq_fwi_set_profile(rdq_fwi_plan *plan, int32_t enable);
 int rdq_fwi_read_profile(rdq_fwi_plan *plan, uint64_t out[12]);
 int rdq_fwi_profile_waves(rdq_fwi_plan *plan, int32_t adj, uint64_t *out, size_t count);
+int rdq_fwi_profile_split(rdq_fwi_plan *plan, uint64_t out[10]);
+int rdq_fwi_profile_waves_split(rdq_fwi_plan *plan, int32_t adj, uint64_t *out, size_t count);
 
 #define RDQ_VEL_NORMALIZED 0
 #define RDQ_VEL_PHYSICAL 1
diff --git a/red-diffeq_amd/csrc/fwi.hip b/red-diffeq_amd/csrc/fwi.hip
--- a/red-diffeq_amd/csrc/fwi.hip
+++ b/red-diffeq_amd/csrc/fwi.hip
@@ -1036,9 +1036,10 @@
 
 constexpr int CP_SC1 = 16;
 constexpr int PT_ADJ_SG = 8;
-constexpr size_t PROF_RAW = 8;
+constexpr size_t PROF_RAW = 16;
+constexpr size_t PROF_REC = 8;
 constexpr size_t PROF_WAVES = 4096 * 16;
-constexpr size_t PROF_WORDS = PROF_RAW + PROF_WAVES * 3;
+constexpr size_t PROF_WORDS = PROF_RAW + PROF_WAVES * PROF_REC;
 constexpr unsigned long long PT_TIMEOUT_TICKS = 20000000ull;
 
 typedef unsigned int u32x2 __attribute__((ext_vector_type(2)));
@@ -1178,8 +1179,17 @@
     {                                                                                               \
         unsigned long long t0_ = 0;                                                                 \
         const unsigned long long ts_ = prof ? __builtin_amdgcn_s_memrealtime() : 0;                 \
+        unsigned long long tb_ = ts_;                                                               \
+        if (prof) tsa += ts_ - tm;                                                                  \
         if constexpr (PT_PRIO) __builtin_amdgcn_s_setprio(PT_PRIO_WAIT);                            \
-        for (unsigned pass_ = 0; live; ++pass_) {                                                   \
+        PT_SWEEP_PASSES(GR, TAG, V0, V1, SG, 0)                                                     \
+        if (prof) { tlast = __builtin_amdgcn_s_memrealtime(); tsc += tlast - tb_; }                 \
+        if constexpr (PT_PRIO) __builtin_amdgcn_s_setprio(PT_PRIO_SWEPT);                           \
+        PT_SWEEP_ZERO(V0, V1)                                                                       \
+    }
+#define PT_SWEEP_PASSES(GR, TAG, V0, V1, SG, P0)                                                    \
+    {                                                                                               \
+        for (unsigned pass_ = (P0); live; ++pass_) {                                                \
              \
             unsigned rin_ = rin, rcy_ = rcy;                                                        \
             LAUNDER(rin_); LAUNDER(rcy_);                                                           \
@@ -1203,7 +1213,7 @@
                 }                                                                                   \
             }                                                                                       \
             const bool done_ = __all(ok_);                                                          \
-            if (prof && pass_ == 0) tfp += __builtin_amdgcn_s_memrealtime() - ts_;                   \
+            if (prof && pass_ == 0) { tb_ = __builtin_amdgcn_s_memrealtime(); tfp += tb_ - ts_; tsb += tb_ - ts_; } \
             if (done_) { npass += pass_ + 1; break; }                                               \
             if (pass_ == 0) t0_ = __builtin_amdgcn_s_memrealtime();                                 \
             if ((pass_ & 15) == 15) {                                                               \
@@ -1220,7 +1230,9 @@
             }                                                                                       \
             __builtin_amdgcn_s_sleep(1);                                                            \
         }                                                                                           \
-        if constexpr (PT_PRIO) __builtin_amdgcn_s_setprio(PT_PRIO_SWEPT);                           \
+    }
+#define PT_SWEEP_ZERO(V0, V1)                                                                       \
+    {                                                                                               \
                      \
         unsigned rin_ = rin, rcy_ = rcy;                                                            \
         LAUNDER(rin_); LAUNDER(rcy_);                                                               \
@@ -1230,6 +1242,75 @@
             PT_AT(V0, r) = keep_ ? PT_AT(V0, r) : 0.0f;                                             \
             PT_AT(V1, r) = keep_ ? PT_AT(V1, r) : 0.0f;                                             \
         }                                                                                           \
+    }
+#define PT_SWEEP_ZERO_LEAN(V0, V1)                                                                  \
+    {                                                                                               \
+        unsigned rin_ = rin, rcy_ = rcy;                                                            \
+        LAUNDER(rin_); LAUNDER(rcy_);                                                               \
+        const unsigned kc_ = (keep_in ? 1u : 0u) | (cx ? 2u : 0u);                                  \
+        _Pragma("unroll") for (int r = 0; r < R; ++r) {                                             \
+            const unsigned sel_ = ((rin_ >> r) & 1u) ? 1u : (((rcy_ >> r) & 1u) ? 2u : 0u);         \
+            const bool keep_ = (kc_ & sel_) != 0u;                                                  \
+            PT_AT(V0, r) = keep_ ? PT_AT(V0, r) : 0.0f;                                             \
+            PT_AT(V1, r) = keep_ ? PT_AT(V1, r) : 0.0f;                                             \
+        }                                                                                           \
+    }
+
+#define PT_SWEEP_SHADOW(GR, TAG, V0, V1, SG, EN)                                                    \
+    {                                                                                               \
+        u32x4 xe_[(EN)];                                                                            \
+        unsigned long long tei = 0;                                                                 \
+        PT_SWEEP_EARLY(GR, xe_, EN)                                                                 \
+        PT_SWEEP_ZERO_LEAN(V0, V1)                                                                  \
+        _Pragma("unroll") for (int i_ = 0; i_ < RP; ++i_) asm volatile("" : "+v"(V0[i_]), "+v"(V1[i_])); \
+        PT_SWEEP_OV(GR, TAG, V0, V1, SG, xe_, EN)                                                   \
+    }
+#define PT_SWEEP_ROW_OFS(r) ((((rin_) >> (r)) & 1u) ? vo_hx : ((((rcy_) >> (r)) & 1u) ? vo_cx : OOB))
+#define PT_SWEEP_EARLY(GR, XE, EN)                                                                  \
+    {                                                                                               \
+        if (prof) { tei = __builtin_amdgcn_s_memrealtime(); tsa += tei - tm; }                      \
+        unsigned rin_ = rin, rcy_ = rcy;                                                            \
+        LAUNDER(rin_); LAUNDER(rcy_);                                                               \
+        _Pragma("unroll") for (int r = 0; r < (EN); ++r)                                            \
+            XE[r] = gran_get(GR, PT_SWEEP_ROW_OFS(r), PT_ROFS(r) * 16);                             \
+        asm volatile("" ::: "memory");                                                              \
+    }
+#define PT_SWEEP_MERGE(X, r, TAG, V0, V1)                                                           \
+    {                                                                                               \
+        const bool nd_ = PT_SWEEP_ROW_OFS(r) != OOB;                                                \
+        ok_ = ok_ && (!nd_ || ((X).y == (TAG) && (X).w == (TAG)));                                  \
+        PT_AT(V0, r) = nd_ ? __uint_as_float((X).x) : PT_AT(V0, r);                                 \
+        PT_AT(V1, r) = nd_ ? __uint_as_float((X).z) : PT_AT(V1, r);                                 \
+    }
+#define PT_SWEEP_OV(GR, TAG, V0, V1, SG, XE, EN)                                                    \
+    {                                                                                               \
+        constexpr int LN_ = R - (EN);                    \
+        static_assert(LN_ >= 0 && LN_ <= (SG), "PT_SWEEP_OV: one load group after the early rows"); \
+        unsigned long long t0_ = 0;                                                                 \
+        const unsigned long long ts_ = tei;                                                         \
+        unsigned long long tb_ = tei;                                                               \
+        if constexpr (PT_PRIO) __builtin_amdgcn_s_setprio(PT_PRIO_WAIT);                            \
+        bool first_ = false;                                                                        \
+        if (live) {                                                                                 \
+            unsigned rin_ = rin, rcy_ = rcy;                                                        \
+            LAUNDER(rin_); LAUNDER(rcy_);                                                           \
+            bool ok_ = true;                                                                        \
+            u32x4 x_[LN_ > 0 ? LN_ : 1];                                                            \
+            _Pragma("unroll") for (int i_ = 0; i_ < LN_; ++i_)                                      \
+                x_[i_] = gran_get(GR, PT_SWEEP_ROW_OFS((EN) + i_), PT_ROFS((EN) + i_) * 16);        \
+            _Pragma("unroll") for (int r = 0; r < (EN); ++r) PT_SWEEP_MERGE(XE[r], r, TAG, V0, V1)  \
+            _Pragma("unroll") for (int i_ = 0; i_ < LN_; ++i_) PT_SWEEP_MERGE(x_[i_], (EN) + i_, TAG, V0, V1) \
+            first_ = __all(ok_);                                                                    \
+            if (prof) {                                                                             \
+                const unsigned long long now_ = __builtin_amdgcn_s_memrealtime();                   \
+                tfp += now_ - ts_; tsb += now_ - tb_; tb_ = now_;                                   \
+            }                                                                                       \
+            if (first_) npass += 1;                                                                 \
+            else { t0_ = __builtin_amdgcn_s_memrealtime(); __builtin_amdgcn_s_sleep(1); }           \
+        }                                                                                           \
+        if (!first_) PT_SWEEP_PASSES(GR, TAG, V0, V1, SG, 1)                                        \
+        if (prof) { tlast = __builtin_amdgcn_s_memrealtime(); tsc += tlast - tb_; }                 \
+        if constexpr (PT_PRIO) __builtin_amdgcn_s_setprio(PT_PRIO_SWEPT);                           \
     }
 
 #define PT_PUBLISH(GR, TAG, V0, V1)                                                                 \
@@ -1260,6 +1341,28 @@
 
 #define PT_PROF(ACC)                                                                                \
     if (prof) { const unsigned long long now_ = __builtin_amdgcn_s_memrealtime(); ACC += now_ - tm; tm = now_; }
+#define PT_PROF_VARS                                                                                \
+    unsigned long long tsw = 0, tst = 0, tpb = 0, tgr = 0, tm = prof ? __builtin_amdgcn_s_memrealtime() : 0; \
+    unsigned long long tsa = 0, tsb = 0, tsc = 0, tsd = 0, tlast = 0;                               \
+    unsigned long long tfp = 0, npass = 0;
+#define PT_PROF_TAIL                                                                                \
+    if (prof) {                                                                                     \
+        const unsigned long long now_ = __builtin_amdgcn_s_memrealtime();                           \
+        tsw += now_ - tm; tsd += now_ - (tlast ? tlast : tm);                                       \
+        tm = now_; tlast = 0;                                                                       \
+    }
+#define PT_PROF_FLUSH                                                                               \
+    if (prof && lane == 0) {                                                                        \
+        atomicAdd(prof + 0, tsw); atomicAdd(prof + 1, tst); atomicAdd(prof + 2, tpb + tgr); atomicAdd(prof + 3, 1ull); \
+        atomicAdd(prof + 4, tfp); atomicAdd(prof + 5, npass);                                       \
+        atomicAdd(prof + 6, tsa); atomicAdd(prof + 7, tsb); atomicAdd(prof + 8, tsc); atomicAdd(prof + 9, tsd); \
+        atomicAdd(prof + 10, tgr);                                                                  \
+        if (blockIdx.x < PROF_WAVES / 16) {                                                         \
+            unsigned long long *raw = prof + PROF_RAW + ((size_t)blockIdx.x * 16 + w) * PROF_REC;   \
+            raw[0] = tsw; raw[1] = tst; raw[2] = tpb + tgr; raw[3] = tsa; raw[4] = tsb; raw[5] = tsc; \
+            raw[6] = tsd; raw[7] = tgr;                                                             \
+        }                                                                                           \
+    }
 
 #define LAUNDER(x)                                                                                  \
     do {                                                                                            \
@@ -1440,8 +1543,7 @@
     for (int r = 0; r < R; ++r) hv[r] = (((rin >> r) & 1u) && xin) ? (PT_ROFS(r) + gx) * 4 : OOB;
     const int nep = (a.nt + T - 1) / T;
     bool live = true;
-    unsigned long long tsw = 0, tst = 0, tpb = 0, tm = prof ? __builtin_amdgcn_s_memrealtime() : 0;
-    unsigned long long tfp = 0, npass = 0;
+    PT_PROF_VARS
     float wv[T];
 #pragma unroll
     for (int t = 0; t < T; ++t) wv[t] = wav_s(a.wav, min(t, a.nt - 1));
@@ -1454,7 +1556,7 @@
     for (int e = 0; e < nep; ++e) {
         const int n0 = e * T;
         const __amdgpu_buffer_rsrc_t HFe = rsrc_of(a.hist + (size_t)(n0 + 2) * L + so);
-        PT_PROF(tsw)
+        PT_PROF_TAIL
 #pragma unroll
         for (int t = 0; t < T; ++t) {
             const int n = n0 + t;
@@ -1482,15 +1584,8 @@
     }
 #undef FWD_STEP_SEL
 #undef FWD_ISSUE
-    PT_PROF(tsw)
-    if (prof && lane == 0) {
-        atomicAdd(prof + 0, tsw); atomicAdd(prof + 1, tst); atomicAdd(prof + 2, tpb); atomicAdd(prof + 3, 1ull);
-        atomicAdd(prof + 4, tfp); atomicAdd(prof + 5, npass);
-        if (blockIdx.x < PROF_WAVES / 16) {
-            unsigned long long *raw = prof + PROF_RAW + ((size_t)blockIdx.x * 16 + w) * 3;
-            raw[0] = tsw; raw[1] = tst; raw[2] = tpb;
-        }
-    }
+    PT_PROF_TAIL
+    PT_PROF_FLUSH
 }
 
 #undef FWD_HIST
@@ -1668,8 +1763,7 @@
     }
     const int nep = (a.nt + T - 1) / T;
     bool live = true;
-    unsigned long long tsw = 0, tst = 0, tpb = 0, tm = prof ? __builtin_amdgcn_s_memrealtime() : 0;
-    unsigned long long tfp = 0, npass = 0;
+    PT_PROF_VARS
     for (int e = 0; e < nep; ++e) {
         const int ke = a.nt - e * T;
         const bool last = e + 1 == nep;
@@ -1695,26 +1789,20 @@
             const unsigned tag = (unsigned)(e + 1);
             const __amdgpu_buffer_rsrc_t GR = rsrc_of(a.gran + (size_t)(2 * ((e + 1) & 1)) * L + 2 * so);
             PT_PUBLISH(GR, tag, L0, L1)
+            PT_PROF(tpb)
             ADJ_GRAD(L0, L1, PB, PHB, wv[T - 1])
             const int kn = ke - T;
-            PT_PROF(tpb)
+            PT_PROF(tgr)
             PT_SWEEP_DELAY()
             PT_SWEEP(GR, tag, L0, L1, PT_ADJ_SG)
             ADJ_ISSUE
-            PT_PROF(tsw)
+            PT_PROF_TAIL
         }
     }
 #undef DLOAD
 #undef ADJ_ISSUE
 #undef HIST_RSRC
-    if (prof && lane == 0) {
-        atomicAdd(prof + 0, tsw); atomicAdd(prof + 1, tst); atomicAdd(prof + 2, tpb); atomicAdd(prof + 3, 1ull);
-        atomicAdd(prof + 4, tfp); atomicAdd(prof + 5, npass);
-        if (blockIdx.x < PROF_WAVES / 16) {
-            unsigned long long *raw = prof + PROF_RAW + ((size_t)blockIdx.x * 16 + w) * 3;
-            raw[0] = tsw; raw[1] = tst; raw[2] = tpb;
-        }
-    }
+    PT_PROF_FLUSH
     if (xin) {
 #pragma unroll
         for (int r = 0; r < R; ++r)
@@ -1810,7 +1898,7 @@
         if (t + 1 < T || last) ADJR_GRAD(CUR, PRV, wv[t], P0, P1, P2)                               \
     }
 
-template <int T, int NW, int RW, bool PROF>
+template <int T, int NW, int RW, bool PROF, int OV = 0>
 __global__ __launch_bounds__(64 * NW) void k_adj_pr(AdjPtArgs a)
 {
     unsigned long long *const prof = PROF ? a.prof : nullptr;
@@ -1886,8 +1974,7 @@
     }
     const int nep = (a.nt + T - 1) / T;
     bool live = true;
-    unsigned long long tsw = 0, tst = 0, tpb = 0, tm = prof ? __builtin_amdgcn_s_memrealtime() : 0;
-    unsigned long long tfp = 0, npass = 0;
+    PT_PROF_VARS
     xm_init<NW>(xm, w, lane);
     __syncthreads();
     xm_put<NW>(xm, 0, w, lane, 1u, f32x2{0.0f, 0.0f}, f32x2{0.0f, 0.0f});
@@ -1917,14 +2004,16 @@
             const unsigned tag = (unsigned)(e + 1);
             const __amdgpu_buffer_rsrc_t GR = rsrc_of(a.gran + (size_t)(2 * ((e + 1) & 1)) * L + 2 * so);
             PT_PUBLISH(GR, tag, L0, L1)
+            PT_PROF(tpb)
+            const int kn = ke - T;
             ADJR_GRAD(L0, L1, wv[T - 1], QW(0), QW(1), QW(2))
-            const int kn = ke - T;
-            PT_PROF(tpb)
+            PT_PROF(tgr)
             PT_SWEEP_DELAY()
-            PT_SWEEP(GR, tag, L0, L1, PT_ADJ_SG)
+            if constexpr (OV == 0) PT_SWEEP(GR, tag, L0, L1, PT_ADJ_SG)
+            else PT_SWEEP_SHADOW(GR, tag, L0, L1, PT_ADJ_SG, (PT_ADJ_SG < R ? PT_ADJ_SG : R))
             xm_put<NW>(xm, (e + 1) * T & 1, w, lane, (unsigned)((e + 1) * T) + 1u, A[0] * L1[0], A[1] * L1[1]);
             ADJ_ISSUE
-            PT_PROF(tsw)
+            PT_PROF_TAIL
         }
         if constexpr ((T & 3) != 0) {
 #pragma unroll
@@ -1938,14 +2027,7 @@
 #undef DLOAD
 #undef ADJ_ISSUE
 #undef HIST_RSRC
-    if (prof && lane == 0) {
-        atomicAdd(prof + 0, tsw); atomicAdd(prof + 1, tst); atomicAdd(prof + 2, tpb); atomicAdd(prof + 3, 1ull);
-        atomicAdd(prof + 4, tfp); atomicAdd(prof + 5, npass);
-        if (blockIdx.x < PROF_WAVES / 16) {
-            unsigned long long *raw = prof + PROF_RAW + ((size_t)blockIdx.x * 16 + w) * 3;
-            raw[0] = tsw; raw[1] = tst; raw[2] = tpb;
-        }
-    }
+    PT_PROF_FLUSH
     double ksum = 0.0;
     if (xin) {
 #pragma unroll
@@ -1979,8 +2061,19 @@
 #undef PAIR_VERT
 #undef PT_AT
 #undef PT_SWEEP
+#undef PT_SWEEP_PASSES
+#undef PT_SWEEP_ZERO
+#undef PT_SWEEP_ZERO_LEAN
+#undef PT_SWEEP_ROW_OFS
+#undef PT_SWEEP_EARLY
+#undef PT_SWEEP_MERGE
+#undef PT_SWEEP_OV
+#undef PT_SWEEP_SHADOW
 #undef PT_PUBLISH
 #undef PT_PROF
+#undef PT_PROF_VARS
+#undef PT_PROF_TAIL
+#undef PT_PROF_FLUSH
 #undef PT_SWEEP_DELAY
 #undef PT_ROFS
 #undef PT_REGION_INIT
@@ -2276,6 +2369,7 @@
 };
 
 constexpr int RDQ_SWEEP_DELAY_FWD = 15, RDQ_SWEEP_DELAY_ADJ = 0;
+constexpr int RDQ_OVERLAP_ADJ = 1, PT_OV_T = 4;
 
 struct rdq_fwi_plan {
     rdq_fwi_geom g;
@@ -2300,6 +2394,7 @@
     int fwd_rw = 6, adj_rw = 6;
     int fwd_T = 4, adj_T = 4;
     int fwd_delay = RDQ_SWEEP_DELAY_FWD, adj_delay = RDQ_SWEEP_DELAY_ADJ;
+    int adj_ov = RDQ_OVERLAP_ADJ;
     int adj_Tw = 0;
     int fwd_Tw = 0;
     int adj_spw = 0;
@@ -2559,23 +2654,27 @@
     if (prof && T == 4) return fwd_pt_T<4, true>(NW, p->fwd_rw);
     return with_depth<TB_MAXT>(T, [&](auto t) { return fwd_pt_T<t(), false>(NW, p->fwd_rw); });
 }
-template <int T, bool PROF>
+template <int T, bool PROF, int OV = 0>
 KernelRef<AdjPtArgs> adj_pt_T(int NW, int rw, bool fma)
 {
     if (!fma) {
         if (NW != 12) return {k_adj_pt<T, 8, PROF>, 64 * 8};
         return {k_adj_pt<T, 12, PROF>, 64 * 12};
     }
-    if (NW == 16) return {k_adj_pr<T, 16, 4, PROF>, 64 * 16};
-    if (NW != 12) return {k_adj_pr<T, 8, 8, PROF>, 64 * 8};
+    if (NW == 16) return {k_adj_pr<T, 16, 4, PROF, OV>, 64 * 16};
+    if (NW != 12) return {k_adj_pr<T, 8, 8, PROF, OV>, 64 * 8};
     switch (rw) {
-    case 12: return {k_adj_pr<T, 8, 12, PROF>, 64 * 8};
-    case 6: return {k_adj_pr<T, 16, 6, PROF>, 64 * 16};
-    default: return {k_adj_pr<T, 12, 8, PROF>, 64 * 12};
-    }
-}
+    case 12: return {k_adj_pr<T, 8, 12, PROF, OV>, 64 * 8};
+    case 6: return {k_adj_pr<T, 16, 6, PROF, OV>, 64 * 16};
+    default: return {k_adj_pr<T, 12, 8, PROF, OV>, 64 * 12};
+    }
+}
+int adj_overlap(const rdq_fwi_plan *p) { return p->adj_T == PT_OV_T && p->adj_fma ? p->adj_ov : 0; }
 KernelRef<AdjPtArgs> adj_pt_kernel(const rdq_fwi_plan *p, int NW, int T, bool fma, bool prof)
 {
+    static_assert(PT_OV_T == 4, "the profiled and the overlap builds share their depth");
+    if (T == 4 && fma && adj_overlap(p))
+        return prof ? adj_pt_T<4, true, 1>(NW, p->adj_rw, true) : adj_pt_T<4, false, 1>(NW, p->adj_rw, true);
     if (prof && T == 4) return adj_pt_T<4, true>(NW, p->adj_rw, fma);
     return with_depth<TB_MAXT>(T, [&](auto t) { return adj_pt_T<t(), false>(NW, p->adj_rw, fma); });
 }
@@ -3197,7 +3296,7 @@
     return 0;
 }
 
-int rdq_fwi_launch_info(rdq_fwi_plan *p, int32_t B, int32_t out[6])
+int rdq_fwi_launch_info(rdq_fwi_plan *p, int32_t B, int32_t out[8])
 {
     if (!p || !out || B < 1) return RDQ_E_INVALID;
     std::lock_guard<std::mutex> lk(p->mu);
@@ -3210,6 +3309,8 @@
     const CkptPlan all = ckpt_plan(p, p->g.nt);
     out[4] = out[0] ? (ns + perf - 1) / perf : count_launches(chunked_schedule(p, B, Pass::fwd_ring, all), Launch::fwd);
     out[5] = out[1] ? (ns + pera - 1) / pera : count_launches(chunked_schedule(p, B, Pass::adj_hist, all), Launch::adj);
+    out[6] = 0;
+    out[7] = out[1] ? adj_overlap(p) : 0;
     return 0;
 }
 
@@ -3219,6 +3320,14 @@
     std::lock_guard<std::mutex> lk(p->mu);
     p->fwd_delay = fwd_ticks;
     p->adj_delay = adj_ticks;
+    return 0;
+}
+
+int rdq_fwi_set_handoff_overlap(rdq_fwi_plan *p, int32_t fwd_mode, int32_t adj_mode)
+{
+    if (!p || fwd_mode != 0 || adj_mode < 0 || adj_mode > 1) return RDQ_E_INVALID;
+    std::lock_guard<std::mutex> lk(p->mu);
+    p->adj_ov = adj_mode;
     return 0;
 }
 
@@ -3265,11 +3374,32 @@
     return 0;
 }
 
+int rdq_fwi_profile_split(rdq_fwi_plan *p, uint64_t out[10])
+{
+    if (!p || !out) return RDQ_E_INVALID;
+    std::lock_guard<std::mutex> lk(p->mu);
+    for (int i = 0; i < 5; ++i) {
+        out[i] = p->prof_host.empty() ? 0 : p->prof_host[6 + i];
+        out[5 + i] = p->prof_host.empty() ? 0 : p->prof_host[PROF_WORDS + 6 + i];
+    }
+    return 0;
+}
+
 int rdq_fwi_profile_waves(rdq_fwi_plan *p, int32_t adj, uint64_t *out, size_t count)
 {
     if (!p || !out || (adj != 0 && adj != 1)) return RDQ_E_INVALID;
     std::lock_guard<std::mutex> lk(p->mu);
     const size_t n = std::min(count, PROF_WAVES * 3);
+    for (size_t i = 0; i < n; ++i)
+        out[i] = p->prof_host.empty() ? 0 : p->prof_host[(adj ? PROF_WORDS : 0) + PROF_RAW + i / 3 * PROF_REC + i % 3];
+    return 0;
+}
+
+int rdq_fwi_profile_waves_split(rdq_fwi_plan *p, int32_t adj, uint64_t *out, size_t count)
+{
+    if (!p || !out || (adj != 0 && adj != 1)) return RDQ_E_INVALID;
+    std::lock_guard<std::mutex> lk(p->mu);
+    const size_t n = std::min(count, PROF_WAVES * PROF_REC);
     for (size_t i = 0; i < n; ++i)
         out[i] = p->prof_host.empty() ? 0 : p->prof_host[(adj ? PROF_WORDS : 0) + PROF_RAW + i];
     return 0;
diff --git a/red-diffeq_amd/red_diffeq/_hip.py b/red-diffeq_amd/red_diffeq/_hip.py
--- a/red-diffeq_amd/red_diffeq/_hip.py
+++ b/red-diffeq_amd/red_diffeq/_hip.py
@@ -54,6 +54,9 @@
     "rdq_fwi_launch_info": (c_int32, [c_void_p, c_int32, ctypes.POINTER(c_int32)]),
     "rdq_fwi_wide_info": (c_int32, [c_void_p, c_int32, ctypes.POINTER(c_int32)]),
     "rdq_fwi_set_sweep_delay": (c_int32, [c_void_p, c_int32, c_int32]),
+    "rdq_fwi_set_handoff_overlap": (c_int32, [c_void_p, c_int32, c_int32]),
+    "rdq_fwi_profile_split": (c_int32, [c_void_p, ctypes.POINTER(ctypes.c_uint64)]),
+    "rdq_fwi_profile_waves_split": (c_int32, [c_void_p, c_int32, ctypes.POINTER(ctypes.c_uint64), c_size_t]),
     "rdq_fwi_read_profile": (c_int32, [c_void_p, ctypes.POINTER(ctypes.c_uint64)]),
     "rdq_fwi_coeffs": (c_int32, [c_void_p, c_int32, c_void_p, ctypes.POINTER(c_int64), c_int32,
                                  c_void_p, c_void_p, c_void_p]),
diff --git a/red-diffeq_amd/red_diffeq/solvers/pde.py b/red-diffeq_amd/red_diffeq/solvers/pde.py
--- a/red-diffeq_amd/red_diffeq/solvers/pde.py
+++ b/red-diffeq_amd/red_diffeq/solvers/pde.py
@@ -112,15 +112,20 @@
         return int(out[0]), [int(v) for v in out[1:7]], [int(v) for v in out[16:24]]
 
     def launch_info(self, B):
-        out = (ctypes.c_int32 * 6)()
+        out = (ctypes.c_int32 * 8)()
         _hip.check(self.lib.rdq_fwi_launch_info(self.handle, int(B), out), "rdq_fwi_launch_info")
         return {"fwd_persistent": bool(out[0]), "adj_persistent": bool(out[1]),
                 "fwd_class": int(out[0]), "adj_class": int(out[1]), "fwd_T": int(out[2]),
-                "adj_T": int(out[3]), "fwd_launches": int(out[4]), "adj_launches": int(out[5])}
+                "adj_T": int(out[3]), "fwd_launches": int(out[4]), "adj_launches": int(out[5]),
+                "fwd_overlap": int(out[6]), "adj_overlap": int(out[7])}
 
     def set_sweep_delay(self, fwd_ticks, adj_ticks):
         _hip.check(self.lib.rdq_fwi_set_sweep_delay(self.handle, int(fwd_ticks), int(adj_ticks)),
                    "rdq_fwi_set_sweep_delay")
+
+    def set_handoff_overlap(self, fwd_mode, adj_mode):
+        _hip.check(self.lib.rdq_fwi_set_handoff_overlap(self.handle, int(fwd_mode), int(adj_mode)),
+                   "rdq_fwi_set_handoff_overlap")
 
     def wide_info(self, B):
         out = (ctypes.c_int32 * 4)()
@@ -139,6 +144,14 @@
             res[name] = {"wait_us": out[o] / n / 100.0, "steps_us": out[o + 1] / n / 100.0,
                          "publish_us": out[o + 2] / n / 100.0, "waves": int(out[o + 3]),
                          "first_pass_us": out[o + 4] / n / 100.0, "passes": out[o + 5] / n}
+        sp = (ctypes.c_uint64 * 10)()
+        _hip.check(self.lib.rdq_fwi_profile_split(self.handle, sp), "rdq_fwi_profile_split")
+        for name, o in (("fwd", 0), ("adj", 5)):
+            n = max(res[name]["waves"], 1)
+            res[name].update({"wait_a_issue_us": sp[o] / n / 100.0, "wait_b_first_us": sp[o + 1] / n / 100.0,
+                              "wait_c_later_us": sp[o + 2] / n / 100.0, "wait_d_tail_us": sp[o + 3] / n / 100.0,
+                              "gradient_us": sp[o + 4] / n / 100.0,
+                              "publish_issue_us": res[name]["publish_us"] - sp[o + 4] / n / 100.0})
         return res
 
     def profile_waves(self, adj):
@@ -146,6 +159,14 @@
         out = (ctypes.c_uint64 * n)()
         _hip.check(self.lib.rdq_fwi_profile_waves(self.handle, int(bool(adj)), out, n), "rdq_fwi_profile_waves")
         return np.frombuffer(out, dtype=np.uint64).reshape(-1, 3).astype(np.float64) / 100.0
+
+    def profile_waves_split(self, adj, ticks=False):
+        n = 4096 * 16 * 8
+        out = (ctypes.c_uint64 * n)()
+        _hip.check(self.lib.rdq_fwi_profile_waves_split(self.handle, int(bool(adj)), out, n),
+                   "rdq_fwi_profile_waves_split")
+        raw = np.frombuffer(out, dtype=np.uint64).reshape(-1, 8)
+        return raw.copy() if ticks else raw.astype(np.float64) / 100.0
 
     def set_tuning(self, fwd_steps, adj_steps, chains=0):
         _hip.check(self.lib.rdq_fwi_set_tuning(self.handle, int(fwd_steps), int(adj_steps), int(chains)),
```
